# aukeschaap/ttcross

Measured on AMD Instinct MI355X. Metric: fiber evals/s (neval / wall time of dtt_dmrgg), Ising C_64 n=51 r=32 piv=2 (d=63), higher is better.
Workload: dtype f64; 1 GPU; Ising C_64 n=51 r=32 piv=2 (d=63); driver=test_crs_ising c 64 51 32 2, bond_groups=8, transport=none (single process), arith=exact, sweeps=16

## Files before the change

### include/ttx.h

```cpp
#ifndef TTX_H
#define TTX_H
#include <stdint.h>

#ifdef __cplusplus
extern "C" {
#endif

#define TTX_OK 0
#define TTX_EINVAL 1
#define TTX_ENODEV 2
#define TTX_EHIP 3
#define TTX_ESTATE 4

#define TTX_FUN_ISING 1
#define TTX_FUN_STDNORM 2
#define TTX_FUN_MVN 3
#define TTX_FUN_HOST 4
#define TTX_FUN_COSCOEFF 5
#define TTX_FUN_DEVICE 6
#define TTX_FUN_TRAINS 7
#define TTX_FUN_PULLBACK 8

#define TTX_ARITH_EXACT 0
#define TTX_ARITH_FAST 1
// ... 53 lines not shown
typedef double (*ttx_host_fun)(const int32_t *m, const int32_t *ind, const int32_t *n, const double *par);
int ttx_set_integrand_host(ttx_engine *h, ttx_host_fun fun, const double *par);
int64_t ttx_host_calls(const ttx_engine *h);

int ttx_set_integrand_device(ttx_engine *h, const void *image, int64_t nbytes, const char *name, const double *par, int32_t npar);
int ttx_set_integrand_device_file(ttx_engine *h, const char *path, const char *name, const double *par, int32_t npar);
int ttx_eval_device(ttx_engine *h, int64_t npts, const int32_t *ind , double *out );

#define TTX_TRAINS_MAX 8
#define TTX_TOP_PRODUCT 1
#define TTX_TOP_RATIO   2
#define TTX_TOP_SQRTABS 3
#define TTX_TOP_DEVICE  4
int ttx_set_integrand_trains(ttx_engine *h, int32_t m, ttx_engine *const *x, int32_t op);
int ttx_set_integrand_trains_device(ttx_engine *h, int32_t m, ttx_engine *const *x, const void *image, int64_t nbytes,
                                    const char *name, const double *par, int32_t npar);
int ttx_set_integrand_trains_device_file(ttx_engine *h, int32_t m, ttx_engine *const *x, const char *path,
                                         const char *name, const double *par, int32_t npar);
int ttx_trainfun_last(const ttx_engine *h, double *ms, int64_t *launches, int64_t *elements);

#define TTX_PULLBACK_MAX 8
typedef struct { ttx_engine *x; const double *const *nodes; double gamma; } ttx_layer;
int ttx_set_integrand_pullback     (ttx_engine *h, int32_t m, const ttx_layer *layer, const double *const *ref ,
                                    const void *image, int64_t nbytes, const char *name, const double *par, int32_t npar);
int ttx_set_integrand_pullback_file(ttx_engine *h, int32_t m, const ttx_layer *layer, const double *const *ref,
                                    const char *path, const char *name, const double *par, int32_t npar);
int ttx_pullback_points(ttx_engine *h, int64_t npts, const int32_t *ind , double *x , double *logq, double *val);
int ttx_pullback_last(const ttx_engine *h, double *ms, int64_t *launches, int64_t *elements, int64_t *nfailed);

int ttx_run(ttx_engine *h);

int ttx_num_sweeps(const ttx_engine *h);
int ttx_get_sweeps(const ttx_engine *h, ttx_sweep_rec *out, int cap);
int ttx_get_tapes(const ttx_engine *h, int32_t *out , int64_t cap);
int64_t ttx_neval(const ttx_engine *h);
double ttx_seconds(const ttx_engine *h);
int ttx_get_ranks(const ttx_engine *h, int32_t *r );
int64_t ttx_core_size(const ttx_engine *h, int k);
int ttx_get_core(const ttx_engine *h, int k, double *buf);

int ttx_quad(ttx_engine *h, const double *w, double *val);

int ttx_accchk(ttx_engine *h, int32_t nlot, double *einf, double *efro, double *ainf, double *afro, int32_t *pivot);

int ttx_ort(ttx_engine *h);
int ttx_svd(ttx_engine *h, double tol, int32_t rmax);
int ttx_norm(ttx_engine *h, double tol, double *val);
int ttx_lognrm(ttx_engine *h, double tol, double *val);
int ttx_dot(ttx_engine *hx, ttx_engine *hy, double *val);
int ttx_ijk(ttx_engine *h, const int32_t *ind, double *val);
#define TTX_EVAL_EXACT 0
#define TTX_EVAL_MFMA 1
#define TTX_EVAL_AUTO 2
int ttx_ijk_batch(ttx_engine *h, int64_t npts, const int32_t *ind , double *out , int32_t mode);
int ttx_ijk_batch_dev(ttx_engine *h, int64_t npts, const int32_t *ind_dev, double *out_dev, int32_t mode);
int ttx_value_batch(ttx_engine *h, int64_t npts, int32_t dd, const double *x , double *out, int32_t mode);
int ttx_eval_last_mode(const ttx_engine *h);
int ttx_zquad(ttx_engine *h, int32_t nf, const double *w, double *out);

int ttx_contract(ttx_engine *h, const int32_t *keep, const double *w, ttx_engine **out);
int ttx_marginals(ttx_engine *h, const double *w, double *out);
int ttx_contract_modesum(const ttx_engine *h, double *ms, double *bytes);

int ttx_lincomb(int32_t m, const double *coef , ttx_engine *const *x , ttx_engine **out);
int ttx_hadamard(ttx_engine *x, ttx_engine *y, ttx_engine **out);
int ttx_algebra_last(const ttx_engine *h, double *ms, double *bytes_read, double *bytes_written);

int ttx_lincomb_round(int32_t m, const double *coef, ttx_engine *const *x, int32_t rsketch, double tol, int32_t rmax,
                      uint64_t seed, int32_t mode, ttx_engine **out);
int ttx_roundsum_last(const ttx_engine *h, double *ms , double *flops, int32_t *lsk , int32_t *mode_ran);

int ttx_mode_apply    (ttx_engine *h, const int32_t *m , const double *A, int32_t mode, ttx_engine **out);
int ttx_mode_apply_dev(ttx_engine *h, const int32_t *m, const double *A_dev, int32_t mode, ttx_engine **out);
int ttx_mode_apply_last(const ttx_engine *h, double *ms, double *bytes_read, double *bytes_written, double *flops, int32_t *mode_ran);

#define TTX_BASIS_COS    1
#define TTX_BASIS_LINEAR 2
#define TTX_BASIS_HALVE_FIRST 1
typedef struct { int32_t kind, flags; double a, b; const double *nodes ; } ttx_basis;

int ttx_basis_batch    (ttx_engine *h, int64_t npts, const double *x , const ttx_basis *basis , double *out, int32_t mode);
int ttx_basis_batch_dev(ttx_engine *h, int64_t npts, const double *x_dev, const ttx_basis *basis, double *out_dev, int32_t mode);
int ttx_basis_tab      (ttx_engine *h, int64_t npts, const double *phi , double *out, int32_t mode);
int ttx_basis_tab_dev  (ttx_engine *h, int64_t npts, const double *phi_dev, double *out_dev, int32_t mode);
int ttx_basis_host     (const ttx_basis *b, int32_t n, int64_t npts, const double *x, int64_t ldx, double *phi );
int ttx_basis_last     (const ttx_engine *h, double *ms_table, double *ms_chain, double *flops, int32_t *mode_ran);

int ttx_basis_grad_batch    (ttx_engine *h, int64_t npts, const double *x , const ttx_basis *basis , double *val, double *grad , int32_t mode);
int ttx_basis_grad_batch_dev(ttx_engine *h, int64_t npts, const double *x_dev, const ttx_basis *basis, double *val_dev, double *grad_dev, int32_t mode);
int ttx_basis_grad_tab      (ttx_engine *h, int64_t npts, const double *phi, const double *dphi , double *val, double *grad, int32_t mode);
int ttx_basis_grad_tab_dev  (ttx_engine *h, int64_t npts, const double *phi_dev, const double *dphi_dev, double *val_dev, double *grad_dev, int32_t mode);
int ttx_basis_host_d        (const ttx_basis *b, int32_t n, int64_t npts, const double *x, int64_t ldx, double *dphi );
int ttx_basis_grad_last     (const ttx_engine *h, double *ms_table, double *ms_back, double *ms_fwd, double *flops, int32_t *mode_ran, int64_t *chunk_ran);

int ttx_sample(ttx_engine *h, int64_t npts, const double *u , const double *w, const int32_t *fixed, int32_t *ind, double *logq, double *val);
int ttx_sample_dev(ttx_engine *h, int64_t npts, const double *u, const double *w, const int32_t *fixed, int32_t *ind, double *logq, double *val);
int ttx_sample_last(const ttx_engine *h, double *ms_head, double *bytes_head, double *ms_draw, int64_t *nfailed);

int ttx_sample_sq    (ttx_engine *h, int64_t npts, const double *u , const double *w, const int32_t *fixed,
                      double gamma, int32_t mode, int32_t *ind, double *logq, double *val);
int ttx_sample_sq_dev(ttx_engine *h, int64_t npts, const double *u, const double *w, const int32_t *fixed,
                      double gamma, int32_t mode, int32_t *ind, double *logq, double *val);
int ttx_sample_sq_last(const ttx_engine *h, double *ms_head, double *ms_rows, double *ms_pick, double *flops, int64_t *nfailed, int32_t *mode_ran);

int ttx_sample_real    (ttx_engine *h, int64_t npts, const double *u , const double *const *nodes ,
                        const double *cond , double *x , int32_t *cell , double *logq, double *val);
int ttx_sample_real_dev(ttx_engine *h, int64_t npts, const double *u, const double *const *nodes, const double *cond, double *x, int32_t *cell, double *logq, double *val);
int ttx_sample_real_last(const ttx_engine *h, double *ms_head, double *bytes_head, double *ms_draw, int64_t *nfailed);

int ttx_sample_sq_real    (ttx_engine *h, int64_t npts, const double *u , const double *const *nodes ,
                           const double *cond , double gamma, int32_t mode, double *x , int32_t *cell ,
                           double *logq, double *val);
int ttx_sample_sq_real_dev(ttx_engine *h, int64_t npts, const double *u, const double *const *nodes, const double *cond, double gamma, int32_t mode, double *x,
                           int32_t *cell, double *logq, double *val);
int ttx_sample_sq_real_last(const ttx_engine *h, double *ms_head, double *ms_rows, double *ms_pick, double *flops, int64_t *nfailed, int32_t *mode_ran);

int ttx_rosenblatt_sq_real    (ttx_engine *h, int64_t npts, const double *x , const double *const *nodes ,
                               const double *cond , double gamma, int32_t mode, double *u , int32_t *cell ,
                               double *logq, double *val);
int ttx_rosenblatt_sq_real_dev(ttx_engine *h, int64_t npts, const double *x, const double *const *nodes, const double *cond, double gamma, int32_t mode, double *u,
                               int32_t *cell, double *logq, double *val);
int ttx_rosenblatt_sq_real_last(const ttx_engine *h, double *ms_head, double *ms_rows, double *ms_cdf, double *flops, int64_t *nfailed, int32_t *mode_ran);

#define TTX_TOPK_ABS 0
#define TTX_TOPK_MAX 1
#define TTX_TOPK_MIN 2
int ttx_topk(ttx_engine *h, int32_t K, int32_t which, const int32_t *fixed , int32_t mode,
             int32_t *nfound, int32_t *ind , double *val , double *bound);
int ttx_topk_last(const ttx_engine *h, double *ms_gram, double *ms_score, double *ms_select, double *flops, int32_t *mode_ran);

int ttx_replicate(ttx_engine *h, ttx_engine **out);

int ttx_from_tt(ttx_engine **out, int32_t d, const int32_t *n, const int32_t *r, const double *cores, int32_t device);
int ttx_write(const ttx_engine *h, const char *path);
int ttx_read(ttx_engine **out, const char *path, int32_t device);
int ttx_get_modes(const ttx_engine *h, int32_t *d, int32_t *n);
int ttx_write_hdf5(const ttx_engine *h, const char *path);
int ttx_read_hdf5(ttx_engine **out, const char *path, int32_t device);

#define TTX_K_LOTTERY 0
#define TTX_K_HALFSTEP 1
#define TTX_K_ACCEPT 2
#define TTX_K_EXCHANGE 3
#define TTX_K_QUAD 4
#define TTX_K_OTHER 5
#define TTX_K_NKINDS 6
int ttx_set_profile(ttx_engine *h, int on);
int ttx_sweep_path(const ttx_engine *h);
int ttx_plan_describe(const ttx_engine *h, char *buf, int64_t cap);
int ttx_cluster_eval(const ttx_engine *h);
int ttx_arith(const ttx_engine *h);
int ttx_cluster_fallbacks(const ttx_engine *h);
int ttx_cluster_entry(const ttx_engine *h, int64_t out[3]);
int ttx_det_fallbacks(const ttx_engine *h);
int ttx_fun_id(const ttx_engine *h);
int64_t ttx_resid_halfsteps(const ttx_engine *h);
int ttx_kernel_stats(const ttx_engine *h, int64_t launches[TTX_K_NKINDS], double ms[TTX_K_NKINDS], double bytes[TTX_K_NKINDS]);


int ttx_k_residual_argmax(int32_t device, int32_t m, int32_t r, const double *a, const double *F, const double *x,
                          double *b_out, int32_t *imax, double *bmax);
int ttx_k_residual_bench(int32_t device, int64_t m, int32_t r, int32_t iters, double *avg_ms, double *bytes);
int ttx_k_eval(int32_t device, int32_t fun_id, int32_t d, const int32_t *n, const double *par, int32_t npar,
               const double *aux, int32_t naux, int64_t npts, const int32_t *ind, double *out);
int ttx_k_eval_arith(int32_t device, int32_t fun_id, int32_t d, const int32_t *n, const double *par, int32_t npar,
                     const double *aux, int32_t naux, int64_t npts, const int32_t *ind, double *out, int32_t arith);
int ttx_k_lottery(int32_t device, int32_t npnt, int32_t m, int32_t n, int32_t nz, const int32_t *zcol,
                  const int32_t *zrow, uint64_t rngpos, int32_t *points );
int ttx_k_fast_block(int32_t device, int32_t fun_id, int32_t d, int32_t n, const double *par, int32_t npar, const double *aux, int32_t naux,
                     int32_t p, int32_t rL, const int32_t *Lidx, int32_t rR, const int32_t *Ridx, int32_t cap, int32_t chain,
                     int64_t npts, const int32_t *pts, double *near, double *dv, double *piv, double *lot, double *colf, double *rowf,
                     double *nfar, double *pnt);
int ttx_fast_tables(const ttx_engine *h, int32_t group, int32_t side, int32_t bond, int32_t cols, int32_t *info, int32_t *idx, double *near,
                    double *dv, double *piv);

int ttx_k_exp(int32_t device, int64_t n, const double *x, double *out);
int ttx_exp_host(int64_t n, const double *x, double *out);

int ttx_k_latency_probe(int32_t device, double out[5]);

int ttx_k_rccl_selftest(int32_t device, int64_t msg_bytes, int32_t nsum);

int ttx_k_xcc_map(int32_t device, int32_t nblocks, int32_t *out);

#ifdef __cplusplus
}
#endif
#endif
```

### ttcross_amd/csrc/ttx_cluster.h

```cpp
#pragma once
#include "ttx_fused.h"
#include "ttx_mvn.h"
#include "ttx_cluster_rules.h"

#define CB 256

struct ClD2 { double a, b; };
struct ClStrided {
    const char *p; size_t sb; unsigned at;
    __device__ __forceinline__ ClStrided(const double *base, size_t at_, size_t stride) : p((const char *)base), sb(8 * stride), at((unsigned)(8 * at_)) {}
    __device__ __forceinline__ double operator()() { const double v = *(const double *)(p + at); p += sb; return v; }
};

__device__ __forceinline__ double f_ising_c4p(int m, int A, const double *an, const double *aw, double s1n, double s1w,
                                              double s2n, double s2w, const double *bn, const double *bw,
                                              double pv, double pvk, double pw, double pwk)
{
    const int nb = m - A - 2;
    double v = pv, w = pw, vk = pvk, wk = pwk;
    auto vstep = [&](double xv) { vk = vk * xv; v = v + vk; };
    auto wstep = [&](double xv) { wk = wk * xv; w = w + wk; };
    vstep(s2n); vstep(s1n);
    chain8v<true>(an, A, vstep);
    wstep(s1n); wstep(s2n);
    chain8v<false>(bn, nb, wstep);
    double b = 1.0 / (v * w);
    double f = 2 * b;
    auto fstep = [&](double xv) { f = f * xv; };
    chain8v<false>(aw, A, fstep);
    fstep(s1w); fstep(s2w);
    chain8v<false>(bw, nb, fstep);
    return f;
}

template <class STEP>
__device__ __forceinline__ void chain8w(const double *p, int nc, STEP step)
{
#pragma unroll 1
    for (int ch = 0; ch < nc; ch++) {
        double x[8];
        ld8d(p + 8 * ch, x);
#pragma unroll
        for (int k = 0; k < 8; k++) step(x[k]);
    }
}
__device__ __forceinline__ double f_ising_c4w(int cA, int cB, const double *an, const double *aw, double s1n, double s1w,
                                              double s2n, double s2w, const double *bn, const double *bw,
                                              double pv, double pvk, double pw, double pwk)
{
    double v = pv, w = pw, vk = pvk, wk = pwk;
    auto vstep = [&](double xv) { vk = vk * xv; v = v + vk; };
    auto wstep = [&](double xv) { wk = wk * xv; w = w + wk; };
    vstep(s2n); vstep(s1n);
    chain8w(an, cA, vstep);
    wstep(s1n); wstep(s2n);
    chain8w(bn, cB, wstep);
    double b = 1.0 / (v * w);
    double f = 2 * b;
    auto fstep = [&](double xv) { f = f * xv; };
    chain8w(aw, cA, fstep);
    fstep(s1w); fstep(s2w);
    chain8w(bw, cB, fstep);
    return f;
}

__device__ __forceinline__ double wave_max_key(double x)
{
    const ClKey k = cl_key(x);
    const int hmax = wave_max_i(k.hi);
    const unsigned lmax = wave_max_u(cl_key_lo_at(k, hmax));
    return cl_unkey(ClKey{hmax, lmax});
}
__device__ __forceinline__ void wave_argmax2(double &a, double &v, int &idx)
{
    const double amx = wave_max_key(a);
    const int key = (a == amx && idx != INT_MAX) ? ((idx << 1) | (signbit(v) ? 1 : 0)) : INT_MAX;
    const int kmin = wave_min_i(key);
    a = amx;
    if (kmin == INT_MAX) { idx = INT_MAX; v = 0.0; }
    else { idx = kmin >> 1; v = (kmin & 1) ? -amx : amx; }
}

__device__ __forceinline__ double f_ising_cfast(double xj, double wj, double xk, double wk, double pv, double pvk, double pw, double pwk,
                                                double SL, double WL, double SR, double WR)
{
    const double v = pv + pvk * xk * (1.0 + xj * (1.0 + SL));
    const double w = pw + pwk * xj * (1.0 + xk * (1.0 + SR));
    return 2.0 / (v * w) * ((WL * wj) * (wk * WR));
}

typedef unsigned int u4 __attribute__((ext_vector_type(4)));
struct ClRec { u4 a, b; };
static_assert(sizeof(ClRec) == sizeof(ClPart), "record buffers are sized as ClPart: [2][G][TTX_CLREC] u4 arg-max records, then as many running-maximum records");
__device__ __forceinline__ void st16(void *p, u4 v) { asm volatile("global_store_dwordx4 %0, %1, off sc1" :: "v"(p), "v"(v) : "memory"); }
__device__ __forceinline__ u4 ld16(const void *p)
{
    u4 v;
    asm volatile("global_load_dwordx4 %0, %1, off sc1\n\ts_waitcnt vmcnt(0)" : "=v"(v) : "v"(p) : "memory");
    return v;
}

__device__ __forceinline__ int xcc_id() { return (int)__builtin_amdgcn_s_getreg(((4 - 1) << 11) | 20) & 15; }

__device__ __forceinline__ bool cluster_sync(unsigned *ctr, unsigned target, int *abortflag, int *s_ok)
{
    asm volatile("s_waitcnt vmcnt(0)" ::: "memory");
    __syncthreads();
    if (threadIdx.x == 0) {
        int ok = 1;
        unsigned spins = 0;
        __hip_atomic_fetch_add(ctr, 1u, __ATOMIC_RELEASE, __HIP_MEMORY_SCOPE_AGENT);
        while (__hip_atomic_load(ctr, __ATOMIC_RELAXED, __HIP_MEMORY_SCOPE_AGENT) < target) {
            __builtin_amdgcn_s_sleep(1);
            if (++spins > (1u << 22)) { ok = 0; __hip_atomic_store(abortflag, 1, __ATOMIC_RELAXED, __HIP_MEMORY_SCOPE_SYSTEM); break; }
            if ((spins & 1023u) == 0 && __hip_atomic_load(abortflag, __ATOMIC_RELAXED, __HIP_MEMORY_SCOPE_SYSTEM)) { ok = 0; break; }
        }
        __atomic_thread_fence(__ATOMIC_ACQUIRE);
        *s_ok = ok;
    }
    __syncthreads();
    return *s_ok != 0;
}

#ifdef TTX_STAMPS
#define CST_DECL const bool t_me = (threadIdx.x == 0 && g == 0 && cb == 0); long long t_prev = wall_clock64()
#define CST(k) do { if (t_me) { long long t_now = wall_clock64(); gs.stamp[0][k] += t_now - t_prev; t_prev = t_now; } } while (0)
#define CST_END() do { if (t_me) gs.nstamp[0]++; } while (0)
#define CSE_DECL const int t_eb = (threadIdx.x == 0 && g == 0 && cb <= 1) ? cb : -1; long long t_eprev = wall_clock64()
#define CSE_MARK() do { if (t_eb >= 0) t_eprev = wall_clock64(); } while (0)
#define CSE(k) do { if (t_eb >= 0) { long long t_now = wall_clock64(); P.gs[0].stamp[1][8 * t_eb + (k)] += t_now - t_eprev; t_eprev = t_now; } } while (0)
#define CSE_END() do { if (t_eb == 0) P.gs[0].nstamp[1]++; } while (0)
#define WST(k) do { if (P.dbg && g == 0 && epoch == 8 && pp == 4 && lane == 0 && h < 8) P.dbg[((size_t)(h * 64 + cb * 4 + wv)) * 8 + (k)] = (long long)__builtin_readcyclecounter(); } while (0)
#else
#define WST(k)
#define CST_DECL
#define CST(k)
#define CST_END()
#define CSE_DECL
#define CSE_MARK()
#define CSE(k)
#define CSE_END()
#endif

#define CL_ZKEEP 1
#define CL_ZCARRY 2
#define CL_WORD 4
#define CL_POWTAB 8
static_assert(CL_POWTAB_N == CB, "one table entry per thread of a workgroup");
__device__ const ClPowTab cl_powtab = cl_make_powtab();
struct ClArgs { DevProb P; int dir, nsteps, NB, ldsinv, epoch, zkeep; };
__device__ __forceinline__ int *cl_zimage(const DevProb &P, int g, int nsteps)
{ return (int *)(P.cl_part + (size_t)2 * P.G * TTX_CLREC) + (size_t)g * cl_zimage_ints(nsteps, P.RM); }

template <bool CFAST, bool CPAD>
__global__ __launch_bounds__(CB) void k_sweep_cluster(DevProb P, int dir, int nsteps, int NB, int ldsinv, int epoch, int zkeep)
{
    extern __shared__ __align__(16) double dyn[];
    __shared__ int zc[128], zr[128], zcs[128], zrs[128], keepc[128], keepr[128];
    __shared__ int nzc, nzr, nsc, nsr, s_ok;
    __shared__ int slt[2][TTX_CLMAX + 1], wtab[TTX_CLMAX];
    __shared__ ttx_cdfseg segc[TTX_TABSEG], segr[TTX_TABSEG];
    __shared__ double sha[8], shv[8], shm[8]; __shared__ int shi[8];
    __shared__ double pLw[64], pLk[64], pRv[64], pRk[64];
    static_assert(!(CFAST && CPAD), "the closed form reads the rows in dimension order");
    constexpr int NFT = CFAST ? 64 : 1;
    __shared__ double fSL[NFT], fWL[NFT], fSR[NFT], fWR[NFT];
    __shared__ struct { int ii, jj, kk, qq, hcount, rc_k, rc_q, rr_i, rr_j; double pivot, amax, bytes_half; long long neval, n_resid; } s_rook;
    const int bid = blockIdx.x;
    const int g = (bid & 7) + 8 * (bid / (8 * NB)), cb = (bid >> 3) % NB;
    CSE_DECL;
    if (g >= P.G || P.ctl[0]) return;
    const int bpar = (epoch - 1) & 1;
    if (P.tail_side && epoch >= 2) {
        const TailRec &t0 = P.tailrec[(size_t)bpar * P.G];
        if (stop_rule(epoch - 1, P.maxrank, P.accuracy, t0.pivotmax, max_pos(t0.amax, P.gs[0].amax_bnd[bpar]), P.strk[epoch & 1]).ready) return;
    }
    if (P.cl_test_abort && P.cl_test_abort == epoch && g == 0 && cb == 0) {
        if (threadIdx.x == 0) { __hip_atomic_store(P.cl_abort, 1, __ATOMIC_RELAXED, __HIP_MEMORY_SCOPE_SYSTEM); P.ctl[0] = 1; }
        return;
    }
    const int tid = threadIdx.x, m = P.d, RM = P.RM, NM = P.NM;
    const int lane = tid & 63, wv = tid >> 6;
    GroupState &gs = P.gs[g];
    const int first = gs.first, last = gs.last, nbonds = last - first + 1;
    int *r = P.r + (size_t)g * (m + 2);
    const int VS = ((m + 7) & ~7) + 8;
    const int RS = 2 * VS + 2;
    const int n1m = P.n[1];
    const int SL = RM * ((NM + NB - 1) / NB + 1);
    unsigned *ctr = P.cl_ctr + g;
    unsigned nbar = (unsigned)(epoch - 1) * (unsigned)min(nsteps, nbonds);
    ClPart *part = P.cl_part;
    double *par = dyn;
    double *XL = par + ((P.npar + 1) & ~1);
    double *XR = XL + (size_t)RM * RS;
    double *acol = XR + (size_t)RM * RS;
    double *arow = acol + SL;
    double *resc = arow + SL;
    double *resr = resc + SL;
    double *xsc = resr + SL;
    double *xsr = xsc + ((RM + 1) & ~1);
    int *lot = (int *)(xsr + ((RM + 1) & ~1));
    double *GL = (double *)(lot + 4 * ((2 * RM + 2 * NM + 4 + 1) & ~1));
    double *GU = GL + (size_t)RM * RM;
    int *ZK = (int *)(ldsinv ? GU + (size_t)RM * RM : GL);
    int *ZN = ZK + (size_t)nsteps * 2 * RM;
    for (int x = tid; x < P.npar; x += CB) par[x] = P.par[x];
    if (cb == 0) {
        if (tid == 0) { gs.pivotmax = -1.0; gs.pivotmin = -1.0; }
        int *rr = P.rr + (size_t)g * (m + 2);
        for (int s = tid; s <= m; s += CB) rr[s] = r[s];
    }
    __syncthreads();
    CSE(0);
    if ((zkeep & CL_ZCARRY) && cl_lists_valid(gs.zk_epoch, epoch)) {
        const int *img = cl_zimage(P, g, nsteps);
        for (int x = tid; x < nbonds * 2 * RM; x += CB) ZK[x] = img[x];
        for (int x = tid; x < 2 * nbonds; x += CB) ZN[x] = img[(size_t)nsteps * 2 * RM + x];
        if (cb == 0 && tid == 0) gs.n_zload++;
        __syncthreads();
    } else if (zkeep & CL_ZKEEP) {
        int *TMP = (int *)XL;
        const int E = nbonds * 2 * RM;
        for (int x = tid; x < E; x += CB) {
            const int b = x / (2 * RM), side = (x / RM) & 1, u = x % RM, pb = first + b;
            if (u < r[pb]) { const int *vp = vip_ptr(P, g, pb, first) + 4 * u; TMP[x] = (vp[2 * side + 1] << 16) | vp[2 * side]; }
        }
        __syncthreads();
        for (int x = tid; x < E; x += CB) {
            const int b = x / (2 * RM), u = x % RM, nb_ = r[first + b];
            if (u < nb_) {
                const int *src = TMP + (x - u); const int a = src[u]; int ra = 0;
                for (int t = 0; t < nb_; t++) ra += (src[t] < a) || (src[t] == a && t < u);
                ZK[(x - u) + ra] = a;
            }
        }
        __syncthreads();
        for (int x = tid; x < E; x += CB) {
            const int b = x / (2 * RM), u = x % RM, nb_ = r[first + b];
            if (u < nb_) {
                const int *src = ZK + (x - u); int pc = 0;
                for (int t = 1; t <= u; t++) pc += (src[t] != src[t - 1]);
                const bool keep = (u == 0) || (src[u] != src[u - 1]);
                TMP[x] = keep ? pc : -1;
                if (u == nb_ - 1) ZN[x / RM] = pc + 1;
            }
        }
        __syncthreads();
        int mykey = 0, mypos = -1;
        for (int x0 = 0; x0 < E; x0 += CB) {
            const int x = x0 + tid;
            mypos = -1;
            if (x < E) { const int b = x / (2 * RM), u = x % RM; if (u < r[first + b]) { mypos = TMP[x]; mykey = ZK[x]; } }
            __syncthreads();
            if (mypos >= 0) ZK[(x - x % RM) + mypos] = mykey;
            __syncthreads();
        }
    }
    double amax = gs.amax, pivotmax = -1.0, pivotmin = -1.0;
    if (P.tail_side && epoch >= 2) amax = max_pos(amax, gs.amax_bnd[bpar]);
    const double pivotmax_prev = gs.pivotmax_prev;
    long long neval = gs.neval;
    unsigned long long rngpos = gs.rngpos;
    double bytes_half = gs.bytes_half; long long n_resid = gs.n_resid;
    int hcount = 0;
    CSE(1);
    const bool ptab = (zkeep & CL_POWTAB) != 0;
    const unsigned long long bil0 = ptab ? cl_powtab.v[tid] : ttx_minstd_pow(2ull * tid);
    unsigned long long sA0;
    {
        const unsigned long long cw = gs.rngword, cwpos = gs.rngword_pos;
        if ((zkeep & CL_WORD) && cl_word_valid(cw, cwpos, rngpos)) { sA0 = cw; if (cb == 0 && tid == 0) gs.n_wload++; }
        else sA0 = ttx_minstd_pow(2 * rngpos + 1);
    }
    const int bl0 = ptab ? (int)cl_powtab.v[lane] : (int)ttx_minstd_pow(2ull * lane);
    constexpr unsigned long long c64 = cl_minstd_pow_c(128);
    CSE(2);
    CST_DECL;

    for (int pp = 1; pp <= nsteps; pp++) {
        if (pp > nbonds) break;
        const int p = (dir == 1) ? first + pp - 1 : last + 1 - pp;
        const int r0 = r[p - 1], r1 = r[p], r2 = r[p + 1], n1 = P.n[p], n2 = P.n[p + 1];
        const int nlot = r0 + n1 + n2 + r2;
        double *Cp = core_ptr(P, P.col, g, p, first), *Wq = core_ptr(P, P.row, g, p + 1, first);
        double *Ap = core_ptr(P, P.arg, g, p, first), *Aq = core_ptr(P, P.arg, g, p + 1, first);
        const short *Lt = L_ptr(P, g, p - 1, first), *Rt = R_ptr(P, g, p + 1, first);
        const int cA = (p - 1 + 7) >> 3, cB = (m - p - 1 + 7) >> 3;
        const int sside = (tid >> 6) & 1, sseg = tid & 63;
        double sg_a0 = 0.0, sg_al = 0.0, sg_de = 0.0; int sg_k0 = 0, sg_cn = 0, myns = 0;
        auto seg_issue = [&](int Kc_, int Kr_) {
            if (tid >= 128) {
                const int K = sside ? Kr_ : Kc_; const ttx_cdfseg *sp = P.cdf_tab + (size_t)K * TTX_TABSEG + sseg;
                myns = P.cdf_ns[K]; sg_a0 = sp->a0; sg_al = sp->alast; sg_de = sp->delta; sg_k0 = sp->k0; sg_cn = sp->cnt;
            }
        };
        {
            const int AL = min(VS, (p - 1 + 7) & ~7), AR = min(VS, (m - p - 1 + 7) & ~7);
            if (AL > 0) {
                int c = tid / AL, o = tid - c * AL;
// ... 232 lines not shown
            if (resid) wave_argmax2(ab, bb, ix);
            WST(5);
            if (!ok) {
                if (lane == 0) { __hip_atomic_store(P.cl_abort, 1, __ATOMIC_RELAXED, __HIP_MEMORY_SCOPE_SYSTEM); P.ctl[0] = 1; *(volatile int *)&s_ok = 0; }
                return;
            }
            CST(9);
            hcount++;
            neval += nf;
            bytes_half += resid ? 8.0 * ((double)nf * r1 + r1 + 2.0 * nf) : 8.0 * nf;
            n_resid += resid ? 1 : 0;
            done = dn;
            if (resid) {
                if (ix == INT_MAX) ix = 0;
                if (iscol) { const int i = ix % r0 + 1, j = ix / r0 + 1; done = havecol && haverow && (i == ii && j == jj); ii = i; jj = j; }
                else       { const int k = ix % n2 + 1, q = ix / n2 + 1; done = havecol && haverow && (k == kk && q == qq); kk = k; qq = q; }
                pivot = bb;
            }
        }
        if (P.piv != 0) {
            u4 *bufB = (u4 *)part + ((size_t)((hcount - 1) & 1) * P.G + g) * TTX_CLREC + (size_t)2 * P.G * TTX_CLREC;
            const unsigned gen = ((unsigned)epoch << 20) | (unsigned)hcount;
            double mx = 0.0; int ok = 1;
            if (slot_on) {
                unsigned spins = 0;
                for (;;) {
                    const u4 rb = ld16(&bufB[lane]);
                    if (rb.z == gen) { mx = __longlong_as_double((long long)(((unsigned long long)rb.y << 32) | rb.x)); break; }
                    if (++spins > 64u) __builtin_amdgcn_s_sleep(1);
                    if (spins > (1u << 22)) { ok = 0; break; }
                    if ((spins & 1023u) == 0 && __hip_atomic_load(P.cl_abort, __ATOMIC_RELAXED, __HIP_MEMORY_SCOPE_SYSTEM)) { ok = 0; break; }
                }
            }
            ok = __all(ok);
            if (!ok) {
                if (lane == 0) { __hip_atomic_store(P.cl_abort, 1, __ATOMIC_RELAXED, __HIP_MEMORY_SCOPE_SYSTEM); P.ctl[0] = 1; *(volatile int *)&s_ok = 0; }
                return;
            }
            amax = fmax(amax, wave_max_key(mx));
        }
        if (tid == 0) {
            s_rook.ii = ii; s_rook.jj = jj; s_rook.kk = kk; s_rook.qq = qq; s_rook.hcount = hcount; s_rook.rc_k = rc_k; s_rook.rc_q = rc_q;
            s_rook.rr_i = rr_i; s_rook.rr_j = rr_j; s_rook.pivot = pivot; s_rook.amax = amax; s_rook.bytes_half = bytes_half; s_rook.neval = neval; s_rook.n_resid = n_resid;
        }
        }
        __syncthreads();
        if (!*(volatile int *)&s_ok) return;
        if (!rook_active) {
            ii = s_rook.ii; jj = s_rook.jj; kk = s_rook.kk; qq = s_rook.qq; hcount = s_rook.hcount; rc_k = s_rook.rc_k; rc_q = s_rook.rc_q;
            rr_i = s_rook.rr_i; rr_j = s_rook.rr_j; pivot = s_rook.pivot; amax = s_rook.amax; bytes_half = s_rook.bytes_half; neval = s_rook.neval; n_resid = s_rook.n_resid;
        }
        CST(10);
        int *tape = P.tape + ((size_t)g * (m + 2) + p) * 4;
        const bool upd = accept_pivot(pivot, amax, pivotmax_prev, P.small_element, P.small_pivot);
        if (!upd) {
            if (cb == 0 && tid == 0) { tape[0] = tape[1] = tape[2] = tape[3] = -1; P.upd[(size_t)g * (m + 2) + p] = 0; }
        } else {
            const int i0 = ii - 1, j0 = jj - 1, k0 = kk - 1, q0 = qq - 1;
            double *gI = inv_ptr(P, g, p, first);
            const bool reuseA = (rc_k == kk && rc_q == qq), reuseB = (rr_i == ii && rr_j == jj);
            AppendTab tab{0, 0};
            if (cb == 0) tab = append_tables_fetch(P, g, p, first, ii, qq, tid);
            if (reuseA && reuseB) {
                if (cb == 0)
                    for (int s = tid; s < r1; s += CB) {
                        const double c = Wq[k0 + (size_t)NM * q0 + P.SW * s], w = Cp[i0 + (size_t)RM * j0 + P.SS * s];
                        gI[r1 * r1 + s] = w; gI[r1 * r1 + r1 + s] = c;
                    }
            } else {
                for (int s = tid; s < r1; s += CB) { xsc[s] = Wq[k0 + (size_t)NM * q0 + P.SW * s]; xsr[s] = Cp[i0 + (size_t)RM * j0 + P.SS * s]; }
                __syncthreads();
                if (cb == 0)
                    for (int s = tid; s < r1; s += CB) { gI[r1 * r1 + s] = xsr[s]; gI[r1 * r1 + r1 + s] = xsc[s]; }
            }
            for (int u = tid; u < r0 * nj; u += CB) {
                const int i = u % r0, j = jlo + u / r0; const size_t o = i + (size_t)RM * j;
                const double a = acol[u];
                Ap[o + P.SS * r1] = a;
                double y;
                if (reuseA) y = resc[u];
                else {
                    y = a;
                    ClStrided lc(Cp, o, P.SS); const double *xp = xsc;
                    cl_ordered_sum<16>(r1u, [&] { const double xv = *xp++; return ClD2{xv, lc()}; }, [&](int, ClD2 e) { y = y + (-e.a) * e.b; });
                }
                Cp[o + P.SS * r1] = (1.0 / pivot) * y;
            }
            for (int u = tid; u < nk * r2; u += CB) {
                const int k = klo + u % nk, q = u / nk;
                const double a = arow[u];
                Aq[r1 + (size_t)RM * k + P.SS * q] = a;
                const size_t o = k + (size_t)NM * q;
                if (reuseB) Wq[o + P.SW * r1] = resr[u];
                else {
                    double tt = 0.0;
                    ClStrided lw(Wq, o, P.SW); const double *xp = xsr;
                    cl_ordered_sum<16>(r1u, [&] { const double xv = *xp++; return ClD2{lw(), xv}; }, [&](int, ClD2 e) { tt = tt + e.a * e.b; });
                    Wq[o + P.SW * r1] = a + (-1.0) * tt;
                }
            }
            CST(11);
            if (p > first) {
                const double *gL = ldsinv ? GL : inv_ptr(P, g, p - 1, first);
                double *Wp = core_ptr(P, P.row, g, p, first);
                const int pk = (r0 <= 32) ? 2 : 1, lw = 64 / pk, l = lane & (lw - 1), sub = lane / lw;
                for (int base = wv * pk; base < nj; base += (CB / 64) * pk) {
                    const int jl = base + sub, j = jlo + jl;
                    const bool on = (jl < nj) && (l < r0);
                    const double a = on ? acol[l + r0 * jl] : 0.0;
                    const double xf = (pk == 2) ? dev_solve_L<2>(gL, r0, a, l, sub) : dev_solve_L<1>(gL, r0, a, l, 0);
                    if (on) Wp[j + (size_t)NM * r1 + P.SW * l] = xf;
                }
            }
            CST(12);
            if (p < last) {
                const double *gU = ldsinv ? GU : inv_ptr(P, g, p + 1, first);
                double *Cq = core_ptr(P, P.col, g, p + 1, first);
                const int pk = (r2 <= 32) ? 2 : 1, lw = 64 / pk, l = lane & (lw - 1), sub = lane / lw;
                const double rdg = dev_solve_rdg(gU, r2, l);
                for (int base = wv * pk; base < nk; base += (CB / 64) * pk) {
                    const int kl = base + sub, k = klo + kl;
                    const bool on = (kl < nk) && (l < r2);
                    const double y0 = on ? arow[kl + nk * l] : 0.0;
                    const double y = (pk == 2) ? dev_solve_U<2>(gU, r2, y0, rdg, l, sub) : dev_solve_U<1>(gU, r2, y0, rdg, l, 0);
                    if (on) Cq[r1 + (size_t)RM * k + P.SS * l] = y;
                }
            }
            CST(13);
            if (cb == 0) {
                append_tables_store(P, g, p, first, r1, ii, jj, kk, qq, tid, CB, tab);
                if (tid == 0) append_scalars(P, g, p, first, r1, ii, jj, kk, qq, pivot);
            }
            if ((zkeep & CL_ZKEEP) && wv < 2) {
                const int b = p - first;
                int *kl = ZK + (size_t)b * 2 * RM + (size_t)wv * RM;
                const int nl = ZN[2 * b + wv];
                const int key = wv == 0 ? ((jj << 16) | ii) : ((qq << 16) | kk);
                const int v = (lane < nl) ? kl[lane] : INT_MAX;
                const bool dup = __ballot(v == key) != 0ull;
                const int pos = __popcll(__ballot(v < key));
                if (!dup) {
                    if (lane < nl && v > key) kl[lane + 1] = v;
                    if (lane == 0) { kl[pos] = key; ZN[2 * b + wv] = nl + 1; }
                }
            }
            pivot_range(pivotmax, pivotmin, fabs(pivot));
        }
        CST(14);
        if (!cluster_sync(ctr, (++nbar) * (unsigned)NB, P.cl_abort, &s_ok)) { if (tid == 0) P.ctl[0] = 1; return; }
        CST(15);
        CST_END();
    }
    CSE_MARK();
    if (cb == 0) {
        const ClArgs *K = (const ClArgs *)__builtin_amdgcn_kernarg_segment_ptr();
        asm volatile("" : "+s"(K));
        if (K->zkeep & CL_ZCARRY) {
            const int ns = K->nsteps, rm = K->P.RM;
            int *img = cl_zimage(K->P, g, ns);
            for (int x = tid; x < nbonds * 2 * rm; x += CB) img[x] = ZK[x];
            for (int x = tid; x < 2 * nbonds; x += CB) img[(size_t)ns * 2 * rm + x] = ZN[x];
        }
        if (tid == 0) {
            gs.amax = amax; gs.pivotmax = pivotmax; gs.pivotmin = pivotmin; gs.neval = neval; gs.rngpos = rngpos;
            gs.bytes_half = bytes_half; gs.n_resid = n_resid;
            if (K->zkeep & CL_WORD) { gs.rngword = sA0; gs.rngword_pos = rngpos; }
            if (K->zkeep & CL_ZCARRY) gs.zk_epoch = K->epoch;
            if (P.tail_side) gs.amax_bnd[epoch & 1] = 0.0;
        }
        __syncthreads();
        exch_pack_group(P, g);
        CSE(3);
        CSE_END();
    }
}
```

### ttcross_amd/csrc/ttx_cluster_rules.h

```cpp
#pragma once
#include "ttx_cdf.h"

TTX_HD int cl_slice(int c, int n, int NB) { return (int)((unsigned)c * (unsigned)n / (unsigned)NB); }

TTX_HD int cl_wact(int nj, int nk, int r0, int r2, int nw)
{
    const int a = r0 * nj, b = nk * r2, e = a > b ? a : b, w = (e + 63) >> 6;
    return w < 1 ? 1 : (w > nw ? nw : w);
}

struct ClKey { int hi; unsigned lo; };
TTX_HD ClKey cl_key(double x) { const uint64_t b = ttx_dbits(x); return ClKey{(int)(uint32_t)(b >> 32), (unsigned)b}; }
TTX_HD double cl_unkey(ClKey k) { return ttx_bitsd(((uint64_t)(uint32_t)k.hi << 32) | k.lo); }
TTX_HD unsigned cl_key_lo_at(ClKey k, int hmax) { return k.hi == hmax ? k.lo : 0u; }

#if defined(__clang__)
#define CL_UNROLL _Pragma("unroll")
#define CL_NO_UNROLL _Pragma("unroll 1")
#else
#define CL_UNROLL
#define CL_NO_UNROLL
#endif
template <int N, class LD, class TM>
TTX_HD void cl_sum_piece(int s0, LD &ld, TM &tm)
{
    decltype(ld()) v[N];
    CL_UNROLL
    for (int k = 0; k < N; k++) v[k] = ld();
    CL_UNROLL
    for (int k = 0; k < N; k++) tm(s0 + k, v[k]);
}
template <int B, class LD, class TM>
TTX_HD void cl_ordered_sum(int n, LD ld, TM tm)
{
    static_assert(B == 16 || B == 8, "batches of 16 or 8 terms");
    int s = 0;
    CL_NO_UNROLL
    for (; s + B <= n; s += B) cl_sum_piece<B>(s, ld, tm);
    const int rem = n - s;
    if constexpr (B > 8) if (rem & 8) { cl_sum_piece<8>(s, ld, tm); s += 8; }
    if (rem & 4) { cl_sum_piece<4>(s, ld, tm); s += 4; }
    if (rem & 2) { cl_sum_piece<2>(s, ld, tm); s += 2; }
    if (rem & 1) cl_sum_piece<1>(s, ld, tm);
}

#define CL_POWTAB_N 256
constexpr uint64_t cl_mulmod31_c(uint64_t a, uint64_t b)
{
    uint64_t x = a * b;
    x = (x & 2147483647ULL) + (x >> 31);
    x = (x & 2147483647ULL) + (x >> 31);
    return (x >= 2147483647ULL) ? x - 2147483647ULL : x;
}
constexpr uint64_t cl_minstd_pow_c(uint64_t e)
{
    uint64_t base = 48271ULL, w = 1;
    while (e) { if (e & 1) w = cl_mulmod31_c(w, base); base = cl_mulmod31_c(base, base); e >>= 1; }
    return w;
}
struct ClPowTab { uint32_t v[CL_POWTAB_N]; };
constexpr ClPowTab cl_make_powtab()
{
    ClPowTab t{};
    for (int k = 0; k < CL_POWTAB_N; k++) t.v[k] = (uint32_t)cl_minstd_pow_c(2ULL * (uint64_t)k);
    return t;
}

template <class LANE>
TTX_HD uint64_t cl_stepmul(int nlot, LANE lane, uint64_t c64)
{
    if (nlot >= 512) return ttx_minstd_pow(2ull * (uint64_t)nlot);
    uint64_t s = lane(nlot & 63);
    for (int a = 0; a < (nlot >> 6); a++) s = ttx_mulmod31(s, c64);
    return s;
}

TTX_HD bool cl_word_valid(uint64_t word, uint64_t wpos, uint64_t rngpos) { return word != 0 && wpos == rngpos; }
TTX_HD bool cl_lists_valid(int tag, int epoch) { return tag != 0 && tag == epoch - 1; }
TTX_HD size_t cl_zimage_ints(int nsteps, int RM) { return ((size_t)nsteps * 2 * (size_t)RM + 2 * (size_t)nsteps + 3) & ~(size_t)3; }
```

### ttcross_amd/csrc/ttx_create_plan.h

```cpp
#pragma once
#include <algorithm>
#include <cmath>
#include <cstdarg>
#include <cstddef>
#include <cstdio>
#include <cstdlib>
#include <cstring>
#include <mutex>
#include <string>
#include <vector>

#include "../../include/ttx.h"
#include "ttx_dev.h"
#include "ttx_qr_plan.h"

#if defined(__HIPCC__)
#define TTX_PLAN_HD __host__ __device__ inline
#else
#define TTX_PLAN_HD inline
#endif

#define DE5_W 4
#define DE5_SEG 16
TTX_PLAN_HD size_t de5_lds_doubles(int m) { const int VS = ((m + 7) & ~7) + 8 + DE5_SEG; return (size_t)5 * VS + 128 + (size_t)DE5_W * 64; }
TTX_PLAN_HD bool de5_fits(int m) { return m >= 3; }
TTX_PLAN_HD int de_rows_stride(int m) { const int s = m + 56; return ((s + 31) & ~31) + 16; }
TTX_PLAN_HD size_t de_rows_lds_doubles(int m) { return (size_t)12 * de_rows_stride(m); }
TTX_PLAN_HD int det_vs(int m) { return ((m + 7) & ~7) + 8; }
TTX_PLAN_HD size_t det_lds_doubles(int m, int nbk) { return (size_t)4 * det_vs(m) + 256 + (det_vs(m) + 48) + (size_t)3 * nbk * 16 * 64; }

constexpr int TTX_PLAN_FB = 1024;
constexpr int TTX_PLAN_FNR = 24;
constexpr int TTX_PLAN_MVN_MAXQ = 8;

struct EnvText { bool set = false; std::string v; };
struct CreateEnv {
    EnvText arith;
    EnvText sweep;
    EnvText cl_pad;
    bool fullpiv_mfma = false;
    bool fast_persist_off = false;
    bool de_lane = false;
    bool de_tables_off = false, de_fastdiv_off = false, de_cut_off = false, de_v2_off = false, de_team_off = false;
    bool de_lot_point_set = false; int de_lot_point = 0;
    int de_team_units = 256, de_team6_units = 1024;
    int de_test_fault = 0;
    bool de_v5 = false;
    int cluster_nb = 8;
    bool cluster_coop = false;
    int cluster_test_abort = 0;
    bool dbg_waves = false;
    bool lottery_one_block = false;
    bool lottery_wave_off = false;
    bool lottery_rows2 = false;
    bool mvn_v2_off = false;
    bool tail_off = false;
    bool tail_side_off = false;
    bool head_direct_off = false;
    bool init_wave_off = false;
    bool fin_early_off = false;
    bool fin_skip_exch_off = false;
    bool init_wide_off = false;
    bool quad_lds_off = false;
    bool cl_powtab_off = false;
    bool cl_word_off = false;
    bool cl_lists_off = false;
};
template <class Get>
CreateEnv create_env_from(Get get)
{
    auto text = [&](const char *name) { EnvText t; if (const char *e = get(name)) { t.set = true; t.v = e; } return t; };
    auto num = [&](const char *name, int dflt) { const char *e = get(name); return e ? atoi(e) : dflt; };
    auto off = [&](const char *name) { const char *e = get(name); return e && atoi(e) == 0; };
    CreateEnv v;
    v.arith = text("TTX_ARITH"); v.sweep = text("TTX_SWEEP"); v.cl_pad = text("TTX_CL_PAD");
    v.fullpiv_mfma = text("TTX_FULLPIV").v == "mfma";
    v.fast_persist_off = off("TTX_FAST_PERSIST");
    v.de_lane = num("TTX_DE_LANE", 0) == 1;
    v.de_tables_off = off("TTX_DE_TABLES"); v.de_fastdiv_off = off("TTX_DE_FASTDIV"); v.de_cut_off = off("TTX_DE_CUT");
    v.de_v2_off = off("TTX_DE_V2"); v.de_team_off = off("TTX_DE_TEAM");
    v.de_lot_point_set = get("TTX_DE_LOT_POINT") != nullptr; v.de_lot_point = num("TTX_DE_LOT_POINT", 0);
    v.de_team_units = num("TTX_DE_TEAM_UNITS", v.de_team_units); v.de_team6_units = num("TTX_DE_TEAM6_UNITS", v.de_team6_units);
    v.de_test_fault = num("TTX_DE_TEST_FAULT", 0);
    v.de_v5 = num("TTX_DE_V5", 0) == 1;
    v.cluster_nb = num("TTX_CLUSTER_NB", v.cluster_nb);
    v.cluster_coop = num("TTX_CLUSTER_COOP", 0) == 1;
    v.cluster_test_abort = num("TTX_CLUSTER_TEST_ABORT", 0);
    v.dbg_waves = get("TTX_DBG_WAVES") != nullptr;
    v.lottery_one_block = num("TTX_LOTTERY_NB", 0) == 1;
    v.lottery_wave_off = off("TTX_LOTTERY_WAVE");
    v.lottery_rows2 = num("TTX_LOTTERY_ROWS", 0) == 2;
    v.mvn_v2_off = off("TTX_MVN_V2");
    v.tail_off = off("TTX_TAIL"); v.tail_side_off = off("TTX_TAIL_SIDE");
    v.head_direct_off = off("TTX_HEAD_DIRECT"); v.init_wave_off = off("TTX_INIT_WAVE");
    v.fin_early_off = off("TTX_FIN_EARLY"); v.fin_skip_exch_off = off("TTX_FIN_SKIP_EXCH");
    v.init_wide_off = off("TTX_INIT_WIDE"); v.quad_lds_off = off("TTX_QUAD_LDS");
    v.cl_powtab_off = off("TTX_CL_POWTAB"); v.cl_word_off = off("TTX_CL_WORD"); v.cl_lists_off = off("TTX_CL_LISTS");
    return v;
}
struct DevCaps { int ncu = 0; bool coop = false; };

enum SweepWant { SWEEP_AUTO, SWEEP_CHAIN, SWEEP_FUSED, SWEEP_CLUSTER };
enum SlotKind { SLOTS_NONE, SLOTS_HOST, SLOTS_DEVICE };

struct CdfTables { std::vector<ttx_cdfseg> tab; std::vector<int> ns; };

struct CreatePlan {
    int err = TTX_OK; std::string errtext;
    int d = 0, RM = 0, NM = 0, W = 1, wrank = 0, nproc = 1, g0 = 0, G = 0, nbmax = 0, NC = 0, mode = 0, H = 0;
    std::vector<int32_t> own;
    int ising_id = 0; bool isDE = false;
    double mvn_norm = 1.0;
    size_t SS = 0, SW = 0, CS = 0, XD = 0, IOFF = 0, MSZ = 0, QB = 0, SB = 0, VS = 0;
    int nfb = 0, nlotmax = 0;
    int nn = 0, snum = 0;
    SlotKind slots = SLOTS_NONE; size_t HS = 0;
    int cdf_kmax = -1;
    bool pfull = false, qscr = false;
    bool want_fast = false;
    bool unit_nodes = false;
    int arith = 0, FD = 0, fpersist = 0;
    bool fast_tables = false;
    int de_npair = 0;
    int de_unit = 0, de_cut = 0;
    int de_slots = 0;
    int de_v2 = 0;
    int de_team = 0, de_team_units = 256, de_team6_units = 1024;
    int de_v5 = 0;
    int de_test_fault = 0;
    int de_lot_point = 0;
    int lot_wave = 0, lot_rows = 0;
    size_t lds_de = 0, lds_det = 0, lds_det6 = 0, lds_de5 = 0, lds_der = 0;
    int mvn_v2 = 0; size_t lds_mvn = 0;
    int lot_nb = 1, bnd_wave = 0;
    bool lot_cand = false;
    int fp_mfma = 0, fp_tiles = 0;
    size_t lds_par = 0, lds_half = 0, lds_lot = 0;
    int half_vals = 0, lot_vals = 0, fast_cap = 0;
    size_t lds_fused = 0, lds_cluster = 0;
    bool fused_ok = false;
    int cluster_cand = 0;
    int cluster_var = 0;
    int cluster_ldsinv = 0, cluster_zkeep = 0, cluster_coop = 0;
    bool cl_powtab = true, cl_word = true, cl_lists = false;
    int cl_test_abort = 0; bool dbg_waves = false;
    bool sweep_tail = true;
    bool sweep_tail_side = true;
    bool head_direct = true;
    size_t lds_qtree = 0;
    bool init_wide = true;
    bool init_wave = true;
    bool fin_early = true;
    bool fin_skip_exch = true;
    SweepWant sweep_want = SWEEP_AUTO; int ncu = 0;
    int fused = 0;
    int cluster = 0;
};

inline size_t quad_tree_lds(int nproc, size_t RM, bool on)
{
    const size_t need = sizeof(double) * 2 * (size_t)nproc * RM * RM;
    return on && nproc > 1 && need <= TTX_LDS_WORK ? need : 0;
}
struct InitSamplesPlan { int threads = 256, rows = 0; size_t lds = 0; };
inline InitSamplesPlan init_samples_plan(size_t lds_par, size_t VS, int d, long nsamples, bool own_rows, bool wide)
{
    InitSamplesPlan p;
    const size_t lds1 = lds_par + 16 + sizeof(short) * 256 * VS;
    p.rows = lds1 <= TTX_LDS_WORK ? 1 : 0;
    p.lds = p.rows ? lds1 : lds_par;
    if (!p.rows || !wide || !own_rows) return p;
    const int threads = (int)std::min<long>(512, std::max<long>(256, (nsamples + 63) / 64 * 64));
    const size_t lds2 = lds_par + 16 + sizeof(short) * (size_t)threads * VS + 16 + sizeof(int) * (size_t)(d + 1);
    if (lds2 <= TTX_LDS_WORK) { p.threads = threads; p.rows = 2; p.lds = lds2; }
    return p;
}

inline void share(int first, int last, int nproc, std::vector<int32_t> &own)
{
    own.assign(nproc + 1, 0);
    own[0] = first;
    for (int p = 1; p < nproc; p++) own[p] = first + (int)((double)(last - first + 1) * (double)p / nproc);
    own[nproc] = last + 1;
}
inline double powi(double a, int b)
{
    double r = 1.0;
    for (;;) { if (b & 1) r *= a; b /= 2; if (b == 0) break; a *= a; }
    return r;
}
inline bool cdf_tables(int kmax, CdfTables &out)
{
    out.tab.assign((size_t)(kmax + 1) * TTX_TABSEG, ttx_cdfseg());
    out.ns.assign(kmax + 1, 0);
    std::vector<ttx_cdfseg> tmp(TTX_MAXSEG);
    for (int K = 1; K <= kmax; K++) {
        const int n_ = ttx_cdf_build(K, tmp.data());
        if (n_ > TTX_TABSEG) { out = CdfTables(); return false; }
        out.ns[K] = n_;
        memcpy(&out.tab[(size_t)K * TTX_TABSEG], tmp.data(), sizeof(ttx_cdfseg) * n_);
    }
    return true;
}
inline bool cdf_table_fits(int kmax)
{
    static std::mutex mu;
    static int looked = 0, first_over = -1;
    if (kmax > 16384) return false;
    std::lock_guard<std::mutex> lk(mu);
    std::vector<ttx_cdfseg> tmp(TTX_MAXSEG);
    while (looked < kmax && first_over < 0) { looked++; if (ttx_cdf_build(looked, tmp.data()) > TTX_TABSEG) first_over = looked; }
    return first_over < 0 || kmax < first_over;
}

#if defined(__GNUC__)
__attribute__((format(printf, 3, 4)))
#endif
inline CreatePlan &plan_refuse(CreatePlan &p, int code, const char *fmt, ...)
{
    char buf[512];
    va_list ap; va_start(ap, fmt); vsnprintf(buf, sizeof buf, fmt, ap); va_end(ap);
    p.err = code; p.errtext = buf;
    return p;
}

inline CreatePlan create_plan(const ttx_config &cfg, bool nofun, const CreateEnv &env, const DevCaps &caps)
{
    CreatePlan p;
    const int d = cfg.d, fun = cfg.fun_id, nproc = std::max(cfg.nproc, 1);
    p.d = d; p.RM = cfg.maxrank; p.nproc = nproc; p.ncu = caps.ncu;
    p.W = cfg.world_size < 1 ? 1 : cfg.world_size; p.wrank = cfg.world_rank;
    int NM = 1;
    for (int k = 0; k < d; k++) { if (cfg.n[k] < 1 || cfg.n[k] > 32000) return plan_refuse(p, TTX_EINVAL, "bad mode size"); NM = std::max(NM, cfg.n[k]); }
    p.NM = NM;
    if ((long long)p.RM * NM > (long long)TTX_MAXPART * TTX_BLK) return plan_refuse(p, TTX_EINVAL, "maxrank*n too large");
    if (cfg.mybonds) p.own.assign(cfg.mybonds, cfg.mybonds + nproc + 1);
    else share(1, d - 1, nproc, p.own);
    for (int g = 0; g < nproc; g++) if (p.own[g + 1] <= p.own[g]) return plan_refuse(p, TTX_EINVAL, "mybonds: empty group %d", g);
    if (p.own[0] != 1 || p.own[nproc] != d) return plan_refuse(p, TTX_EINVAL, "mybonds: must run from 1 to d = %d (got %d .. %d)", d, p.own[0], p.own[nproc]);
    p.g0 = (int)((long long)nproc * p.wrank / p.W);
    p.G = (int)((long long)nproc * (p.wrank + 1) / p.W) - p.g0;
    for (int g = 0; g < nproc; g++) p.nbmax = std::max(p.nbmax, p.own[g + 1] - p.own[g]);
    p.NC = p.nbmax + 1;
    p.mode = (cfg.pivoting == 0) ? 1 : (cfg.pivoting < 0) ? 2 : 0;
    p.H = (cfg.pivoting <= 0) ? 2 : 2 * cfg.pivoting;
    p.ising_id = (fun == TTX_FUN_ISING) ? (int)cfg.par[2 * cfg.n[0]] : 0;
    p.isDE = fun == TTX_FUN_ISING && p.ising_id != 1;
    if (fun == TTX_FUN_MVN) {
        if (cfg.naux < d + d * d + 1) return plan_refuse(p, TTX_EINVAL, "mvn: aux too short");
        p.mvn_norm = std::sqrt(powi(2.0 * 3.141592653589793, d) * cfg.aux[d + (size_t)d * d]);
        if (!(p.mvn_norm > 0.0) || !std::isfinite(p.mvn_norm))
            return plan_refuse(p, TTX_EINVAL, "ttx_create: mvn normalisation sqrt((2 pi)^d det) = %g is not a positive finite number (det = %g under- or overflows at d = %d)",
                               p.mvn_norm, cfg.aux[d + (size_t)d * d], d);
    }
    const size_t RM = p.RM;
    const size_t VS = ((d + 7) & ~7) + 8;
    const int nlotmax = 2 * p.RM + 2 * NM;
    p.VS = VS; p.nlotmax = nlotmax;
    p.SS = RM * NM; p.SW = (size_t)NM * RM; p.CS = RM * NM * RM;
    p.nfb = (int)((RM * NM + TTX_BLK - 1) / TTX_BLK);
    p.XD = RM * NM + RM * RM;
    p.IOFF = (sizeof(int) * (XH + d + 2) + 15) & ~(size_t)15;
    p.MSZ = (p.IOFF + sizeof(double) * p.XD + 15) & ~(size_t)15;
    p.QB = (size_t)nproc * RM * RM + 2 * nproc;
    p.lds_qtree = quad_tree_lds(nproc, RM, !env.quad_lds_off);
    p.SB = SUM_HDR + nproc + 5 * (size_t)(d + 1);
    p.qscr = 2 * sizeof(double) * (RM * RM + 2) > TTX_LDS_WORK;
    p.nn = cfg.n[0];
    for (int k = 1; k < d; k++) p.nn = std::min(p.nn, cfg.n[k]);
    p.snum = std::max(8, nproc);

    bool want = cfg.arith == TTX_ARITH_FAST;
    if (cfg.arith != TTX_ARITH_EXACT && cfg.arith != TTX_ARITH_FAST) return plan_refuse(p, TTX_EINVAL, "ttx_create: arith must be TTX_ARITH_EXACT or TTX_ARITH_FAST (got %d)", cfg.arith);
    if (env.arith.set) {
        if (env.arith.v == "fast") want = true;
        else if (env.arith.v != "exact") return plan_refuse(p, TTX_EINVAL, "TTX_ARITH must be exact or fast (got %s)", env.arith.v.c_str());
    }
    p.want_fast = want && !nofun;
    bool unit = fun == TTX_FUN_ISING;
    for (int j = 0; unit && j < std::min(NM, (int)cfg.npar); j++) unit = cfg.par[j] >= 0.0 && cfg.par[j] <= 1.0;
    p.unit_nodes = unit;
    p.arith = (p.want_fast && ((p.isDE && unit) || fun == TTX_FUN_MVN)) ? 1 : 0;
    if (p.arith) {
        p.fast_tables = true;
        p.FD = d + 1;
        p.fpersist = (fun == TTX_FUN_MVN && env.fast_persist_off) ? 0 : 1;
    }
    if (p.isDE && !p.arith && env.de_lane) p.de_unit = unit;
    if (p.isDE && !p.arith && !env.de_lane && !env.de_tables_off) {
        p.de_npair = d * (d + 1) / 2;
        p.de_unit = unit && !env.de_fastdiv_off;
        p.de_cut = (p.de_unit && !env.de_cut_off) ? 1 : 0;
        p.de_lot_point = (env.de_lot_point_set ? env.de_lot_point : (int)(d <= 160)) != 0;
        p.de_slots = (int)RM * ((NM + 63) / 64);
        p.lds_de = sizeof(double) * (5 * VS + 256) + (p.de_cut ? sizeof(int) * VS : 0);
        p.de_v2 = cfg.pivoting >= 0 && p.de_slots <= TTX_MAXPART && p.lds_de <= TTX_LDS_WORK && !env.de_v2_off;
        p.lds_det = sizeof(double) * det_lds_doubles(d, 3);
        p.lds_det6 = sizeof(double) * det_lds_doubles(d, 1);
        p.de_team = p.de_v2 && !p.de_cut && p.lds_det <= TTX_LDS_WORK && !env.de_team_off;
        p.de_team_units = env.de_team_units;
        p.de_team6_units = env.de_team6_units;
        p.de_test_fault = env.de_test_fault;
        p.lds_de5 = sizeof(double) * de5_lds_doubles(d);
        p.de_v5 = p.de_v2 && !p.de_cut && de5_fits(d) && p.lds_de5 <= TTX_LDS_WORK && env.de_v5;
    }
    p.pfull = cfg.pivoting < 0;
    if (cfg.pivoting < 0 && env.fullpiv_mfma && RM <= 64 && (long long)(RM * NM) * (long long)(RM * NM) < (1LL << 31)) {
        const size_t side = RM * NM;
        p.fp_mfma = 1; p.fp_tiles = (int)(((side + 63) / 64) * ((side + 63) / 64));
    }
    if (cdf_table_fits(p.RM * NM)) p.cdf_kmax = p.RM * NM;

    p.lds_par = sizeof(double) * (cfg.npar + 2);
    {
        const size_t base = sizeof(double) * (cfg.npar + RM + 4);
        const size_t idx_bytes = sizeof(short) * ((RM + 1) * VS + 16), val_bytes = sizeof(double) * ((RM + 1) * 2 * VS + 4);
        p.half_vals = (fun == TTX_FUN_ISING && p.ising_id == 1 && base + val_bytes <= TTX_LDS_VALUES) ? 1 : 0;
        p.lds_half = base + (p.half_vals ? val_bytes : idx_bytes);
        const size_t dif_bytes = sizeof(double) * ((RM + 1) * VS + 4);
        if (fun == TTX_FUN_MVN && base + dif_bytes <= TTX_LDS_HALF_DIFF) { p.half_vals = 1; p.lds_half = base + dif_bytes; }
        if (p.arith) p.lds_half = std::max(p.lds_half, base + sizeof(double) * ((size_t)std::max(p.FD, TTX_PLAN_FNR) + 4 + RM + 2));
    }
    const size_t lot_hdr = sizeof(double) * (cfg.npar + 4) + sizeof(int) * 4 * (nlotmax + 4);
    {
        p.lds_lot = lot_hdr + sizeof(short) * (2 * RM * VS + 16);
        const size_t lot_dif = lot_hdr + sizeof(double) * (2 * RM * VS + 4);
        if (fun == TTX_FUN_MVN && lot_dif <= TTX_LDS_LOTTERY) { p.lot_vals = 1; p.lds_lot = lot_dif; }
        if (p.arith && fun == TTX_FUN_ISING) {
            const size_t hdr = lot_hdr + 32;
            const size_t rowb = 2 * sizeof(double) * RM;
            p.fast_cap = (int)std::min<size_t>(std::min<size_t>(40, (size_t)d + 1), hdr < TTX_LDS_VALUES ? (TTX_LDS_VALUES - hdr) / rowb : 0);
            p.lds_lot = std::max(p.lds_lot, hdr + rowb * p.fast_cap);
        }
    }
    {
        const bool fastc = fun == TTX_FUN_ISING && p.ising_id == 1 && cfg.pivoting >= 0 && p.cdf_kmax >= 0;
        p.lds_fused = sizeof(double) * (cfg.npar + 4 + 4 * RM * VS + 2 * RM * NM + RM + 4) + sizeof(int) * 4 * (nlotmax + 4);
        p.fused_ok = fastc && p.RM <= 64 && nlotmax <= TTX_PLAN_FB && p.lds_fused <= TTX_LDS_WORK;
        int NB = std::max(1, std::min(env.cluster_nb, TTX_CLMAX));
        while (NB > 1 && p.G * NB > caps.ncu / 2) NB--;
        const size_t SL = RM * ((NM + NB - 1) / NB + 1);
        p.lds_cluster = sizeof(double) * (cfg.npar + 4 + 2 * RM * (2 * VS + 2) + 4 * SL + 2 * RM + 8) + sizeof(int) * 4 * (nlotmax + 4);
        if (p.lds_cluster + sizeof(double) * 2 * RM * RM <= TTX_LDS_WORK) { p.cluster_ldsinv = 1; p.lds_cluster += sizeof(double) * 2 * RM * RM; }
        const size_t zk = sizeof(int) * ((size_t)p.nbmax * 2 * RM + 2 * p.nbmax + 4);
        if (p.lds_cluster + zk <= TTX_LDS_WORK) { p.cluster_zkeep = 1; p.lds_cluster += zk; }
        p.cl_powtab = !env.cl_powtab_off; p.cl_word = !env.cl_word_off; p.cl_lists = p.cluster_zkeep && !env.cl_lists_off;
        const bool cfastc = p.want_fast && fun == TTX_FUN_ISING && p.ising_id == 1;
        if (env.cl_pad.set && env.cl_pad.v != "0" && env.cl_pad.v != "1") return plan_refuse(p, TTX_EINVAL, "TTX_CL_PAD must be 0 or 1 (got %s)", env.cl_pad.v.c_str());
        p.cluster_var = cfastc ? 2 : (unit && !(env.cl_pad.set && env.cl_pad.v == "0")) ? 1 : 0;
        if (fastc && p.RM <= 64 && NB >= 2 && p.G * NB <= caps.ncu && p.lds_cluster <= TTX_LDS_WORK) {
            p.cluster_cand = NB;
            p.cluster_coop = caps.coop && env.cluster_coop;
        }
        p.cl_test_abort = env.cluster_test_abort; p.dbg_waves = env.dbg_waves;
        p.sweep_tail = !env.tail_off; p.sweep_tail_side = !env.tail_side_off;
        p.head_direct = !env.head_direct_off; p.init_wave = !env.init_wave_off; p.init_wide = !env.init_wide_off;
        p.fin_early = !env.fin_early_off; p.fin_skip_exch = !env.fin_skip_exch_off;
        const std::string want_sweep = env.sweep.set ? env.sweep.v : "auto";
        if (want_sweep == "cluster") p.sweep_want = SWEEP_CLUSTER;
        else if (want_sweep == "fused") p.sweep_want = SWEEP_FUSED;
        else if (want_sweep == "auto") p.sweep_want = SWEEP_AUTO;
        else if (want_sweep == "chain") p.sweep_want = SWEEP_CHAIN;
        else return plan_refuse(p, TTX_EINVAL, "TTX_SWEEP must be auto, chain, fused or cluster (got %s)", want_sweep.c_str());
    }
    if (!nofun && (p.lds_half > TTX_LDS_DEVICE || p.lds_lot > TTX_LDS_LOTTERY)) return plan_refuse(p, TTX_EINVAL, "problem too large for LDS staging (d*maxrank)");
    {
        const bool heavy = p.isDE || fun == TTX_FUN_MVN;
        if (heavy && !env.lottery_one_block) p.lot_nb = std::min((nlotmax + 63) / 64, 64);
        if (p.lot_nb > 1 && (nlotmax + p.lot_nb - 1) / p.lot_nb > 64) p.lot_nb = 1;
        if (fun == TTX_FUN_MVN && d <= 64 * TTX_PLAN_MVN_MAXQ && cfg.pivoting >= 0 && (int)RM * ((NM + 63) / 64) <= TTX_MAXPART && !env.mvn_v2_off) {
            p.lot_cand = true;
            p.mvn_v2 = 1; p.de_slots = (int)RM * ((NM + 63) / 64);
            p.bnd_wave = 1;
            p.lds_mvn = sizeof(double) * (3 * (size_t)d + 8);
        }
        if (p.isDE && p.arith) p.bnd_wave = 1;
        if (p.isDE && p.de_npair) {
            p.lot_cand = true;
            p.lds_der = sizeof(double) * de_rows_lds_doubles(d);
            p.lot_wave = p.de_v2 && !p.de_cut && p.lds_der <= TTX_LDS_WORK && !env.lottery_wave_off;
            p.bnd_wave = p.lot_wave || (p.de_cut && p.de_v2 && p.lds_der <= TTX_LDS_WORK);
            p.lot_rows = p.lot_wave ? (env.lottery_rows2 ? 2 : 1) : 0;
        }
    }
    if (fun == TTX_FUN_HOST || fun == TTX_FUN_COSCOEFF || fun == TTX_FUN_DEVICE || fun == TTX_FUN_TRAINS || fun == TTX_FUN_PULLBACK) {
        p.HS = std::max<size_t>({RM * NM, (size_t)p.nn * p.snum, (size_t)p.NC * NM, (size_t)nlotmax, (size_t)2 * NM, (size_t)256});
        p.slots = fun == TTX_FUN_HOST ? SLOTS_HOST : SLOTS_DEVICE;
    }
    return p;
}

inline void create_admit(CreatePlan &p, int occ)
{
    bool cluster_ok = p.cluster_cand != 0;
    if (cluster_ok) {
        const long long cap = (long long)occ * p.ncu;
        const long long grid = 8LL * p.cluster_cand * ((p.G + 7) / 8);
        if (grid * 2 > cap) cluster_ok = false;
    }
    if (p.sweep_want == SWEEP_CLUSTER) { if (cluster_ok) p.cluster = p.cluster_cand; }
    else if (p.sweep_want == SWEEP_FUSED) { if (p.fused_ok) p.fused = 1; }
    else if (p.sweep_want == SWEEP_AUTO) { if (cluster_ok) p.cluster = p.cluster_cand; else if (p.fused_ok && p.G == 1) p.fused = 1; }
    if (p.cluster && p.cluster_var == 2) p.arith = 1;
}
```

### ttcross_amd/csrc/ttx_engine.hip

```cpp
#include <hip/hip_runtime.h>

#include <chrono>
#include <cmath>
#include <cstdarg>
#include <cstdio>
#include <cstdlib>
#include <cstring>
#include <map>
#include <memory>
#include <string>
#include <thread>
#include <type_traits>
#include <vector>

#include <atomic>
#include <dlfcn.h>
#include <rccl/rccl.h>

#include "../../include/ttx.h"
#include "../../include/ttx_device_fun.h"
#include "ttx_err.h"
#include "ttx_lds.h"
#include "ttx_qr_plan.h"
#include "ttx_create_plan.h"
#include "ttx_loop_plan.h"
#include "ttx_shm.h"
#include "ttx_host_pool.h"
#include "ttx_files.h"
#include "ttx_init.h"
#include "ttx_kernels.h"
#include "ttx_wavestep.h"
#include "ttx_de.h"
#include "ttx_mvn.h"
#include "ttx_quadfin.h"
#include "ttx_exchange.h"
#include "ttx_sweep_end.h"
#include "ttx_ttops.h"
#include "ttx_fused.h"
#include "ttx_cluster.h"
#include "ttx_coscoeff.h"
#include "ttx_eval.h"
#include "ttx_contract.h"
#include "ttx_modeapply.h"
#include "ttx_basis.h"
#include "ttx_basis_grad.h"
#include "ttx_algebra.h"
#include "ttx_roundsum.h"
#include "ttx_sample.h"
#include "ttx_sample_real.h"
#include "ttx_topk.h"
#include "ttx_sample_sq.h"
#include "ttx_sample_sq_real.h"
#include "ttx_trainfun.h"
#include "ttx_pullback.h"

typedef void (*cluster_kernel_t)(DevProb, int, int, int, int, int, int);
static cluster_kernel_t cluster_kernel(int var)
{
    return var == 2 ? k_sweep_cluster<true, false> : var == 1 ? k_sweep_cluster<false, true> : k_sweep_cluster<false, false>;
}


static int env_int(const char *name, int dflt) { const char *e = getenv(name); return e ? atoi(e) : dflt; }
static bool env_off(const char *name) { const char *e = getenv(name); return e && atoi(e) == 0; }

static int ensure_lds(int device, const void *fn, size_t need)
{
    return ttx_lds_raise(device, fn, need, [](const void *fn, size_t need) -> int {
        HIPCHECK(hipFuncSetAttribute(fn, hipFuncAttributeMaxDynamicSharedMemorySize, (int)need));
        return TTX_OK;
    });
}

extern "C" const char *ttx_last_error(void) { return g_err.c_str(); }
extern "C" int ttx_version(void) { return 3; }


struct RcclApi {
    void *lib = nullptr;
    ncclResult_t (*GetUniqueId)(ncclUniqueId *) = nullptr;
    ncclResult_t (*CommInitRank)(ncclComm_t *, int, ncclUniqueId, int) = nullptr;
    ncclResult_t (*CommDestroy)(ncclComm_t) = nullptr;
    ncclResult_t (*Send)(const void *, size_t, ncclDataType_t, int, ncclComm_t, hipStream_t) = nullptr;
    ncclResult_t (*Recv)(void *, size_t, ncclDataType_t, int, ncclComm_t, hipStream_t) = nullptr;
    ncclResult_t (*AllReduce)(const void *, void *, size_t, ncclDataType_t, ncclRedOp_t, ncclComm_t, hipStream_t) = nullptr;
    ncclResult_t (*GroupStart)() = nullptr;
    ncclResult_t (*GroupEnd)() = nullptr;
    const char *(*GetErrorString)(ncclResult_t) = nullptr;
};
static RcclApi g_rccl;
static int rccl_load()
{
    if (g_rccl.lib) return TTX_OK;
    void *L = dlopen("librccl.so", RTLD_NOW | RTLD_GLOBAL);
    if (!L) L = dlopen("/opt/rocm/lib/librccl.so", RTLD_NOW | RTLD_GLOBAL);
    if (!L) return fail(TTX_EHIP, "cannot load librccl.so: %s", dlerror());
#define SYM_(f, name) *(void **)(&g_rccl.f) = dlsym(L, name); if (!g_rccl.f) return fail(TTX_EHIP, "librccl.so lacks %s", name);
    SYM_(GetUniqueId, "ncclGetUniqueId") SYM_(CommInitRank, "ncclCommInitRank") SYM_(CommDestroy, "ncclCommDestroy")
    SYM_(Send, "ncclSend") SYM_(Recv, "ncclRecv") SYM_(AllReduce, "ncclAllReduce") SYM_(GroupStart, "ncclGroupStart")
    SYM_(GroupEnd, "ncclGroupEnd") SYM_(GetErrorString, "ncclGetErrorString")
#undef SYM_
    g_rccl.lib = L;
    return TTX_OK;
}
#define NCCLCHECK(x) do { ncclResult_t e_ = (x); if (e_ != ncclSuccess) return fail(TTX_EHIP, "%s failed: %s", #x, g_rccl.GetErrorString(e_)); } while (0)

enum {
    SC_TRAIN,
    SC_META,
    SC_IND, SC_OUT, SC_X,
    SC_FLAG, SC_LQ,
    SC_XA, SC_XB, SC_SORT,
    SC_W, SC_M, SC_P, SC_SCR, SC_VEC,
    SC_H, SC_ROW, SC_CNT,
    SC_SRX,
    SC_TFUN, SC_TVAL,
    SC_PB, SC_PBREF, SC_PBVAL,
    SC_MAT,
    SC_KP, SC_KW, SC_KS, SC_KX,
    SC_KREC, SC_KSEL, SC_KOUT,
    SC_RSO, SC_RSW, SC_RSYA, SC_RSYB,
    SC_RSM, SC_RSTAB,
    SC_QH, SC_QF, SC_QS, SC_QX,
    SC_BTAB,
    SC_GST,
    SC_NBUF
};
struct EvBuf { void *p = nullptr; size_t bytes = 0; };
struct OpTimer {
    hipEvent_t ev[2] = {nullptr, nullptr};
    int start(hipStream_t s) { for (auto &e : ev) if (!e) HIPCHECK(hipEventCreate(&e)); HIPCHECK(hipEventRecord(ev[0], s)); return TTX_OK; }
    int stop(hipStream_t s) { HIPCHECK(hipEventRecord(ev[1], s)); return TTX_OK; }
    int ms(double *out) { float t = 0.f; HIPCHECK(hipEventElapsedTime(&t, ev[0], ev[1])); *out = t; return TTX_OK; }
};
enum { TM_MODESUM, TM_ALG, TM_HEAD, TM_DRAW, TM_APPLY,
       TM_GRAM, TM_SCORE, TM_SELECT,
       TM_RS_SKETCH, TM_N };
struct OpMarks {
    enum { DISCARD = -1 };
    std::vector<hipEvent_t> &pool;
    std::vector<int> phase;
    explicit OpMarks(std::vector<hipEvent_t> &p) : pool(p) {}
    int mark(hipStream_t s, int ph)
    {
        if (phase.size() == pool.size()) { hipEvent_t e; HIPCHECK(hipEventCreate(&e)); pool.push_back(e); }
        HIPCHECK(hipEventRecord(pool[phase.size()], s));
        phase.push_back(ph);
        return TTX_OK;
    }
    int sum(double *ms)
    {
        for (size_t x = 1; x < phase.size(); x++) {
            if (phase[x] == DISCARD) continue;
            float t = 0.f;
            HIPCHECK(hipEventElapsedTime(&t, pool[x - 1], pool[x]));
            ms[phase[x]] += t;
        }
        phase.clear();
        return TTX_OK;
    }
};

enum { SMP_GRID, SMP_REAL, SMP_SQ, SMP_SQ_REAL, SMP_ROS_SQ_REAL, SMP_N };
struct SampleLast { double ms_head = 0.0, bytes = 0.0, ms_draw = 0.0, ms_rows = 0.0, ms_pick = 0.0, flops = 0.0; int64_t failed = 0; int mode = -1; };
struct CtLast { double ms = 0.0, bytes = 0.0; };
struct AlgLast { double ms = 0.0, rd = 0.0, wr = 0.0; };
struct MaLast { double ms = 0.0, rd = 0.0, wr = 0.0, flops = 0.0; int mode = -1; };
struct TkLast { double ms_gram = 0.0, ms_score = 0.0, ms_select = 0.0, flops = 0.0; int mode = -1; };
struct RsLast {
    double ms[4] = {0.0, 0.0, 0.0, 0.0}, flops = 0.0;
    std::vector<int32_t> l;
    int mode = -1;
};
struct BsLast { double ms[2] = {0.0, 0.0}, flops = 0.0; int mode = -1; };
struct BgLast { double ms[3] = {0.0, 0.0, 0.0}, flops = 0.0; int mode = -1; int64_t chunk = 0; };

struct DevFun;
struct TrainFun;
struct PullFun;
struct ttx_engine {
    ttx_config cfg;
    std::vector<int32_t> n1;
    std::vector<double> par, aux, quadw;
    std::vector<int32_t> own;
    int d = 0, RM = 0, NM = 0, G = 0, NC = 0, nbmax = 0, H = 0, mode = 0;
    int g0 = 0;
    int W = 1, wrank = 0;
    DevProb P{};
    hipStream_t stream = nullptr;
    std::vector<void *> allocs;
    size_t SB = 0, QB = 0;
    double *h_sum = nullptr;
    char *h_msg = nullptr;
    double *h_tmp = nullptr;
    char *recvL = nullptr, *recvR = nullptr;
    ncclComm_t comm = nullptr;
    ttx_transport cb{};
    bool have_cb = false;
    int cb_error = 0;
    struct RedJob { ttx_engine *h; double *buf; size_t count; int op; };
    static const int NRED = 16;
    RedJob red[NRED];
    double *red_mem = nullptr; size_t red_cap = 0; int red_next = 0;
    RedJob *red_slot(size_t count, int op)
    {
        if (!red_mem || count > red_cap) return nullptr;
        RedJob *j = &red[red_next];
        j->h = this; j->buf = red_mem + (size_t)red_next * red_cap; j->count = count; j->op = op;
        red_next = (red_next + 1) % NRED;
        return j;
    }
    ShmTransport *shm = nullptr;
    std::vector<ttx_sweep_rec> recs;
    std::vector<int32_t> tapes;
    std::vector<int32_t> rfinal;
    std::vector<std::vector<uint8_t>> updhist;
    int64_t neval = 0;
    double seconds = 0.0;
    bool ran = false;
    bool profile = false;
    struct Ev { int kind, n; hipEvent_t a, b; };
    std::vector<Ev> evs;
    std::vector<hipEvent_t> evpool;
    int64_t k_launches[TTX_K_NKINDS] = {0};
    double k_ms[TTX_K_NKINDS] = {0}, k_bytes[TTX_K_NKINDS] = {0};
    double *Wa = nullptr, *Wb = nullptr, *Wc = nullptr, *Wd = nullptr, *Sm = nullptr, *bak = nullptr;
    int *Si = nullptr;
    CreatePlan sel;
    struct Retired { bool cluster = false, de_team = false, de_v5 = false; } retired;
    int cluster_nb() const { return retired.cluster ? 0 : sel.cluster; }
    bool de_team() const { return sel.de_team && !retired.de_team; }
    bool de_v5() const { return sel.de_v5 && !retired.de_v5; }
    int arith() const { return P.arith; }
    int cluster_fallbacks = 0;
    int det_fallbacks = 0, de5_fallbacks = 0;
    bool cluster_aborted = false;
    double *h_svd = nullptr; double svd_seq = 0.0;
    hipStream_t qstream = nullptr;
    hipEvent_t ev_sum[2] = {nullptr, nullptr}, ev_val[2] = {nullptr, nullptr}, ev_tail[2] = {nullptr, nullptr}, ev_qb[2] = {nullptr, nullptr}, ev_fin[2] = {nullptr, nullptr};
    double *h_sum_base = nullptr;
    double *h_val = nullptr;
    int *h_abort = nullptr;
    ttx_host_fun hfun = nullptr;
    const double *hfun_par = nullptr;
    std::shared_ptr<DevFun> dfun;
    std::shared_ptr<TrainFun> tfun;
    TfOps tf_ops{};
    std::vector<char> tf_host;
    std::vector<std::pair<hipEvent_t, hipEvent_t>> tf_evs;
    bool tf_figures = false;
    int64_t tf_launches = 0, tf_elements = 0;
    double tf_ms = 0.0;
    std::shared_ptr<PullFun> pfun;
    const PullFun *pb_ref_of = nullptr;
    PbOps pb_ops{};
    PbPlan pb_pl;
    std::vector<char> pb_host;
    int64_t pb_failed = 0;
    int64_t host_calls = 0;
    int64_t n_resid = 0;
    EvBuf scratch[SC_NBUF];
    std::vector<char> train_host, meta_host;
    OpTimer timer[TM_N];
    int ncu = 0;
    int ev_last_mode = -1;
    SampleLast smp[SMP_N];
    CtLast ct;
    AlgLast alg;
    MaLast ma;
    TkLast tk;
    RsLast rs;
    BsLast bs;
    BgLast bg;
    std::vector<hipEvent_t> op_ev;
};

static HostPool &host_pool()
{
    static HostPool p(host_pool_threads(getenv("TTX_HOST_THREADS"), getenv("OMP_NUM_THREADS"), std::thread::hardware_concurrency()));
    return p;
}

static int host_eval(ttx_engine *h)
{
    HIPCHECK(hipStreamSynchronize(h->stream));
    HIPCHECK(hipGetLastError());
    DevProb &P = h->P;
    const size_t nslot = (size_t)h->G * h->sel.HS;
    std::vector<uint32_t> todo;
    for (size_t s = 0; s < nslot; s++) if (P.hreq[s]) { todo.push_back((uint32_t)s); P.hreq[s] = 0; }
    const int32_t d = h->d;
    const int32_t *nn = h->n1.data() + 1;
    host_pool().run(todo.size(), [&](size_t i) {
        int32_t ind[2048];
        const short *row = P.hidx + (size_t)todo[i] * d;
        for (int k = 0; k < d; k++) ind[k] = row[k];
        P.hval[todo[i]] = h->hfun(&d, ind, nn, h->hfun_par);
    });
    h->host_calls += (int64_t)todo.size();
    return TTX_OK;
}

struct DevFun {
    int device = 0;
    hipModule_t mod = nullptr;
    hipFunction_t slots = nullptr, list = nullptr;
    ttx_devfun_info info{};
    double *par = nullptr;
    std::string name;
    std::vector<unsigned char> image;
    ~DevFun()
    {
        (void)hipSetDevice(device);
        if (par) (void)hipFree(par);
        else (void)hipDeviceSynchronize();
        if (mod) (void)hipModuleUnload(mod);
    }
};
#define DEVFUN_LAUNCHCHECK(x) do { hipError_t e_ = (x); if (e_ != hipSuccess) return fail(TTX_EHIP, "%s failed: %s (%s:%d)", #x, hipGetErrorString(e_), __FILE__, __LINE__); } while (0)
static int devfun_slots(ttx_engine *h)
{
    DevFun &f = *h->dfun;
    DevProb &P = h->P;
    int d = P.d;
    long long nslot = (long long)h->G * h->sel.HS;
    const int *n = P.n + 1;
    const double *par = f.par;
    const short *hidx = P.hidx; unsigned char *hreq = P.hreq; double *hval = P.hval;
    const int waves = f.info.block / 64;
    const long long want = f.info.kind == TTX_DEVFUN_KIND_WAVE ? (nslot + waves - 1) / waves : (nslot + f.info.block - 1) / f.info.block;
    const unsigned grid = (unsigned)std::max<long long>(1, std::min<long long>(want, 4096));
    void *args[] = {&d, &n, &par, &nslot, &hidx, &hreq, &hval};
    DEVFUN_LAUNCHCHECK(hipModuleLaunchKernel(f.slots, grid, 1, 1, (unsigned)f.info.block, 1, 1, (unsigned)(f.info.lds_per_wave * waves), h->stream, args, nullptr));
    return TTX_OK;
}

struct TrainFun {
    std::vector<ttx_engine *> x;
    int op = 0;
    std::shared_ptr<DevFun> comb;
};
static int tf_grid(ttx_engine *h, long long items);
static int tf_prepare(ttx_engine *h, const char *who, bool figures);
static int tf_finish(ttx_engine *h);
static int tf_eval_list(ttx_engine *h, int64_t npts, const int32_t *ind, double *out);
struct PullFun {
    struct Layer { ttx_engine *x; std::vector<std::vector<double>> nodes; double gamma; };
    std::vector<Layer> layer;
    std::vector<double> ref;
    std::vector<size_t> roff;
    std::shared_ptr<DevFun> comb;
};
static int pb_prepare(ttx_engine *h, const char *who, bool figures, bool need_comb);
static int pb_slots(ttx_engine *h);
static int pb_finish(ttx_engine *h);
static int pb_eval_list(ttx_engine *h, int64_t npts, const int32_t *ind, double *out);
struct TfScope {
    ttx_engine *h; hipEvent_t a = nullptr, b = nullptr;
    bool on;
    explicit TfScope(ttx_engine *h_) : h(h_), on(h_->profile && h_->tf_figures) { if (on) { (void)hipEventCreate(&a); (void)hipEventCreate(&b); (void)hipEventRecord(a, h->stream); } }
    ~TfScope() { if (on) { (void)hipEventRecord(b, h->stream); h->tf_evs.push_back({a, b}); } }
};
static int tf_slots(ttx_engine *h)
{
    const TrainFun &f = *h->tfun;
    DevProb &P = h->P;
    long long nslot = (long long)h->G * h->sel.HS;
    const TfOps &O = h->tf_ops;
    const size_t lds = sizeof(double) * TTX_TF_WAVES * tf_lds_doubles(O.ldx, O.d);
    const dim3 grid(tf_grid(h, nslot)), block(64 * TTX_TF_WAVES);
    const short *hidx = P.hidx; unsigned char *hreq = P.hreq; double *hval = P.hval;
    double *tval = (double *)h->scratch[SC_TVAL].p;
    unsigned long long *cnt = (unsigned long long *)h->scratch[SC_CNT].p;
    if (h->tf_figures) h->tf_launches++;
    TfScope timed(h);
    switch (f.op) {
        case TTX_TOP_PRODUCT: hipLaunchKernelGGL(k_tf_slots<TF_PRODUCT>, grid, block, lds, h->stream, O, nslot, hidx, hreq, hval, tval, cnt); break;
        case TTX_TOP_RATIO: hipLaunchKernelGGL(k_tf_slots<TF_RATIO>, grid, block, lds, h->stream, O, nslot, hidx, hreq, hval, tval, cnt); break;
        case TTX_TOP_SQRTABS: hipLaunchKernelGGL(k_tf_slots<TF_SQRTABS>, grid, block, lds, h->stream, O, nslot, hidx, hreq, hval, tval, cnt); break;
        default: {
            hipLaunchKernelGGL(k_tf_slots<TF_DEVICE>, grid, block, lds, h->stream, O, nslot, hidx, hreq, hval, tval, cnt);
            DevFun &c = *f.comb;
            int m = O.m, d = O.d;
            const int *n = P.n + 1;
            const double *par = c.par, *tv = tval;
            const unsigned cg = (unsigned)std::max<long long>(1, std::min<long long>((nslot + c.info.block - 1) / c.info.block, 4096));
            void *args[] = {&m, &d, &n, &par, &nslot, &hidx, &hreq, &tv, &hval};
            DEVFUN_LAUNCHCHECK(hipModuleLaunchKernel(c.slots, cg, 1, 1, (unsigned)c.info.block, 1, 1, 0, h->stream, args, nullptr));
        }
// ... 781 lines not shown
    const KLaunch de = KUNIT_(k_halfstep_de, slots, dim3(64), s.lds_de, true);
    const KLaunch det3 = KUNIT2_(k_halfstep_det, 3, dim3(1, G), dim3(64 * 14), s.lds_det, true);
    const KLaunch det1 = KUNIT2_(k_halfstep_det, 1, dim3(1, G), dim3(64 * 6), s.lds_det6, true);
    const KLaunch de5 = KUNIT_(k_halfstep_de5, slots, dim3(64 * DE5_W), s.lds_de5, true);
    const KLaunch rows = KUNIT2_(k_lottery_eval_de_rows, false, cand4, dim3(64), s.lds_der, true);
    const KLaunch rows_tab = KUNIT2_(k_lottery_eval_de_rows, true, cand4, dim3(64), s.lds_der, true);
    if (fastk) p.lot_eval = KLaunch();
    else if (FUN == FUN_MVN && s.mvn_v2) p.lot_eval = kl(k_lottery_eval_mvn, "k_lottery_eval_mvn", cand, dim3(64), s.lds_mvn);
    else if (FUN == FUN_ISING && P.de_cut && s.de_v2 && s.lot_cand)
        p.lot_eval = s.de_lot_point ? kl(k_lottery_eval_decp, "k_lottery_eval_decp", cand, dim3(64), sizeof(double) * (2 * (size_t)(d + 64) + 2048), true)
                                    : kl(k_lottery_eval_dec, "k_lottery_eval_dec", cand, dim3(64), s.lds_de, true);
    else if (FUN == FUN_ISING && s.lot_wave) p.lot_eval = s.lot_rows == 2 ? rows_tab : rows;
    if (p.lot_eval) { p.lottery.grid = dim3(1, G); p.lottery.block = dim3(512); }
    if (fastk) { p.half[p.ntier++].k = p.base; p.half_vals = 0; }
    else if (FUN == FUN_MVN && s.mvn_v2) p.half[p.ntier++].k = kl(k_halfstep_mvn, "k_halfstep_mvn", slots, dim3(64), s.lds_mvn);
    else if (FUN == FUN_ISING && s.de_v2) {
        if (h->de_team() && !h->de_v5()) { p.half[p.ntier++] = {det3, s.de_team_units}; p.half[p.ntier++] = {det1, s.de_team6_units}; }
        p.half[p.ntier++].k = h->de_v5() ? de5 : P.de_cut ? kl(k_halfstep_dec, "k_halfstep_dec", slots, dim3(64), s.lds_de, true) : de;
    } else { p.half[p.ntier++].k = p.base; p.half_vals = s.half_vals; }
    p.fullpiv = FUN == FUN_HOST ? ChainPlan::FP_COLUMNS : P.fp_mfma ? ChainPlan::FP_MFMA : ChainPlan::FP_PLAIN;
    p.accept = kl(k_accept, "k_accept", dim3(2 * p.nfb + 2 * NM + 1, G), dim3(TTX_BLK), sizeof(double) * std::max<size_t>(RM + 2, (size_t)std::min<int>(RM, 64) * std::min<int>(RM, 64)));
    {
        const bool own_rows = FUN != FUN_HOST && !(FUN == FUN_ISING && P.arith && P.ising_id != 1);
        const InitSamplesPlan ip = init_samples_plan(s.lds_par, VS, h->d, (long)s.nn * s.snum, own_rows, s.init_wide);
        p.srows = ip.rows;
        p.init_samples = kl(k_init_samples<FUN>, KFUN_(k_init_samples), dim3(G), dim3(ip.threads), ip.lds, ip.rows != 0);
        p.init_fibers = kl(k_init_fibers<FUN>, KFUN_(k_init_fibers), dim3(h->NC, G), dim3(256), s.lds_par);
    }
    if (s.de_npair) p.tables = P.de_cut ? kl(k_de_ctables, "k_de_ctables", dim3(2 * RM, G), dim3(256), sizeof(double) * (size_t)(d + 2))
                                    : kl(k_de_tables, "k_de_tables", dim3((2 * (d + 1) * RM + 255) / 256, G), dim3(256), 0);
    else if (fastk && !P.fpersist) p.tables = kl(k_fast_tables<FUN>, KFUN_(k_fast_tables), dim3(2 * RM, G), dim3(64), sizeof(double) * 2 * (d + 8));
    if (nproc > 1) {
        const size_t lds_b = s.lds_par + 16 + sizeof(short) * 2 * VS + sizeof(double) * (64 * 64 + 4) +
                             (P.bnd_wave ? sizeof(double) * (std::max<size_t>(2 * (size_t)de_rows_stride(d), 3 * (size_t)d + 2) + 8 + (P.de_cut ? 64 * 32 : 0)) : 0);
        p.exch_boundary = kl(k_exch_boundary<FUN>, KFUN_(k_exch_boundary), dim3(2 * NM, G), dim3(TTX_BLK), lds_b, true);
        if constexpr (FUN != FUN_HOST) p.exch_tail = kl(k_exch_tail<FUN>, KFUN_(k_exch_tail), dim3(2 * NM + 1, G), dim3(TTX_BLK), std::max(lds_b, lds_fpersist(P)), true);
    }
    {
        int ft = 256;
        while (ft > 64 && sizeof(double) * ((size_t)RM * RM + (size_t)ft * RM) > TTX_LDS_FIN) ft >>= 1;
        const size_t lds_f = sizeof(double) * ((size_t)RM * RM + (size_t)ft * RM);
        p.fl = lds_f <= TTX_LDS_WORK ? 1 : 0;
        const dim3 gr(h->NC, G, std::max(1, std::min(64, (NM * RM + ft - 1) / ft)));
        p.fin_luar = kl(k_fin_luar, "k_fin_luar", gr, dim3(ft), p.fl ? lds_f : 0, p.fl != 0);
        p.fin_lual = kl(k_fin_lual, "k_fin_lual", gr, dim3(ft), p.fl ? lds_f : 0, p.fl != 0);
    }
    return p;
}
#undef KFUN_
#undef KUNIT_
#undef KUNIT2_

#ifdef TTX_STAMPS
static int dump_stamps(ttx_engine *h)
{
    const DevProb &P = h->P;
    if (P.dbg) {
        std::vector<long long> hb(8 * 64 * 8);
        HIPCHECK(hipMemcpy(hb.data(), P.dbg, sizeof(long long) * hb.size(), hipMemcpyDeviceToHost));
        long long t0 = 0;
        for (long long v : hb) if (v && (!t0 || v < t0)) t0 = v;
        for (int hh = 0; hh < 8; hh++) {
            bool any = false;
            for (int w = 0; w < 64; w++) if (hb[((size_t)hh * 64 + w) * 8]) any = true;
            if (!any) continue;
            fprintf(stderr, "half-step %d (cycles since the first stamp; per wave: start eval-done reduced published polled reduced2)\n", hh);
            for (int w = 0; w < 64; w++) {
                const long long *e = &hb[((size_t)hh * 64 + w) * 8];
                if (!e[0]) continue;
                fprintf(stderr, "  blk %d wave %d: %7lld %7lld %7lld %7lld %7lld %7lld\n", w / 4, w % 4, e[0] - t0, e[1] - t0, e[2] - t0, e[3] - t0, e[4] - t0, e[5] - t0);
            }
        }
    }
    GroupState g0s;
    HIPCHECK(hipMemcpy(&g0s, P.gs, sizeof(GroupState), hipMemcpyDeviceToHost));
    for (int k = 0; k < 2; k++) {
        fprintf(stderr, "stamps kernel %d (n=%lld):", k, g0s.nstamp[k]);
        for (int x = 0; x < 16; x++) fprintf(stderr, " %.2fus", g0s.nstamp[k] ? 0.01 * (double)g0s.stamp[k][x] / (double)g0s.nstamp[k] : 0.0);
        fprintf(stderr, "\n");
    }
    return TTX_OK;
}
#endif

template <int FUN>
struct SweepRun {
    using clk = std::chrono::steady_clock;
    ttx_engine *const h; DevProb &P; const hipStream_t st;
    const int d, G, nproc, cluster, fused;
    const clk::time_point t0 = clk::now();
    LoopPlan L; ChainPlan plan;
    DevProb Pq;
    double val = 1.0, val_prev = 1.0;
    int strike = 0, sweeps = 0; bool ready = false, fin_enqueued = false;
    double *sum_final = nullptr;
    explicit SweepRun(ttx_engine *h_) : h(h_), P(h_->P), st(h_->stream), d(h_->d), G(h_->G), nproc(h_->cfg.nproc), cluster(h_->cluster_nb()), fused(h_->sel.fused) {}
    double since() const { return std::chrono::duration<double>(clk::now() - t0).count(); }
    template <class... A>
    int EV(const KLaunch &k, A... a)
    {
        if (FUN != FUN_HOST) { launch(st, k, P, a...); return TTX_OK; }
        DevProb Q = P;
        Q.hostpass = 1; launch(st, k, Q, a...);
        if (int rc = slot_eval(h)) return rc;
        Q.hostpass = 2; launch(st, k, Q, a...);
        return TTX_OK;
    }
    int prepare()
    {
        LoopIn in;
        in.whole = cluster || fused; in.cluster = cluster != 0; in.profile = h->profile; in.pipeline_off = env_off("TTX_PIPELINE");
        in.W = h->W; in.nproc = nproc; in.has_quad = P.has_quad; in.host_pass = FUN == FUN_HOST;
        in.sweep_tail = h->sel.sweep_tail; in.sweep_tail_side = h->sel.sweep_tail_side; in.maxrank = h->cfg.maxrank;
        in.head_direct = h->sel.head_direct; in.fin_early = h->sel.fin_early; in.fin_skip_exch = h->sel.fin_skip_exch;
        L = loop_plan(in);
        P.tail_side = L.side ? 1 : 0;
        h->recs.clear(); h->tapes.clear();
        plan = chain_plan<FUN>(h);
        for (const KLaunch *k : plan.all()) if (k->raise) if (int rc = ensure_lds(h, k->fn, k->lds)) return rc;
        if (fused) if (int rc = ensure_lds(h, reinterpret_cast<const void *>(k_sweep_fused), h->sel.lds_fused)) return rc;
        if (cluster) { if (int rc = ensure_lds_cluster(h)) return rc; *h->h_abort = 0; }
        Pq = P;
        if (L.pipe) Pq.r = P.rq;
        hipLaunchKernelGGL(k_reset, dim3(64), dim3(256), 0, st, P, h->SB, h->QB);
        {
            KScope ks(h, TTX_K_OTHER, 4);
            if (int rc = EV(plan.init_samples, h->sel.snum, h->sel.nn, FUN == FUN_HOST ? 0 : plan.srows, 0)) return rc;
            if (int rc = EV(plan.init_fibers)) return rc;
            hipLaunchKernelGGL(k_init_factors, dim3(h->NC, G), dim3(256), lds_fpersist(P), st, P);
            hipLaunchKernelGGL(k_init_final, dim3(G), dim3(256), 0, st, P, h->sel.init_wave ? 1 : 0, L.head_direct ? h->h_sum_base : (double *)nullptr);
        }
        if (L.head) {
            h->h_sum = h->h_sum_base;
            if (!L.head_direct) {
                hipLaunchKernelGGL(k_collect, dim3(1), dim3(256), 0, st, P);
                HIPCHECK(hipMemcpyAsync(h->h_sum, P.sumrecv, sizeof(double) * h->SB, hipMemcpyDeviceToHost, st));
            }
            HIPCHECK(hipEventRecord(h->ev_sum[0], st));
            if (int rc = launch_sweep_kernel(1)) return rc;
            HIPCHECK(hipEventSynchronize(h->ev_sum[0]));
        } else if (int rc = readback(h)) return rc;
        HIPCHECK(hipGetLastError());
        for (int g = 0; g < nproc; g++) val = (g == 0) ? h->h_sum[SUM_HDR + g] : val * h->h_sum[SUM_HDR + g];
        if (!P.has_quad) val = 0.0;
        val_prev = val;
        record(0, 0);
        ready = (1 >= h->cfg.maxrank);
        return TTX_OK;
    }
    int launch_sweep_kernel(int it_)
    {
        const CreatePlan &s = h->sel;
        int dir = 2 - it_ % 2, epoch = it_, nsteps = h->nbmax, NB = s.cluster, ldsinv = s.cluster_ldsinv;
        int zkeep = (s.cluster_zkeep ? CL_ZKEEP : 0) | (s.cl_lists ? CL_ZCARRY : 0) | (s.cl_word ? CL_WORD : 0) | (s.cl_powtab ? CL_POWTAB : 0);
        const dim3 grid(8 * NB * ((G + 7) / 8)), block(CB);
        KScope ks(h, TTX_K_HALFSTEP, 1);
        if (!cluster) hipLaunchKernelGGL(k_sweep_fused, dim3(G), dim3(FB), s.lds_fused, st, P, dir, nsteps);
        else if (s.cluster_coop) {
            void *args[] = {&P, &dir, &nsteps, &NB, &ldsinv, &epoch, &zkeep};
            HIPCHECK(hipLaunchCooperativeKernel(reinterpret_cast<const void *>(cluster_kernel(s.cluster_var)), grid, block, args, (unsigned)s.lds_cluster, st));
        } else hipLaunchKernelGGL(cluster_kernel(s.cluster_var), grid, block, s.lds_cluster, st, P, dir, nsteps, NB, ldsinv, epoch, zkeep);
        return TTX_OK;
    }
    int enqueue_chain_sweep(int it_)
    {
        const int dir = 2 - it_ % 2;
        const int rb = std::min((int)h->RM, it_ + 1);
        const int units = (h->sel.de_test_fault && it_ == h->sel.de_test_fault) ? 1 : rb * ((h->NM + 63) / 64);
        KLaunch half = plan.half[plan.ntier - 1].k;
        for (int t = plan.ntier - 2; t >= 0; t--) if (units * G <= plan.half[t].upto) { half = plan.half[t].k; half.grid.x = units; }
        for (int pp = 1; pp <= h->nbmax; pp++) {
            if (plan.tables) { KScope ks(h, TTX_K_OTHER); launch(st, plan.tables, P, dir, pp); }
            if (h->cfg.pivoting < 0) { if (int rc = enqueue_full_pivoting(dir, pp, rb)) return rc; }
            else {
                if (plan.lot_eval) {
                    KScope ks(h, TTX_K_LOTTERY, 3);
                    launch(st, plan.lottery, P, dir, pp, plan.lot_vals, 1);
                    launch(st, plan.lot_eval, P);
                    launch(st, plan.lottery, P, dir, pp, plan.lot_vals, 2);
                } else { KScope ks(h, TTX_K_LOTTERY); if (int rc = EV(plan.lottery, dir, pp, plan.lot_vals, 0)) return rc; }
                KScope ks(h, TTX_K_HALFSTEP, h->H);
                for (int hh = 0; hh < h->H; hh++) {
                    if (plan.half_vals < 0) launch(st, half, P, hh, dir, h->mode);
                    else if (int rc = EV(half, hh, dir, h->mode, plan.half_vals)) return rc;
                }
            }
            { KScope ks(h, TTX_K_ACCEPT); launch(st, plan.accept, P, h->H, plan.nfb); }
        }
        return TTX_OK;
    }
    int enqueue_full_pivoting(int dir, int pp, int rb)
    {
        KScope ks(h, TTX_K_HALFSTEP, 5);
        KLaunch cols = plan.base;
        cols.grid.z = h->NM * h->RM;
        hipLaunchKernelGGL(k_bond_begin, dim3(G), dim3(64), 0, st, P, dir, pp);
        if (plan.fullpiv == ChainPlan::FP_MFMA) {
            const int side = h->RM * h->NM, gx = (side + 63) / 64;
            launch(st, cols, P, 0, dir, 4, plan.base_vals);
            hipLaunchKernelGGL(k_full_gemm_argmax, dim3(gx, gx, G), dim3(256), 0, st, P);
            hipLaunchKernelGGL(k_full_resolve2, dim3(G), dim3(256), 0, st, P, gx, gx);
        } else if (plan.fullpiv == ChainPlan::FP_COLUMNS) {
            for (int z = 0; z < h->NM * rb; z++) {
                DevProb Q = P;
                Q.zbase = z;
                Q.hostpass = 1; launch(st, plan.base, Q, 0, dir, 3, 0);
                if (int rc = slot_eval(h)) return rc;
                Q.hostpass = 2; launch(st, plan.base, Q, 0, dir, 3, 0);
            }
            hipLaunchKernelGGL(k_full_resolve, dim3(G), dim3(256), 0, st, P);
        } else {
            launch(st, cols, P, 0, dir, 3, plan.base_vals);
            hipLaunchKernelGGL(k_full_resolve, dim3(G), dim3(256), 0, st, P);
        }
        if (int rc = EV(plan.base, 0, dir, 2, plan.base_vals)) return rc;
        return EV(plan.base, 1, dir, 2, plan.base_vals);
    }
    int enqueue_sweep_end(int it_)
    {
        const int slot = it_ & 1;
        if (L.side) return end_side(it_);
        if (L.forkq) HIPCHECK(hipStreamWaitEvent(st, h->ev_val[slot ^ 1], 0));
        if (int rc = L.tail ? end_tail(it_) : end_classic(it_)) return rc;
        if (L.pipe) HIPCHECK(hipEventRecord(h->ev_sum[slot], st));
        if (!P.has_quad) return TTX_OK;
        if (L.forkq) HIPCHECK(hipStreamWaitEvent(h->qstream, h->ev_sum[slot], 0));
        return enqueue_quadrature(it_, L.forkq ? h->qstream : st);
    }
    int end_side(int it_)
    {
        const int slot = it_ & 1;
        HIPCHECK(hipStreamWaitEvent(st, h->ev_val[slot ^ 1], 0));
        KScope ks(h, TTX_K_EXCHANGE, 1);
        launch(st, plan.exch_tail, P, it_);
        HIPCHECK(hipEventRecord(h->ev_tail[slot], st));
        return TTX_OK;
    }
    int end_tail(int it_)
    {
        { KScope ks(h, TTX_K_EXCHANGE, 1); launch(st, plan.exch_tail, P, it_); }
        hipLaunchKernelGGL(k_sweep_end, dim3(1), dim3(256), 0, st, P, it_, h->h_sum_base + (size_t)(it_ & 1) * h->SB, 1);
        return TTX_OK;
    }
    int end_classic(int it_)
    {
        {
            KScope ks(h, TTX_K_EXCHANGE, (h->W > 1 ? 4 : 2) + (nproc > 1 ? 1 : 0));
            if (!cluster) hipLaunchKernelGGL(k_exch_pack, dim3(G), dim3(256), 0, st, P, 0);
            if (h->W > 1) {
                hipLaunchKernelGGL(k_exch_localmax, dim3(1), dim3(64), 0, st, P);
                if (int rc = xfer_neighbours(h)) return rc;
                if (int rc = allreduce_dev(h, P.redsend, P.redrecv, 4, 1)) return rc;
            }
            hipLaunchKernelGGL(k_exch_max_apply, dim3(G), dim3(256), lds_fpersist(P), st, P, h->W > 1 ? 1 : 0, nproc > 1 ? 1 : 0);
            if (nproc > 1) { if (int rc = EV(plan.exch_boundary)) return rc; }
        }
        double *const pinned = h->h_sum_base + (size_t)(it_ & 1) * h->SB;
        if (L.pipe) hipLaunchKernelGGL(k_sweep_end, dim3(1), dim3(256), 0, st, P, it_, h->W > 1 ? P.sumsend : pinned, 0);
        if (L.pipe && h->W > 1) {
            if (int rc = allreduce_dev(h, P.sumsend, P.sumrecv, h->SB, 0)) return rc;
            HIPCHECK(hipMemcpyAsync(pinned, P.sumrecv, sizeof(double) * h->SB, hipMemcpyDeviceToHost, st));
        }
        return TTX_OK;
    }
    int enqueue_quadrature(int it_, hipStream_t sq)
    {
        const int slot = it_ & 1;
        KScope ks(h, TTX_K_QUAD, nproc > 1 ? 3 : 2);
        if (int rc = launch_quad(h, sq, L.pipe ? Pq : P, 0, P.quadw, L.fin_early ? h->ev_qb[slot] : nullptr)) return rc;
        if (L.pipe) {
            HIPCHECK(hipMemcpyAsync(h->h_val + slot, &P.gs[0].val, sizeof(double), hipMemcpyDeviceToHost, sq));
            HIPCHECK(hipEventRecord(h->ev_val[slot], sq));
        }
        return h->cb_error ? fail(TTX_EHIP, "host transport: a sendrecv / allreduce callback failed") : TTX_OK;
    }
    int enqueue_side(int it_)
    {
        const int slot = it_ & 1;
        hipStream_t sq = h->qstream;
        HIPCHECK(hipStreamWaitEvent(sq, h->ev_tail[slot], 0));
        hipLaunchKernelGGL(k_sweep_summary, dim3(1), dim3(256), 0, sq, P, it_, h->h_sum_base + (size_t)slot * h->SB);
        HIPCHECK(hipEventRecord(h->ev_sum[slot], sq));
        return enqueue_quadrature(it_, sq);
    }
    int enqueue_final(int after_val)
    {
        if (fin_enqueued) return TTX_OK;
        fin_enqueued = true;
        const bool early = L.fin_early && after_val >= 0;
        if (early) HIPCHECK(hipEventRecord(h->ev_fin[0], st));
        if (after_val >= 0) HIPCHECK(hipStreamWaitEvent(st, early ? h->ev_qb[after_val] : h->ev_val[after_val], 0));
        if (!early) HIPCHECK(hipMemsetAsync(P.ctl, 0, sizeof(int) * 3, st));
        {
            KScope ks(h, TTX_K_OTHER, 2);
            if (L.final_exchange(sweeps)) {
                hipLaunchKernelGGL(k_exch_pack, dim3(G), dim3(256), 0, st, P, 1);
                if (int rc = xfer_neighbours(h)) return rc;
                hipLaunchKernelGGL(k_exch_apply, dim3(G), dim3(256), lds_fpersist(P), st, P);
            }
            launch(st, plan.fin_luar, P, plan.fl);
            launch(st, plan.fin_lual, P, plan.fl);
        }
        if (!early) return TTX_OK;
        const hipStream_t sq = h->qstream;
        HIPCHECK(hipStreamWaitEvent(sq, h->ev_fin[0], 0));
        HIPCHECK(hipMemsetAsync(P.ctl, 0, sizeof(int) * 3, sq));
        sum_final = h->h_sum_base + (size_t)(after_val ^ 1) * h->SB;
        if (int rc = readback_enqueue(h, sum_final, sq)) return rc;
        HIPCHECK(hipEventRecord(h->ev_fin[1], sq));
        return TTX_OK;
    }
    void record(int it_, int dir)
    {
        ttx_sweep_rec r{};
        r.it = it_; r.dir = dir; r.erank = erank_host(h, rank0_view(h, it_).data()); r.neval = (int64_t)h->h_sum[SUM_NEVAL]; r.val = val;
        r.amax = h->h_sum[SUM_AMAX]; r.pivotmax = it_ ? h->h_sum[SUM_PMAX] : -1; r.pivotmin = it_ ? h->h_sum[SUM_PMIN] : -1; r.seconds = since();
        h->recs.push_back(r);
        if (h->cfg.verbose) print_line(h, r, val_prev);
    }
    int process_sweep(int it_)
    {
        const int slot = it_ & 1;
        sweeps = it_;
        if (L.pipe) {
            HIPCHECK(hipEventSynchronize(h->ev_sum[slot]));
            h->h_sum = h->h_sum_base + (size_t)slot * h->SB;
        } else if (int rc = readback(h)) return rc;
        const StopRule sr = stop_rule(it_, h->cfg.maxrank, h->cfg.accuracy, h->h_sum[SUM_PMAX], h->h_sum[SUM_AMAX], strike);
        if (L.pipe && sr.ready) if (int rc = enqueue_final(P.has_quad ? slot : -1)) return rc;
        if (P.has_quad) {
            if (L.pipe) { HIPCHECK(hipEventSynchronize(h->ev_val[slot])); val = h->h_val[slot]; }
            else val = h->h_sum[SUM_VAL];
        }
        HIPCHECK(hipGetLastError());
        if (cluster && *(volatile int *)h->h_abort) { h->cluster_aborted = true; return fail(TTX_EHIP, "cluster sweep kernel: barrier timed out (workgroups of a bond group were not co-resident)"); }
        record(it_, 2 - it_ % 2);
        const size_t o = h->tapes.size();
        h->tapes.resize(o + (size_t)(d + 1) * 4, -1);
        for (int p = 1; p < d; p++) for (int x = 0; x < 4; x++) h->tapes[o + (size_t)p * 4 + x] = (int32_t)sum_bond(h, p)[1 + x];
        val_prev = val;
        strike = sr.strikes;
        ready = ready || sr.ready;
        return TTX_OK;
    }
    int run()
    {
        if (int rc = prepare()) return rc;
        if (!L.pipe) {
            for (int it = 1; !ready; it++) {
                if (int rc = (cluster || fused) ? launch_sweep_kernel(it) : enqueue_chain_sweep(it)) return rc;
                if (int rc = enqueue_sweep_end(it)) return rc;
                if (int rc = process_sweep(it)) return rc;
            }
        } else if (!ready) {
            if (L.forkq) { HIPCHECK(hipEventRecord(h->ev_val[0], h->qstream)); HIPCHECK(hipEventRecord(h->ev_val[1], h->qstream)); }
            if (!L.head) if (int rc = launch_sweep_kernel(1)) return rc;
            for (int it = 1; !ready; it++) {
                if (int rc = enqueue_sweep_end(it)) return rc;
                if (it + 1 < h->cfg.maxrank) if (int rc = launch_sweep_kernel(it + 1)) return rc;
                if (L.side) if (int rc = enqueue_side(it)) return rc;
                if (int rc = process_sweep(it)) return rc;
            }
        }
        if (int rc = enqueue_final(-1)) return rc;
        if (sum_final) h->h_sum = sum_final;
        if (int rc = sum_final ? readback_wait(h) : readback(h)) return rc;
        if (sum_final) HIPCHECK(hipEventSynchronize(h->ev_fin[1]));
        HIPCHECK(hipGetLastError());
#ifdef TTX_STAMPS
        if (int rc = dump_stamps(h)) return rc;
#endif
        h->neval = (int64_t)h->h_sum[SUM_NEVAL];
        h->k_bytes[TTX_K_HALFSTEP] += h->h_sum[SUM_BYTES];
        h->n_resid = (int64_t)h->h_sum[SUM_NRESID];
        h->rfinal = global_ranks(h);
        h->seconds = since();
        h->ran = true;
        return TTX_OK;
    }
};
template <int FUN>
static int run_impl(ttx_engine *h) { return SweepRun<FUN>(h).run(); }

template <class F>
static int with_fun(const ttx_engine *h, const char *who, F f)
{
    switch (h->cfg.fun_id) {
        case TTX_FUN_ISING: return f(std::integral_constant<int, FUN_ISING>());
        case TTX_FUN_STDNORM: return f(std::integral_constant<int, FUN_STDNORM>());
        case TTX_FUN_HOST:
            if (who && !h->hfun) return fail(TTX_ESTATE, "%s: call ttx_set_integrand_host first", who);
            return f(std::integral_constant<int, FUN_HOST>());
        case TTX_FUN_COSCOEFF: return f(std::integral_constant<int, FUN_HOST>());
        case TTX_FUN_DEVICE:
            if (who && !h->dfun) return fail(TTX_ESTATE, "%s: call ttx_set_integrand_device first", who);
            return f(std::integral_constant<int, FUN_HOST>());
        case TTX_FUN_TRAINS:
            if (who && !h->tfun) return fail(TTX_ESTATE, "%s: call ttx_set_integrand_trains first", who);
            return f(std::integral_constant<int, FUN_HOST>());
        case TTX_FUN_PULLBACK:
            if (who && !(h->pfun && h->pfun->comb)) return fail(TTX_ESTATE, "%s: call ttx_set_integrand_pullback with a combiner first", who);
            return f(std::integral_constant<int, FUN_HOST>());
        default: return f(std::integral_constant<int, FUN_MVN>());
    }
}

static void reset_kernel_stats(ttx_engine *h)
{
// ... 1065 lines not shown
    const size_t lds = sizeof(double) * TTX_TF_WAVES * tf_lds_doubles(O.ldx, O.d);
    const dim3 block(64 * TTX_TF_WAVES);
    for (int64_t o = 0; o < npts; o += (int64_t)chunk) {
        long long c = std::min<int64_t>((int64_t)chunk, npts - o);
        const dim3 grid(tf_grid(h, c));
        HIPCHECK(hipMemcpyAsync(sind, ind + (size_t)o * d, sizeof(int) * (size_t)c * d, hipMemcpyHostToDevice, h->stream));
        h->tf_launches++;
        {
            TfScope timed(h);
            switch (f.op) {
                case TTX_TOP_PRODUCT: hipLaunchKernelGGL(k_tf_list<TF_PRODUCT>, grid, block, lds, h->stream, O, c, (const int *)sind, sout, tval, cnt); break;
                case TTX_TOP_RATIO: hipLaunchKernelGGL(k_tf_list<TF_RATIO>, grid, block, lds, h->stream, O, c, (const int *)sind, sout, tval, cnt); break;
                case TTX_TOP_SQRTABS: hipLaunchKernelGGL(k_tf_list<TF_SQRTABS>, grid, block, lds, h->stream, O, c, (const int *)sind, sout, tval, cnt); break;
                default: {
                    hipLaunchKernelGGL(k_tf_list<TF_DEVICE>, grid, block, lds, h->stream, O, c, (const int *)sind, sout, tval, cnt);
                    DevFun &cb = *f.comb;
                    int m = O.m, dd = d;
                    const int *n = h->P.n + 1, *ip = sind;
                    const double *par = cb.par, *tv = tval;
                    const unsigned cg = (unsigned)std::max<long long>(1, std::min<long long>((c + cb.info.block - 1) / cb.info.block, 4096));
                    void *args[] = {&m, &dd, &n, &par, &c, &ip, &tv, &sout};
                    DEVFUN_LAUNCHCHECK(hipModuleLaunchKernel(cb.list, cg, 1, 1, (unsigned)cb.info.block, 1, 1, 0, h->stream, args, nullptr));
                }
            }
        }
        HIPCHECK(hipMemcpyAsync(out + o, sout, sizeof(double) * (size_t)c, hipMemcpyDeviceToHost, h->stream));
        HIPCHECK(hipStreamSynchronize(h->stream));
    }
    HIPCHECK(hipGetLastError());
    return tf_finish(h);
}

static int ev_train(ttx_engine *h, EvTrain *T)
{
    const int d = h->d;
    std::vector<const double *> cp(d);
    std::vector<int> r(h->rfinal.begin(), h->rfinal.begin() + d + 1), n(h->n1.begin() + 1, h->n1.begin() + 1 + d);
    for (int k = 1; k <= d; k++) cp[k - 1] = core_dev(h, k);
    const int rmax = std::max(1, *std::max_element(r.begin(), r.end()));
    if (rmax > 128) return fail(TTX_EINVAL, "ttx_ijk_batch: ranks up to 128 only (got %d)", rmax);
    OpMeta meta(h->train_host);
    const size_t o_core = meta.put(cp), o_r = meta.put(r), o_n = meta.put(n);
    char *m;
    if (int rc = meta.upload(h, SC_TRAIN, &m)) return rc;
    T->d = d; T->RM = h->RM; T->ldx = (rmax + 3) & ~3; T->SS = h->P.SS;
    T->core = (const double *const *)(m + o_core); T->r = (const int *)(m + o_r); T->n = (const int *)(m + o_n);
    return TTX_OK;
}
static EvPlan ev_plan(ttx_engine *h, EvStage st, int64_t npts, int32_t dd, int32_t mode)
{
    return ev_plan(h->d, h->n1.data() + 1, h->rfinal.data(), h->NM, dev_ncu(h), st, npts, dd, mode, env_chunk("TTX_IJK_CHUNK", op_chunk_default(h->RM)));
}
static int ev_run(ttx_engine *h, const EvPlan &pl, const EvTrain &T, int c, const int *ind, const int *flag, double *out)
{
    const int d = h->d;
    if (pl.eff == TTX_EVAL_EXACT) {
        hipLaunchKernelGGL(k_ev_exact, dim3(pl.g_wave(c)), dim3(256), pl.exact_lds, h->stream, T, (long long)c, ind, flag, out);
        return TTX_OK;
    }
    const size_t NM = h->NM;
    double *X = buf<double>(h, SC_XA), *Z = buf<double>(h, SC_XB);
    int *valid = buf<int>(h, SC_SORT), *perm = valid + c, *cnt = perm + c, *off = cnt + NM, *tile = off + NM + 1, *cur = tile + NM + 1;
    hipLaunchKernelGGL(k_ev_init, dim3(pl.g_wave(c)), dim3(256), 0, h->stream, T, c, ind, flag, valid, X, out);
    const int nb = pl.g_sort(c);
    for (int i = d - 2; i >= 0; i--) {
        const EvStep &s = pl.step[i];
        HIPCHECK(hipMemsetAsync(cnt, 0, sizeof(int) * s.nmode, h->stream));
        hipLaunchKernelGGL(k_ev_hist, dim3(nb), dim3(256), s.hist_lds, h->stream, d, i, s.nmode, c, ind, (const int *)valid, cnt);
        hipLaunchKernelGGL(k_ev_scan, dim3(1), dim3(1024), 0, h->stream, s.nmode, (const int *)cnt, off, tile, cur);
        hipLaunchKernelGGL(k_ev_scatter, dim3(nb), dim3(256), s.hist_lds, h->stream, d, i, s.nmode, c, ind, (const int *)valid, cur, perm);
        if (int rc = with_tier(s.tier, [&](auto mr) {
                constexpr int MR = decltype(mr)::value;
                if (int rc = op_lds_raise(h, reinterpret_cast<const void *>(k_ev_gemm<MR>), s.lds)) return rc;
                hipLaunchKernelGGL(k_ev_gemm<MR>, dim3(pl.g_gemm(i, c)), dim3(256), s.lds.bytes, h->stream, T, i, s.nmode, (const int *)off, (const int *)tile, (const int *)perm,
                                   (const double *)X, Z);
                return (int)TTX_OK;
            })) return rc;
        std::swap(X, Z);
    }
    hipLaunchKernelGGL(k_ev_final, dim3(pl.g_final(c)), dim3(256), 0, h->stream, c, T.ldx, (const int *)valid, (const double *)X, out);
    return TTX_OK;
}
extern "C" int ttx_eval_last_mode(const ttx_engine *h) { return h ? h->ev_last_mode : -1; }

static int ev_batch(ttx_engine *h, const char *who, EvStage st, int64_t npts, int32_t dd, const void *in, double *out, int32_t mode)
{
    int rc = tt_prepare(h, st == EV_HOST_COORD ? "dtt_value" : "dtt_ijk");
    if (rc) return rc;
    if (npts < 0 || (npts > 0 && (!in || !out))) return fail(TTX_EINVAL, "%s: null argument or negative npts", who);
    if (st == EV_HOST_COORD && dd < 1) return fail(TTX_EINVAL, "%s: %d coordinates per point", who, dd);
    if (!op_mode_known(mode)) return fail(TTX_EINVAL, "%s: unknown mode %d", who, mode);
    const EvPlan pl = ev_plan(h, st, npts, dd, mode);
    if (npts == 0) { if (st != EV_HOST_COORD) h->ev_last_mode = pl.eff; return TTX_OK; }
    const int32_t *ind = (const int32_t *)in;
    const double *x = (const double *)in;
    if (st == EV_HOST_COORD)
        for (size_t e = 0; e < (size_t)npts * dd; e++) if (!(x[e] < 2147483648.0)) return fail(TTX_EINVAL, "%s: coordinate %g of point %lld is not below 2^31", who, x[e], (long long)(e / dd));
    EvTrain T;
    if ((rc = ev_train(h, &T)) ||
        (rc = buf_reserve(h, {{SC_IND, pl.b_ind}, {SC_OUT, pl.b_out}, {SC_FLAG, pl.b_flag}, {SC_X, pl.b_x}, {SC_XA, pl.b_xa}, {SC_XB, pl.b_xb}, {SC_SORT, pl.b_sort}}))) return rc;
    const size_t d = h->d;
    int *sind = buf<int>(h, SC_IND), *sflag = st == EV_HOST_COORD ? buf<int>(h, SC_FLAG) : nullptr;
    double *sout = buf<double>(h, SC_OUT), *sx = buf<double>(h, SC_X);
    for (int64_t o = 0; o < npts; o += (int64_t)pl.chunk) {
        const int c = (int)std::min<int64_t>((int64_t)pl.chunk, npts - o);
        if (st == EV_ON_DEVICE) {
            if ((rc = ev_run(h, pl, T, c, ind + (size_t)o * d, nullptr, out + o))) return rc;
            continue;
        }
        if (st == EV_HOST_INDEX) HIPCHECK(hipMemcpyAsync(sind, ind + (size_t)o * d, sizeof(int) * (size_t)c * d, hipMemcpyHostToDevice, h->stream));
        else {
            HIPCHECK(hipMemcpyAsync(sx, x + (size_t)o * dd, sizeof(double) * (size_t)c * dd, hipMemcpyHostToDevice, h->stream));
            hipLaunchKernelGGL(k_ev_digits, g1((size_t)c), dim3(256), 0, h->stream, (int)d, T.n, (int)dd, (long long)c, (const double *)sx, sind, sflag);
        }
        if ((rc = ev_run(h, pl, T, c, sind, sflag, sout))) return rc;
        HIPCHECK(hipMemcpyAsync(out + o, sout, sizeof(double) * c, hipMemcpyDeviceToHost, h->stream));
        HIPCHECK(hipStreamSynchronize(h->stream));
    }
    if (st == EV_ON_DEVICE) HIPCHECK(hipStreamSynchronize(h->stream));
    HIPCHECK(hipGetLastError());
    h->ev_last_mode = pl.eff;
    return TTX_OK;
}
extern "C" int ttx_ijk_batch_dev(ttx_engine *h, int64_t npts, const int32_t *ind_dev, double *out_dev, int32_t mode)
{
    return ev_batch(h, "ttx_ijk_batch_dev", EV_ON_DEVICE, npts, 0, ind_dev, out_dev, mode);
}
extern "C" int ttx_ijk_batch(ttx_engine *h, int64_t npts, const int32_t *ind, double *out, int32_t mode)
{
    return ev_batch(h, "ttx_ijk_batch", EV_HOST_INDEX, npts, 0, ind, out, mode);
}
extern "C" int ttx_value_batch(ttx_engine *h, int64_t npts, int32_t dd, const double *x, double *out, int32_t mode)
{
    return ev_batch(h, "ttx_value_batch", EV_HOST_COORD, npts, dd, x, out, mode);
}

extern "C" int ttx_arith(const ttx_engine *h) { return h ? h->arith() : -1; }
extern "C" int ttx_sweep_path(const ttx_engine *h) { return !h ? -1 : h->cluster_nb() ? 2 : h->sel.fused ? 1 : 0; }
extern "C" int64_t ttx_resid_halfsteps(const ttx_engine *h) { return h ? h->n_resid : 0; }
extern "C" int ttx_cluster_eval(const ttx_engine *h) { return !h ? -1 : h->cluster_nb() ? 1 + h->sel.cluster_var : 0; }
extern "C" int ttx_cluster_fallbacks(const ttx_engine *h) { return h ? h->cluster_fallbacks : 0; }
extern "C" int ttx_cluster_entry(const ttx_engine *h, int64_t out[3])
{
    if (!h || !out) return fail(TTX_EINVAL, "ttx_cluster_entry: null argument");
    out[0] = out[1] = out[2] = 0;
    if (!h->cluster_nb()) return TTX_OK;
    const CreatePlan &s = h->sel;
    out[0] = (s.cl_powtab ? 1 : 0) | (s.cl_word ? 2 : 0) | (s.cl_lists ? 4 : 0);
    GroupState g0s;
    HIPCHECK(hipSetDevice(h->cfg.device));
    HIPCHECK(hipStreamSynchronize(h->stream));
    HIPCHECK(hipMemcpy(&g0s, h->P.gs, offsetof(GroupState, S), hipMemcpyDeviceToHost));
    out[1] = g0s.n_zload; out[2] = g0s.n_wload;
    return TTX_OK;
}
extern "C" int ttx_det_fallbacks(const ttx_engine *h) { return h ? h->det_fallbacks + h->de5_fallbacks : 0; }
extern "C" int ttx_fun_id(const ttx_engine *h) { return h ? h->cfg.fun_id : -1; }
extern "C" int ttx_set_profile(ttx_engine *h, int on) { if (!h) return fail(TTX_EINVAL, "null"); h->profile = on != 0; return TTX_OK; }
static void ct_plan(ttx_engine *h, const std::vector<char> &contracted, CtPlan &pl)
{
    ct_plan(h->d, h->n1.data() + 1, h->rfinal.data(), contracted, pl);
    for (int k = 0; k < h->d; k++) pl.cores[k].src = core_dev(h, k + 1);
}
static int ct_modesum(ttx_engine *h, const CtPlan &pl, const double *w, const CtCore *dcores, const CtTile *dtiles, OpTimer *tm)
{
    int rc;
    if ((rc = buf_reserve(h, SC_W, sizeof(double) * pl.wsize)) || (rc = buf_reserve(h, SC_M, sizeof(double) * std::max<size_t>(pl.msize, 1)))) return rc;
    std::vector<double> ones;
    if (!w) { ones.assign(pl.wsize, 1.0); w = ones.data(); }
    HIPCHECK(hipMemcpyAsync(buf<double>(h, SC_W), w, sizeof(double) * pl.wsize, hipMemcpyHostToDevice, h->stream));
    HIPCHECK(hipStreamSynchronize(h->stream));
    if (pl.tiles.empty()) return TTX_OK;
    if (tm && (rc = tm->start(h->stream))) return rc;
    hipLaunchKernelGGL(k_ct_modesum, dim3((unsigned)pl.tiles.size()), dim3(256), 0, h->stream, dcores, dtiles, h->RM, h->P.SS,
                       (const double *)buf<double>(h, SC_W), buf<double>(h, SC_M));
    return tm ? tm->stop(h->stream) : TTX_OK;
}
static int ct_finish(ttx_engine *h, const CtPlan &pl)
{
    HIPCHECK(hipStreamSynchronize(h->stream));
    HIPCHECK(hipGetLastError());
    h->ct = CtLast{0.0, pl.bytes};
    return pl.tiles.empty() ? TTX_OK : h->timer[TM_MODESUM].ms(&h->ct.ms);
}
static int ct_fill(ttx_engine *h, ttx_engine *e, const std::vector<int> &kept, const double *w)
{
    const int d = h->d, m = (int)kept.size();
    std::vector<char> contracted(d, 1);
    for (int k : kept) contracted[k] = 0;
    CtPlan pl;
    ct_plan(h, contracted, pl);
    const std::vector<int> &r = pl.r;
    std::vector<CtRun> runs;
    std::vector<int> run_left(m, -1);
    int run_trail = -1;
    size_t psize = 0, ssize = 0;
    for (int j = 0; j <= m; j++) {
        const int a = j ? kept[j - 1] + 1 : 0, b = (j < m ? kept[j] : d) - 1;
        if (b < a) continue;
        CtRun R{};
        R.k0 = a; R.cnt = b - a + 1; R.kind = j == 0 ? 0 : j == m ? 1 : 2; R.wmax = 1;
        for (int k = a; k <= b; k++) R.wmax = std::max(R.wmax, r[k + 1]);
        R.poff = psize; R.soff = ssize;
        psize += R.kind == 2 ? (size_t)r[a] * r[b + 1] : R.kind == 0 ? (size_t)r[b + 1] : (size_t)r[a];
        if (R.kind == 2 && 2 * (size_t)r[a] * R.wmax > TTX_CT_LDS) ssize += 2 * (size_t)r[a] * R.wmax;
        if (j < m) run_left[j] = (int)runs.size(); else run_trail = (int)runs.size();
        runs.push_back(R);
    }
    int rc;
    if ((rc = buf_reserve(h, SC_P, sizeof(double) * std::max<size_t>(psize, 1))) ||
        (rc = buf_reserve(h, SC_SCR, sizeof(double) * std::max<size_t>(ssize, 1)))) return rc;
    const double *Pb = buf<double>(h, SC_P);
    std::vector<CtKeep> keeps(m);
    long long items = 0;
    for (int j = 0; j < m; j++) {
        const int k = kept[j];
        CtKeep &K = keeps[j];
        K.src = pl.cores[k].src; K.dst = core_dev(e, j + 1);
        K.r0 = r[k]; K.n = h->n1[k + 1]; K.r1 = r[k + 1];
        K.P = run_left[j] >= 0 ? Pb + runs[run_left[j]].poff : nullptr;
        K.q0 = run_left[j] >= 0 ? r[runs[run_left[j]].k0] : K.r0;
        K.t = (j == m - 1 && run_trail >= 0) ? Pb + runs[run_trail].poff : nullptr;
        K.ncol = (K.n + 15) / 16; K.first = items; K.pad = 0;
        items += (long long)K.ncol * (K.t ? 1 : K.r1);
    }
    if (items > 0x7fffffffll) return fail(TTX_EINVAL, "ttx_contract: too many column tiles (%lld)", items);
    OpMeta meta(h->meta_host);
    const size_t o_cores = meta.put(pl.cores), o_tiles = meta.put(pl.tiles), o_runs = meta.put(runs), o_r = meta.put(r), o_moff = meta.put(pl.moff), o_keeps = meta.put(keeps);
    char *dm;
    if ((rc = meta.upload(h, SC_META, &dm)) ||
        (rc = ct_modesum(h, pl, w, (const CtCore *)(dm + o_cores), (const CtTile *)(dm + o_tiles), &h->timer[TM_MODESUM]))) return rc;
    if (!runs.empty())
        hipLaunchKernelGGL(k_ct_runs, dim3((unsigned)runs.size()), dim3(1024), 0, h->stream, (const CtRun *)(dm + o_runs), (const int *)(dm + o_r), (const size_t *)(dm + o_moff),
                           (const double *)buf<double>(h, SC_M), buf<double>(h, SC_P), buf<double>(h, SC_SCR));
    hipLaunchKernelGGL(k_ct_absorb, dim3((unsigned)items), dim3(64), 0, h->stream, (const CtKeep *)(dm + o_keeps), m, h->RM, h->P.SS, e->RM, e->P.SS);
    return ct_finish(h, pl);
}
extern "C" int ttx_contract(ttx_engine *h, const int32_t *keep, const double *w, ttx_engine **out)
{
    if (out) *out = nullptr;
    if (!keep || !out) return fail(TTX_EINVAL, "ttx_contract: null argument");
    int rc = check_train_one_process(h, "ttx_contract");
    if (rc) return rc;
    const int d = h->d;
    std::vector<int> kept;
    for (int k = 0; k < d; k++) {
        if (keep[k] != 0 && keep[k] != 1) return fail(TTX_EINVAL, "ttx_contract: keep(%d) = %d (0 or 1 expected)", k + 1, keep[k]);
        if (keep[k]) kept.push_back(k);
    }
    const int m = (int)kept.size();
    if (m < 2) return fail(TTX_EINVAL, "ttx_contract: %d kept mode%s, but the engine holds trains of at least two cores: ttx_marginals gives the one-mode marginals, ttx_quad the full sum", m, m == 1 ? "" : "s");
    std::vector<int32_t> nn(m), rr(m + 1, 1);
    for (int j = 0; j < m; j++) { nn[j] = h->n1[kept[j] + 1]; if (j < m - 1) rr[j + 1] = h->rfinal[kept[j] + 1]; }
    rr[0] = kept[0] == 0 ? h->rfinal[0] : 1; rr[m] = kept[m - 1] == d - 1 ? h->rfinal[d] : 1;
    return new_train(out, "ttx_contract", m, nn.data(), rr.data(), h->cfg.device, [&](ttx_engine *e) { return ct_fill(h, e, kept, w); });
}
extern "C" int ttx_marginals(ttx_engine *h, const double *w, double *out)
{
    if (!out) return fail(TTX_EINVAL, "ttx_marginals: null argument");
    int rc = check_train_one_process(h, "ttx_marginals");
    if (rc) return rc;
    const int d = h->d;
    CtPlan pl;
    ct_plan(h, std::vector<char>(d, 1), pl);
    const int ldv = h->RM;
    OpMeta meta(h->meta_host);
    const size_t o_cores = meta.put(pl.cores), o_tiles = meta.put(pl.tiles), o_r = meta.put(pl.r), o_moff = meta.put(pl.moff);
    char *dm;
    if ((rc = meta.upload(h, SC_META, &dm)) || (rc = buf_reserve(h, SC_VEC, sizeof(double) * (2 * (size_t)d + 4) * ldv)) ||
        (rc = buf_reserve(h, SC_OUT, sizeof(double) * pl.wsize)) ||
        (rc = ct_modesum(h, pl, w, (const CtCore *)(dm + o_cores), (const CtTile *)(dm + o_tiles), &h->timer[TM_MODESUM]))) return rc;
    double *L = buf<double>(h, SC_VEC), *S = L + (size_t)d * ldv, *dout = buf<double>(h, SC_OUT);
    hipLaunchKernelGGL(k_ct_chains, dim3(2), dim3(1024), 0, h->stream, d, (const int *)(dm + o_r), (const size_t *)(dm + o_moff), (const double *)buf<double>(h, SC_M), L, S, ldv);
    hipLaunchKernelGGL(k_ct_marg, dim3((unsigned)((pl.wsize + 3) / 4)), dim3(256), 0, h->stream, d, (const CtCore *)(dm + o_cores), (long long)pl.wsize, h->RM, h->P.SS,
                       (const double *)L, (const double *)S, ldv, dout);
    HIPCHECK(hipMemcpyAsync(out, dout, sizeof(double) * pl.wsize, hipMemcpyDeviceToHost, h->stream));
    return ct_finish(h, pl);
}
extern "C" int ttx_contract_modesum(const ttx_engine *h, double *ms, double *bytes)
{
    if (!h || !ms || !bytes) return fail(TTX_EINVAL, "ttx_contract_modesum: null argument");
    *ms = h->ct.ms; *bytes = h->ct.bytes;
    return TTX_OK;
}

namespace {
struct SmLoop { size_t chunk = 0; int gridmax = 0; long long *dcnt = nullptr; };
struct SmPrep {
    SmLoop loop;
    EvTrain T;
    std::vector<size_t> hoff;
    std::vector<SmTile> tiles;
    size_t hsize = 0;
    int nrow = 0;
    double bytes = 0.0;
    char *dm = nullptr;
    size_t o_hoff = 0;
    double *H = nullptr, *grow = nullptr;
    size_t growlen = 0, lds = 0;
    int ldsrow = 0;
};
struct SmStage { void *user; size_t bytes; int slot; void *dev; };
}
static int sm_check_fixed(const ttx_engine *h, const char *who, const int32_t *fixed)
{
    if (fixed) for (int k = 0; k < h->d; k++) if (fixed[k] < 0 || fixed[k] > h->n1[k + 1]) return fail(TTX_EINVAL, "%s: fixed(%d) = %d (0 .. %d expected)", who, k + 1, fixed[k], h->n1[k + 1]);
// ... 1585 lines not shown
```

### ttcross_amd/csrc/ttx_exchange.h

```cpp
#pragma once
#include "ttx_kernels.h"
#include "ttx_de.h"
#include "ttx_mvn.h"

__device__ __forceinline__ void exch_pack_group(const DevProb &P, int g)
{
    const int tid = threadIdx.x, m = P.d;
    GroupState &gs = P.gs[g];
    const int first = gs.first, last = gs.last;
    const int *r = P.r + (size_t)g * (m + 2), *rr = P.rr + (size_t)g * (m + 2), *upd = P.upd + (size_t)g * (m + 2);
    if (tid == 0) {
        double *red = P.red + (size_t)g * 4;
        red[0] = gs.amax; red[1] = gs.pivotmax; red[2] = (gs.pivotmin > 0.0) ? -gs.pivotmin : -999e9;
    }
    {
        const int q = last, u = upd[q];
        char *base = P.msgR + (size_t)g * P.MSZ;
        int *hh = (int *)base; int *ix = hh + XH; double *dd = (double *)(base + P.IOFF);
        if (tid == 0) { hh[0] = u; hh[1] = r[q]; }
        const int rq = r[q];
        const double *gI = inv_ptr(P, g, q, first);
        for (int x = tid; x < rq * rq; x += blockDim.x) dd[(size_t)P.RM * P.NM + x] = gI[x];
        if (u) {
            const short *Lt = L_ptr(P, g, q, first);
            for (int x = tid; x < q; x += blockDim.x) ix[x] = Lt[(size_t)x * P.RM + (rq - 1)];
            const double *A = core_ptr(P, P.arg, g, q + 1, first);
            const int n2 = P.n[q + 1], rrq1 = rr[q + 1];
            for (int x = tid; x < n2 * rrq1; x += blockDim.x) dd[x] = A[(rq - 1) + (size_t)P.RM * (x % n2) + P.SS * (x / n2)];
        }
    }
    {
        const int q = first, u = upd[q];
        char *base = P.msgL + (size_t)g * P.MSZ;
        int *hh = (int *)base; int *ix = hh + XH; double *dd = (double *)(base + P.IOFF);
        if (tid == 0) { hh[0] = u; hh[1] = r[q]; }
        if (u) {
            const int rq = r[q];
            const short *Rt = R_ptr(P, g, q, first);
            for (int x = tid; x < m - q; x += blockDim.x) ix[x] = Rt[(size_t)x * P.RM + (rq - 1)];
            const double *A = core_ptr(P, P.arg, g, q, first);
            const int n1 = P.n[q], rr0 = rr[q - 1];
            for (int x = tid; x < rr0 * n1; x += blockDim.x) dd[x] = A[(x % rr0) + (size_t)P.RM * (x / rr0) + P.SS * (rq - 1)];
        }
    }
}

__global__ void k_exch_localmax(DevProb P)
{
    if (P.ctl[0]) return;
    if (threadIdx.x != 0 || blockIdx.x != 0) return;
    double a = -1e300, b = -1e300, c = -1e300;
    for (int g = 0; g < P.G; g++) { a = fmax(a, P.red[4 * g]); b = fmax(b, P.red[4 * g + 1]); c = fmax(c, P.red[4 * g + 2]); }
    P.redsend[0] = a; P.redsend[1] = b; P.redsend[2] = c; P.redsend[3] = 0.0;
}
__device__ __forceinline__ void exch_apply_group(const DevProb &P, int g)
{
    const int tid = threadIdx.x, m = P.d;
    GroupState &gs = P.gs[g];
    const int first = gs.first, last = gs.last;
    int *r = P.r + (size_t)g * (m + 2), *upd = P.upd + (size_t)g * (m + 2);
    if (P.inL[g]) {
        const int bl = first - 1;
        const int *hh = (const int *)P.inL[g], *ix = hh + XH; const double *dd = (const double *)(P.inL[g] + P.IOFF);
        const int u = hh[0], rnew = hh[1];
        if (u) { short *Lt = L_ptr(P, g, bl, first); for (int x = tid; x < bl; x += blockDim.x) Lt[(size_t)x * P.RM + (rnew - 1)] = (short)ix[x]; }
        double *gI = inv_ptr(P, g, bl, first);
        for (int x = tid; x < rnew * rnew; x += blockDim.x) gI[x] = dd[(size_t)P.RM * P.NM + x];
        if (tid == 0) { upd[bl] = u; r[bl] = rnew; }
        if (u && P.arith && P.fpersist && tid < 64) {
            extern __shared__ __align__(16) double dyn_x[];
            double *xs = dyn_x, *ws = xs + m + 8;
            if (P.fun_id == FUN_MVN) {
                for (int k = tid; k < bl; k += 64) xs[k] = P.par[ix[k] - 1] - P.aux[k];
                __builtin_amdgcn_wave_barrier();
                mvn_entry_scratch(P, xs, bl, 0, fast_dv(P, 0, g, bl, first) + (rnew - 1), fast_near(P, 0, g, bl, first) + (rnew - 1), fast_piv(P, 0, g, bl, first) + (rnew - 1), tid);
            } else {
            for (int k = tid; k < bl; k += 64) { xs[k] = P.par[ix[k] - 1]; ws[k] = P.par[P.n[1] + ix[k] - 1]; }
            __builtin_amdgcn_wave_barrier();
            fast_entry_scratch(xs, ws, bl, 0, fast_near(P, 0, g, bl, first) + (rnew - 1), fast_piv(P, 0, g, bl, first) + (rnew - 1), P.RM, tid);
            }
        }
    }
    if (P.inR[g]) {
        const int br = last + 1;
        const int *hh = (const int *)P.inR[g], *ix = hh + XH;
        const int u = hh[0], rnew = hh[1];
        if (u) { short *Rt = R_ptr(P, g, br, first); for (int x = tid; x < m - br; x += blockDim.x) Rt[(size_t)x * P.RM + (rnew - 1)] = (short)ix[x]; }
        if (tid == 0) { upd[br] = u; r[br] = rnew; }
        if (u && P.arith && P.fpersist && tid >= 64 && tid < 128) {
            extern __shared__ __align__(16) double dyn_x[];
            double *xs = dyn_x + 2 * (m + 8), *ws = xs + m + 8;
            const int lane_ = tid - 64;
            if (P.fun_id == FUN_MVN) {
                for (int k = lane_; k < m - br; k += 64) xs[k] = P.par[ix[k] - 1] - P.aux[br + k];
                __builtin_amdgcn_wave_barrier();
                mvn_entry_scratch(P, xs, m - br, br, fast_dv(P, 1, g, br, first) + (rnew - 1), fast_near(P, 1, g, br, first) + (rnew - 1), fast_piv(P, 1, g, br, first) + (rnew - 1), lane_);
            } else {
            for (int k = lane_; k < m - br; k += 64) { xs[k] = P.par[ix[k] - 1]; ws[k] = P.par[P.n[1] + ix[k] - 1]; }
            __builtin_amdgcn_wave_barrier();
            fast_entry_scratch(xs, ws, m - br, 1, fast_near(P, 1, g, br, first) + (rnew - 1), fast_piv(P, 1, g, br, first) + (rnew - 1), P.RM, lane_);
            }
        }
    }
}

__global__ __launch_bounds__(256) void k_exch_pack(DevProb P, int force) { if (P.ctl[0] && !force) return; exch_pack_group(P, blockIdx.x); }
__global__ __launch_bounds__(256) void k_exch_apply(DevProb P) { exch_apply_group(P, blockIdx.x); }

__device__ __forceinline__ void exch_max_group(const DevProb &P, int g, int from_recv)
{
    double a = -1e300, b = -1e300, c = -1e300;
    if (from_recv) { a = P.redrecv[0]; b = P.redrecv[1]; c = P.redrecv[2]; }
    else for (int x = 0; x < P.G; x++) { a = fmax(a, P.red[4 * x]); b = fmax(b, P.red[4 * x + 1]); c = fmax(c, P.red[4 * x + 2]); }
    GroupState &gs = P.gs[g];
    gs.amax = a; gs.pivotmax = b; gs.pivotmin = (-c == 999e9) ? -1.0 : -c;
    gs.pivotmax_prev = b;
}
__global__ __launch_bounds__(256) void k_exch_max_apply(DevProb P, int from_recv, int do_apply)
{
    if (P.ctl[0]) return;
    const int g = blockIdx.x;
    if (threadIdx.x == 0) exch_max_group(P, g, from_recv);
    if (do_apply) exch_apply_group(P, g);
}

template <int FUN, bool MSG>
__device__ __forceinline__ void exch_boundary_block(const DevProb &P, int bx, int g, int par_)
{
    extern __shared__ __align__(16) double dyn[];
    __shared__ double s_bc;
    const int tid = threadIdx.x, m = P.d;
    GroupState &gs = P.gs[g];
    double *amax_to = MSG ? &gs.amax_bnd[par_] : &gs.amax;
    const int first = gs.first, last = gs.last;
    const int *r = P.r + (size_t)g * (m + 2), *rr = P.rr + (size_t)g * (m + 2), *upd = P.upd + (size_t)g * (m + 2);
    double *par = dyn;
    const int VSr = ((m + 7) & ~7) + 8;
    short *rowA = (short *)(((size_t)(dyn + P.npar) + 15) & ~(size_t)15), *rowB = rowA + VSr;
    double *lu = (double *)(rowB + VSr);
    double *wscr = lu + 64 * 64 + 4;
    __shared__ double s_corner;
    const bool dewave = (FUN == FUN_ISING) && P.ising_id != 1 && P.bnd_wave;
    const bool mvwave = (FUN == FUN_MVN) && P.bnd_wave;
    if (bx < P.NM) {
        const int k = bx, p = last, br = last + 1;
        if (!P.inR[g]) return;
        const int *hh = (const int *)P.inR[g], *ix = hh + XH;
        if (!(MSG ? hh[0] : upd[br]) || k >= P.n[br]) return;
        const int rp = r[p], rrp = rr[p], snew = (MSG ? hh[1] : r[br]) - 1, n2 = P.n[br];
        const double *msg = (const double *)(P.inR[g] + P.IOFF);
        double *A = core_ptr(P, P.arg, g, br, first), *W = core_ptr(P, P.row, g, br, first);
        double a = 0.0;
        if (tid < rrp) a = msg[tid + (size_t)rrp * k];
        if (upd[p]) {
            for (int x = tid; x < P.npar; x += TTX_BLK) par[x] = P.par[x];
            const int *vp = vip_ptr(P, g, p, first) + 4 * (rp - 1);
            const short *Lt = L_ptr(P, g, p - 1, first), *Rt = R_ptr(P, g, br, first);
            auto dimv = [&](int s) -> short { return (s < p) ? Lt[(size_t)(s - 1) * P.RM + (vp[0] - 1)] : (s == p) ? (short)vp[1] : (s == p + 1) ? (short)(k + 1) : MSG ? (short)ix[s - p - 2] : Rt[(size_t)(s - p - 2) * P.RM + snew]; };
            for (int x = tid; x < VSr; x += TTX_BLK) { rowA[x] = (x < p - 1) ? dimv(x + 1) : (short)1; rowB[x] = (x < m - p) ? dimv(p + 1 + x) : (short)1; }
            __syncthreads();
            if (dewave || mvwave) {
                if (tid < 64) {
                    const double c_ = dewave ? de_corner_wave(P, par, rowA, p, (int)vp[1], rowB, wscr, tid) : mvn_corner_wave(P, par, rowA, p, (int)vp[1], rowB, wscr, tid);
                    if (tid == 0) s_corner = c_;
                }
                __syncthreads();
            }
            if (tid == rrp) {
                Src3 sx{rowA, p - 1, (int)vp[1], rowB};
                a = (dewave || mvwave) ? s_corner : eval_src3<FUN, true>(P, par, sx, (long)g * P.HS + k);
                if (!HOST_PASS1(FUN, P)) {
                    atomic_max_pos(amax_to, fabs(a));
                    if (!MSG && k == 0) atomicAdd((unsigned long long *)&gs.neval, (unsigned long long)n2);
                }
            }
        }
        if (HOST_PASS1(FUN, P)) return;
        if (tid < rp) A[tid + (size_t)P.RM * k + P.SS * snew] = a;
        const double *gI = inv_ptr(P, g, p, first);
        double tmp = 0.0, xf = 0.0;
        if (rp <= 64) {
            __syncthreads();
            for (int x = tid; x < rp * rp; x += TTX_BLK) lu[x] = gI[x];
            __syncthreads();
            if (tid < 64) xf = dev_solve_L<1>(lu, rp, a, tid, 0);
        } else
        for (int s = 0; s < rp; s++) {
            if (tid == s) { xf = (s == 0) ? a : a + (-1.0) * tmp; s_bc = xf; }
            __syncthreads();
            if (tid > s && tid < rp) tmp = tmp + s_bc * gI[tid * tid + s];
            __syncthreads();
        }
        if (tid < rp) W[k + (size_t)P.NM * snew + P.SW * tid] = xf;
    } else {
        const int j = bx - P.NM, p = first, bl = first - 1;
        if (!P.inL[g]) return;
        const int *hh = (const int *)P.inL[g], *ix = hh + XH;
        if (!(MSG ? hh[0] : upd[bl]) || j >= P.n[p]) return;
        const int rp = r[p], rrp = rr[p], inew = (MSG ? hh[1] : r[bl]) - 1, n1 = P.n[p];
        const double *msg = (const double *)(P.inL[g] + P.IOFF);
        double *A = core_ptr(P, P.arg, g, p, first), *C = core_ptr(P, P.col, g, p, first);
        double y = 0.0;
        if (tid < rrp) y = msg[j + (size_t)n1 * tid];
        if (upd[p]) {
            for (int x = tid; x < P.npar; x += TTX_BLK) par[x] = P.par[x];
            const int *vp = vip_ptr(P, g, p, first) + 4 * (rp - 1);
            const short *Lt = L_ptr(P, g, bl, first), *Rt = R_ptr(P, g, p + 1, first);
            auto dimv = [&](int s) -> short { return (s < p) ? (MSG ? (short)ix[s - 1] : Lt[(size_t)(s - 1) * P.RM + inew]) : (s == p) ? (short)(j + 1) : (s == p + 1) ? (short)vp[2] : Rt[(size_t)(s - p - 2) * P.RM + (vp[3] - 1)]; };
            for (int x = tid; x < VSr; x += TTX_BLK) { rowA[x] = (x < p - 1) ? dimv(x + 1) : (short)1; rowB[x] = (x < m - p) ? dimv(p + 1 + x) : (short)1; }
            __syncthreads();
            if (dewave || mvwave) {
                if (tid < 64) {
                    const double c_ = dewave ? de_corner_wave(P, par, rowA, p, j + 1, rowB, wscr, tid) : mvn_corner_wave(P, par, rowA, p, j + 1, rowB, wscr, tid);
                    if (tid == 0) s_corner = c_;
                }
                __syncthreads();
            }
            if (tid == rrp) {
                Src3 sx{rowA, p - 1, j + 1, rowB};
                y = (dewave || mvwave) ? s_corner : eval_src3<FUN, true>(P, par, sx, (long)g * P.HS + P.NM + j);
                if (!HOST_PASS1(FUN, P)) {
                    atomic_max_pos(amax_to, fabs(y));
                    if (!MSG && j == 0) atomicAdd((unsigned long long *)&gs.neval, (unsigned long long)n1);
                }
            }
        }
        if (HOST_PASS1(FUN, P)) return;
        if (tid < rp) A[inew + (size_t)P.RM * j + P.SS * tid] = y;
        const double *gI = inv_ptr(P, g, p, first);
        if (rp <= 64) {
            __syncthreads();
            for (int x = tid; x < rp * rp; x += TTX_BLK) lu[x] = gI[x];
            __syncthreads();
            if (tid < 64) y = dev_solve_U<1>(lu, rp, y, dev_solve_rdg(lu, rp, tid), tid, 0);
        } else
        for (int s = 0; s < rp; s++) {
            if (tid == s) { y = (1.0 / gI[(s + 1) * (s + 1) - 1]) * y; s_bc = y; }
            __syncthreads();
            if (tid > s && tid < rp) y = y + (-gI[tid * tid + tid + s]) * s_bc;
            __syncthreads();
        }
        if (tid < rp) C[inew + (size_t)P.RM * j + P.SS * tid] = y;
    }
}
template <int FUN>
__global__ __launch_bounds__(TTX_BLK) void k_exch_boundary(DevProb P)
{
    if (P.ctl[0]) return;
    exch_boundary_block<FUN, false>(P, (int)blockIdx.x, (int)blockIdx.y, 0);
}
template <int FUN>
__global__ __launch_bounds__(TTX_BLK) void k_exch_tail(DevProb P, int it)
{
    if (P.ctl[0]) return;
    const int g = blockIdx.y;
    if ((int)blockIdx.x < 2 * P.NM) { exch_boundary_block<FUN, true>(P, (int)blockIdx.x, g, it & 1); return; }
    if (threadIdx.x == 0) {
        exch_max_group(P, g, 0);
        GroupState &gs = P.gs[g];
        const int *upd = P.upd + (size_t)g * (P.d + 2);
        const int u_r = P.inR[g] ? ((const int *)P.inR[g])[0] : 0, u_l = P.inL[g] ? ((const int *)P.inL[g])[0] : 0;
        gs.neval += boundary_neval(P.inR[g] != nullptr, u_r, upd[gs.last], P.n[gs.last + 1], P.inL[g] != nullptr, u_l, upd[gs.first], P.n[gs.first]);
    }
    exch_apply_group(P, g);
    if (!P.tail_side) return;
    __syncthreads();
    const int m = P.d, tid = threadIdx.x, par = it & 1;
    const GroupState &gs = P.gs[g];
    const int *r = P.r + (size_t)g * (m + 2), *tp = P.tape + (size_t)g * (m + 2) * 4;
    int *rq = P.rq + (size_t)g * (m + 2), *tq = P.tail_tape + ((size_t)par * P.G + g) * (m + 2) * 4;
    for (int x = tid; x < m + 2; x += blockDim.x) rq[x] = r[x];
    for (int x = 4 * gs.first + tid; x < 4 * (gs.last + 1); x += blockDim.x) tq[x] = tp[x];
    if (tid == 0) {
        TailRec t;
        t.amax = gs.amax; t.pivotmax = gs.pivotmax; t.pivotmin = gs.pivotmin; t.bytes_half = gs.bytes_half; t.initval = gs.initval;
        t.neval = gs.neval; t.n_resid = gs.n_resid;
        P.tailrec[(size_t)par * P.G + g] = t;
    }
}
```

### ttcross_amd/engine.py

```python
import ctypes
import os
import shutil
import subprocess
from ctypes import POINTER, c_char_p, c_double, c_int32, c_int64, c_uint8, c_uint64, c_void_p

import numpy as np

TTX_FUN_ISING, TTX_FUN_STDNORM, TTX_FUN_MVN, TTX_FUN_HOST = 1, 2, 3, 4
TTX_FUN_COSCOEFF = 5
TTX_FUN_DEVICE = 6
TTX_FUN_TRAINS = 7
TTX_FUN_PULLBACK = 8
TTX_PULLBACK_MAX = 8
TTX_TRAINS_MAX = 8
TTX_TOP_PRODUCT, TTX_TOP_RATIO, TTX_TOP_SQRTABS, TTX_TOP_DEVICE = 1, 2, 3, 4
TRAIN_OPS = {"product": TTX_TOP_PRODUCT, "ratio": TTX_TOP_RATIO, "sqrtabs": TTX_TOP_SQRTABS}
TTX_EVAL_EXACT, TTX_EVAL_MFMA, TTX_EVAL_AUTO = 0, 1, 2
EVAL_MODES = {"exact": TTX_EVAL_EXACT, "mfma": TTX_EVAL_MFMA, "auto": TTX_EVAL_AUTO}
TOPK_WHICH = {"abs": 0, "max": 1, "min": 2}
TTX_BASIS_COS, TTX_BASIS_LINEAR, TTX_BASIS_HALVE_FIRST = 1, 2, 1
BASIS_KINDS = {"cos": TTX_BASIS_COS, "linear": TTX_BASIS_LINEAR}
K_NAMES = ("lottery", "halfstep", "accept", "exchange", "quad", "other")

_HERE = os.path.dirname(os.path.abspath(__file__))
# ... 509 lines not shown
            _check(L.ttx_set_integrand_device_file(self._h, os.fsencode(image_or_path), name.encode(), _dp(p) if p.size else None, p.size))
        return self

    @classmethod
    def of_trains(cls, trains, op, maxrank, accuracy=None, pivoting=3, quad=None, nproc=1, combiner=None, par=None, device=None):
        trains = list(trains)
        if not trains:
            raise ValueError("of_trains: at least one train")
        tt = cls(trains[0]._n, TTX_FUN_TRAINS, [], maxrank, pivoting=pivoting, accuracy=accuracy, quad=quad, nproc=nproc,
                 device=trains[0].device if device is None else device)
        try:
            return tt.set_integrand_trains(trains, combiner if combiner is not None else op, par)
        except Exception:
            tt.close()
            raise

    def set_integrand_trains(self, trains, op, par=None):
        L = load_library()
        trains = list(trains)
        hs = (c_void_p * max(len(trains), 1))(*[t._h if t is not None else None for t in trains])
        if isinstance(op, (tuple, list)):
            image_or_path, name = op
            p = np.zeros(0) if par is None else np.ascontiguousarray(par, dtype=np.float64)
            pp = _dp(p) if p.size else None
            if isinstance(image_or_path, (bytes, bytearray, memoryview)):
                img = bytes(image_or_path)
                _check(L.ttx_set_integrand_trains_device(self._h, len(trains), hs, img, len(img), name.encode(), pp, p.size))
            else:
                _check(L.ttx_set_integrand_trains_device_file(self._h, len(trains), hs, os.fsencode(image_or_path), name.encode(), pp, p.size))
        else:
            _check(L.ttx_set_integrand_trains(self._h, len(trains), hs, int(TRAIN_OPS.get(op, op))))
        self._operands = trains
        return self

    def trainfun_last(self):
        ms, nl, ne = c_double(), c_int64(), c_int64()
        _check(load_library().ttx_trainfun_last(self._h, ctypes.byref(ms), ctypes.byref(nl), ctypes.byref(ne)))
        return dict(ms=ms.value, launches=nl.value, elements=ne.value)

    @classmethod
    def pullback(cls, layers, ref, fun, maxrank, accuracy=None, pivoting=3, quad=None, nproc=1, par=None, device=None):
        layers = list(layers)
        if not layers:
            raise ValueError("pullback: at least one layer")
        d = layers[0][0].d
        refs = [ref] * d if not isinstance(ref, (list, tuple)) or (len(ref) and np.ndim(ref[0]) == 0) else list(ref)
        refs = [np.ascontiguousarray(r, dtype=np.float64).ravel() for r in refs]
        tt = cls([r.size for r in refs], TTX_FUN_PULLBACK, [], maxrank, pivoting=pivoting, accuracy=accuracy, quad=quad, nproc=nproc,
                 device=layers[0][0].device if device is None else device)
        try:
            return tt.set_integrand_pullback(layers, refs, fun, par)
        except Exception:
            tt.close()
            raise

    def set_integrand_pullback(self, layers, ref, fun=None, par=None):
        L = load_library()
        layers = [tuple(y) for y in layers]
        arr = (_Layer * max(len(layers), 1))()
        keep = []
        for t, (x, nodes, gamma) in enumerate(layers):
            arr[t].x = x._h if x is not None else None
            arr[t].gamma = float(gamma)
            if x is not None and nodes is not None:
                _, rowp = x._node_rows(nodes, f"set_integrand_pullback: layer {t + 1}")
                arr[t].nodes = ctypes.cast(rowp, POINTER(POINTER(c_double)))
                keep.append(rowp)
        refs = [ref] * self.d if not isinstance(ref, (list, tuple)) or (len(ref) and np.ndim(ref[0]) == 0) else list(ref)
        _, refp = self._node_rows(refs, "set_integrand_pullback: ref")
        p = np.zeros(0) if par is None else np.ascontiguousarray(par, dtype=np.float64)
        pp = _dp(p) if p.size else None
        if fun is None:
            _check(L.ttx_set_integrand_pullback(self._h, len(layers), arr, refp, None, 0, None, pp, p.size))
        else:
            image_or_path, name = fun
            if isinstance(image_or_path, (bytes, bytearray, memoryview)):
                img = bytes(image_or_path)
                _check(L.ttx_set_integrand_pullback(self._h, len(layers), arr, refp, img, len(img), name.encode(), pp, p.size))
            else:
                _check(L.ttx_set_integrand_pullback_file(self._h, len(layers), arr, refp, os.fsencode(image_or_path), name.encode(), pp, p.size))
        self._operands = [y[0] for y in layers]
        return self

    def pullback_points(self, ind):
        ind = np.ascontiguousarray(ind, dtype=np.int32).reshape(-1, self.d)
        x, lq, v = np.zeros((ind.shape[0], self.d)), np.zeros(ind.shape[0]), np.zeros(ind.shape[0])
        _check(load_library().ttx_pullback_points(self._h, ind.shape[0], _ip(ind), _dp(x), _dp(lq), _dp(v)))
        return x, lq, v

    def pullback_last(self):
        ms, nl, ne, nf = c_double(), c_int64(), c_int64(), c_int64()
        _check(load_library().ttx_pullback_last(self._h, ctypes.byref(ms), ctypes.byref(nl), ctypes.byref(ne), ctypes.byref(nf)))
        return dict(ms=ms.value, launches=nl.value, elements=ne.value, failed=nf.value)

    def eval_device(self, ind):
        ind = np.ascontiguousarray(ind, dtype=np.int32).reshape(-1, self.d)
        out = np.zeros(ind.shape[0])
        _check(load_library().ttx_eval_device(self._h, ind.shape[0], _ip(ind), _dp(out)))
        return out

    @property
    def host_calls(self):
        return int(load_library().ttx_host_calls(self._h))

    @property
    def fun_id(self):
        L = load_library()
        L.ttx_fun_id.argtypes = [c_void_p]
        return L.ttx_fun_id(self._h)

    @property
    def arith(self):
        L = load_library()
        L.ttx_arith.argtypes = [c_void_p]
        return ("exact", "fast")[L.ttx_arith(self._h)]

    def sweep_path(self):
        L = load_library()
        L.ttx_sweep_path.argtypes = [c_void_p]
        return ("chain", "fused", "cluster")[L.ttx_sweep_path(self._h)]

    def plan(self):
        L = load_library()
        L.ttx_plan_describe.argtypes = [c_void_p, c_char_p, c_int64]
        buf = ctypes.create_string_buffer(1024)
        _check(L.ttx_plan_describe(self._h, buf, len(buf)))
        return dict(line.split(": ", 1) for line in buf.value.decode().splitlines())

    def cluster_eval(self):
        L = load_library()
        L.ttx_cluster_eval.argtypes = [c_void_p]
        return ("none", "predicated", "chunks", "closed")[L.ttx_cluster_eval(self._h)]

    @property
    def resid_halfsteps(self):
        L = load_library()
        L.ttx_resid_halfsteps.argtypes = [c_void_p]
        L.ttx_resid_halfsteps.restype = c_int64
        return int(L.ttx_resid_halfsteps(self._h))

    @property
    def cluster_fallbacks(self):
        L = load_library()
        L.ttx_cluster_fallbacks.argtypes = [c_void_p]
        return int(L.ttx_cluster_fallbacks(self._h))

    def cluster_entry(self):
        L = load_library()
        L.ttx_cluster_entry.argtypes = [c_void_p, ctypes.POINTER(c_int64)]
        out = (c_int64 * 3)()
        _check(L.ttx_cluster_entry(self._h, out))
        return {"powtab": bool(out[0] & 1), "word": bool(out[0] & 2), "lists": bool(out[0] & 4), "lists_taken": int(out[1]), "word_taken": int(out[2])}

    @property
    def det_fallbacks(self):
        L = load_library()
        L.ttx_det_fallbacks.argtypes = [c_void_p]
        return int(L.ttx_det_fallbacks(self._h))

    def set_profile(self, on=True):
        _check(load_library().ttx_set_profile(self._h, 1 if on else 0))

    def run(self):
        _check(load_library().ttx_run(self._h))
        return self

    @property
    def neval(self):
        return int(load_library().ttx_neval(self._h))

    @property
    def seconds(self):
        return float(load_library().ttx_seconds(self._h))

    def sweeps(self):
        L = load_library()
        k = L.ttx_num_sweeps(self._h)
        buf = (SweepRec * k)()
        _check(L.ttx_get_sweeps(self._h, buf, k))
        return [dict(it=b.it, dir=b.dir, erank=b.erank, neval=b.neval, val=b.val, amax=b.amax,
                     pivotmax=b.pivotmax, pivotmin=b.pivotmin, seconds=b.seconds) for b in buf]

    def tapes(self):
        L = load_library()
        k = L.ttx_num_sweeps(self._h) - 1
        out = np.zeros((max(k, 0), self.d + 1, 4), dtype=np.int32)
        if k > 0:
            _check(L.ttx_get_tapes(self._h, _ip(out), out.size))
        return out

    def fast_tables(self, group, side=None, bond=None, cols=None):
        L = load_library()
        L.ttx_fast_tables.argtypes = [c_void_p, c_int32, c_int32, c_int32, c_int32, POINTER(c_int32), POINTER(c_int32)] + [POINTER(c_double)] * 3
        info = np.zeros(3, dtype=np.int32)
        if side is None:
            _check(L.ttx_fast_tables(self._h, group, 0, 0, 0, _ip(info), None, None, None, None))
            return int(info[1]), int(info[2])
        cols = 4096 if cols is None else int(cols)
        d = self.d
        idx = np.zeros(d * cols, dtype=np.int32)
        near, dv, piv = np.zeros((d + 1) * cols), np.zeros((d + 1) * cols), np.zeros(8 * cols)
        _check(L.ttx_fast_tables(self._h, group, side, bond, cols, _ip(info), _ip(idx), _dp(near), _dp(dv), _dp(piv)))
        r = int(info[0])
        ln = bond if side == 0 else d - bond
        return dict(r=r, idx=idx[:d * r].reshape(d, r)[:ln], near=near[:(d + 1) * r].reshape(d + 1, r), dv=dv[:(d + 1) * r].reshape(d + 1, r),
                    piv=piv[:8 * r].reshape(8, r))

    def ranks(self):
        r = np.zeros(self.d + 1, dtype=np.int32)
        _check(load_library().ttx_get_ranks(self._h, _ip(r)))
        return r

    def core(self, k):
        L = load_library()
        r = self.ranks()
        sz = L.ttx_core_size(self._h, k)
        buf = np.zeros(sz, dtype=np.float64)
        _check(L.ttx_get_core(self._h, k, _dp(buf)))
        return buf.reshape((r[k - 1], self._n[k - 1], r[k]), order="F")

    def _weights(self, w, who):
        if w is None:
            return None
        if len(w) != self.d or any(np.size(q) != int(nk) for q, nk in zip(w, self._n)):
            raise ValueError(f"{who}: {self.d} weight vectors of lengths {list(map(int, self._n))} expected")
        return np.ascontiguousarray(np.concatenate([np.asarray(q, dtype=np.float64).ravel() for q in w]))

    def quad(self, w=None):
        v = c_double()
        wa = self._weights(w, "quad")
        _check(load_library().ttx_quad(self._h, _dp(wa), ctypes.byref(v)))
        return v.value

    def contract(self, keep, w=None):
        k = np.asarray(keep)
        if k.ndim != 1 or k.size != self.d:
            raise ValueError(f"contract: {self.d} keep flags expected")
        k = np.ascontiguousarray(k.astype(np.int32))
        wa = self._weights(w, "contract")
        h = c_void_p()
        _check(load_library().ttx_contract(self._h, _ip(k), _dp(wa), ctypes.byref(h)))
        return TTCross._adopt(h, self.device)

    def marginals(self, w=None):
        out = np.zeros(int(self._n.sum()))
        _check(load_library().ttx_marginals(self._h, _dp(self._weights(w, "marginals")), _dp(out)))
        return [a.copy() for a in np.split(out, np.cumsum(self._n)[:-1])]

    def contract_modesum(self):
        ms, by = c_double(), c_double()
        _check(load_library().ttx_contract_modesum(self._h, ctypes.byref(ms), ctypes.byref(by)))
        return ms.value, by.value

    @staticmethod
    def lincomb(coefs, trains):
        trains = list(trains)
        c = np.ascontiguousarray(np.asarray(coefs, dtype=np.float64).ravel())
        if not trains or c.size != len(trains):
            raise ValueError(f"lincomb: one coefficient per train expected (got {c.size} and {len(trains)})")
        hs = (c_void_p * len(trains))(*[t._h for t in trains])
        h = c_void_p()
        _check(load_library().ttx_lincomb(len(trains), _dp(c), hs, ctypes.byref(h)))
        return TTCross._adopt(h, trains[0].device)

    def axpby(self, alpha, beta, y):
        return TTCross.lincomb([alpha, beta], [self, y])

    def hadamard(self, y):
        h = c_void_p()
        _check(load_library().ttx_hadamard(self._h, y._h, ctypes.byref(h)))
        return TTCross._adopt(h, self.device)

    def dist(self, y):
        t = TTCross.lincomb([1.0, -1.0], [self, y])
        try:
            return t.norm()
        finally:
            t.close()

    def wdot(self, y, w=None):
        t = self.hadamard(y)
        try:
            return t.quad(w)
        finally:
            t.close()

    def algebra_last(self):
        ms, rd, wr = c_double(), c_double(), c_double()
        _check(load_library().ttx_algebra_last(self._h, ctypes.byref(ms), ctypes.byref(rd), ctypes.byref(wr)))
        return ms.value, rd.value, wr.value

    @staticmethod
    def lincomb_round(coefs, trains, rank=0, tol=-1.0, rmax=0, seed=0, mode="auto"):
        trains = list(trains)
        c = np.ascontiguousarray(np.asarray(coefs, dtype=np.float64).ravel())
        if not trains or c.size != len(trains):
            raise ValueError(f"lincomb_round: one coefficient per train expected (got {c.size} and {len(trains)})")
        md = _eval_mode(mode)
        hs = (c_void_p * len(trains))(*[t._h for t in trains])
        h = c_void_p()
        _check(load_library().ttx_lincomb_round(len(trains), _dp(c), hs, int(rank), float(tol), int(rmax), int(seed) & (2 ** 64 - 1), md, ctypes.byref(h)))
        return TTCross._adopt(h, trains[0].device)

    def roundsum_last(self):
        ms, fl, md = (c_double * 4)(), c_double(), c_int32()
        l = np.zeros(self.d + 1, dtype=np.int32)
# ... 496 lines not shown
```

Before: 252.7 million evals/s.

## Split exchange packing across blocks, lean tail boundary eval, fused tail event

Result: faster. 256.9 million evals/s (median of 6 runs) (+1.7%).

```diff
diff --git a/include/ttx.h b/include/ttx.h
--- a/include/ttx.h
+++ b/include/ttx.h
@@ -229,6 +229,7 @@
 int ttx_arith(const ttx_engine *h);
 int ttx_cluster_fallbacks(const ttx_engine *h);
 int ttx_cluster_entry(const ttx_engine *h, int64_t out[3]);
+int ttx_sweep_gap(const ttx_engine *h, int32_t out[4]);
 int ttx_det_fallbacks(const ttx_engine *h);
 int ttx_fun_id(const ttx_engine *h);
 int64_t ttx_resid_halfsteps(const ttx_engine *h);
diff --git a/ttcross_amd/csrc/ttx_cluster.h b/ttcross_amd/csrc/ttx_cluster.h
--- a/ttcross_amd/csrc/ttx_cluster.h
+++ b/ttcross_amd/csrc/ttx_cluster.h
@@ -146,6 +146,7 @@
 #define CL_ZCARRY 2
 #define CL_WORD 4
 #define CL_POWTAB 8
+#define CL_PACK2 16
 static_assert(CL_POWTAB_N == CB, "one table entry per thread of a workgroup");
 __device__ const ClPowTab cl_powtab = cl_make_powtab();
 struct ClArgs { DevProb P; int dir, nsteps, NB, ldsinv, epoch, zkeep; };
@@ -684,6 +685,12 @@
         CST_END();
     }
     CSE_MARK();
+    if (cb == 1) {
+        const ClArgs *K = (const ClArgs *)__builtin_amdgcn_kernarg_segment_ptr();
+        asm volatile("" : "+s"(K));
+        if (cl_pack_block(CL_PACK_LEFT, K->NB, (K->zkeep & CL_PACK2) != 0) == 1) exch_pack_left(K->P, g);
+        CSE(3);
+    }
     if (cb == 0) {
         const ClArgs *K = (const ClArgs *)__builtin_amdgcn_kernarg_segment_ptr();
         asm volatile("" : "+s"(K));
@@ -701,7 +708,8 @@
             if (P.tail_side) gs.amax_bnd[epoch & 1] = 0.0;
         }
         __syncthreads();
-        exch_pack_group(P, g);
+        exch_pack_right(P, g);
+        if (cl_pack_block(CL_PACK_LEFT, K->NB, (K->zkeep & CL_PACK2) != 0) == 0) exch_pack_left(P, g);
         CSE(3);
         CSE_END();
     }
diff --git a/ttcross_amd/csrc/ttx_cluster_rules.h b/ttcross_amd/csrc/ttx_cluster_rules.h
--- a/ttcross_amd/csrc/ttx_cluster_rules.h
+++ b/ttcross_amd/csrc/ttx_cluster_rules.h
@@ -77,4 +77,7 @@
 
 TTX_HD bool cl_word_valid(uint64_t word, uint64_t wpos, uint64_t rngpos) { return word != 0 && wpos == rngpos; }
 TTX_HD bool cl_lists_valid(int tag, int epoch) { return tag != 0 && tag == epoch - 1; }
+#define CL_PACK_RIGHT 0
+#define CL_PACK_LEFT 1
+TTX_HD int cl_pack_block(int part, int NB, bool split) { return (part == CL_PACK_LEFT && split && NB >= 2) ? 1 : 0; }
 TTX_HD size_t cl_zimage_ints(int nsteps, int RM) { return ((size_t)nsteps * 2 * (size_t)RM + 2 * (size_t)nsteps + 3) & ~(size_t)3; }
diff --git a/ttcross_amd/csrc/ttx_create_plan.h b/ttcross_amd/csrc/ttx_create_plan.h
--- a/ttcross_amd/csrc/ttx_create_plan.h
+++ b/ttcross_amd/csrc/ttx_create_plan.h
@@ -65,6 +65,9 @@
     bool cl_powtab_off = false;
     bool cl_word_off = false;
     bool cl_lists_off = false;
+    EnvText tail_event;
+    bool tail_lean_off = false;
+    bool cl_pack2_off = false;
 };
 template <class Get>
 CreateEnv create_env_from(Get get)
@@ -96,6 +99,8 @@
     v.fin_early_off = off("TTX_FIN_EARLY"); v.fin_skip_exch_off = off("TTX_FIN_SKIP_EXCH");
     v.init_wide_off = off("TTX_INIT_WIDE"); v.quad_lds_off = off("TTX_QUAD_LDS");
     v.cl_powtab_off = off("TTX_CL_POWTAB"); v.cl_word_off = off("TTX_CL_WORD"); v.cl_lists_off = off("TTX_CL_LISTS");
+    v.tail_event = text("TTX_TAIL_EVENT"); v.tail_lean_off = off("TTX_TAIL_LEAN");
+    v.cl_pack2_off = off("TTX_CL_PACK2");
     return v;
 }
 struct DevCaps { int ncu = 0; bool coop = false; };
@@ -146,6 +151,9 @@
     int cl_test_abort = 0; bool dbg_waves = false;
     bool sweep_tail = true;
     bool sweep_tail_side = true;
+    bool tail_event_kernel = true;
+    bool tail_lean = true;
+    bool cl_pack2 = true;
     bool head_direct = true;
     size_t lds_qtree = 0;
     bool init_wide = true;
@@ -354,6 +362,10 @@
         }
         p.cl_test_abort = env.cluster_test_abort; p.dbg_waves = env.dbg_waves;
         p.sweep_tail = !env.tail_off; p.sweep_tail_side = !env.tail_side_off;
+        if (env.tail_event.set && env.tail_event.v != "marker" && env.tail_event.v != "kernel")
+            return plan_refuse(p, TTX_EINVAL, "TTX_TAIL_EVENT must be marker or kernel (got %s)", env.tail_event.v.c_str());
+        p.tail_event_kernel = !(env.tail_event.set && env.tail_event.v == "marker");
+        p.tail_lean = !env.tail_lean_off; p.cl_pack2 = !env.cl_pack2_off;
         p.head_direct = !env.head_direct_off; p.init_wave = !env.init_wave_off; p.init_wide = !env.init_wide_off;
         p.fin_early = !env.fin_early_off; p.fin_skip_exch = !env.fin_skip_exch_off;
         const std::string want_sweep = env.sweep.set ? env.sweep.v : "auto";
diff --git a/ttcross_amd/csrc/ttx_engine.hip b/ttcross_amd/csrc/ttx_engine.hip
--- a/ttcross_amd/csrc/ttx_engine.hip
+++ b/ttcross_amd/csrc/ttx_engine.hip
@@ -1,4 +1,5 @@
 #include <hip/hip_runtime.h>
+#include <hip/hip_ext.h>
 
 #include <chrono>
 #include <cmath>
@@ -235,6 +236,7 @@
     int cluster_fallbacks = 0;
     int det_fallbacks = 0, de5_fallbacks = 0;
     bool cluster_aborted = false;
+    bool tail_event_retired = false; int tail_event_fallbacks = 0;
     double *h_svd = nullptr; double svd_seq = 0.0;
     hipStream_t qstream = nullptr;
     hipEvent_t ev_sum[2] = {nullptr, nullptr}, ev_val[2] = {nullptr, nullptr}, ev_tail[2] = {nullptr, nullptr}, ev_qb[2] = {nullptr, nullptr}, ev_fin[2] = {nullptr, nullptr};
@@ -1322,7 +1324,8 @@
     {
         const CreatePlan &s = h->sel;
         int dir = 2 - it_ % 2, epoch = it_, nsteps = h->nbmax, NB = s.cluster, ldsinv = s.cluster_ldsinv;
-        int zkeep = (s.cluster_zkeep ? CL_ZKEEP : 0) | (s.cl_lists ? CL_ZCARRY : 0) | (s.cl_word ? CL_WORD : 0) | (s.cl_powtab ? CL_POWTAB : 0);
+        int zkeep = (s.cluster_zkeep ? CL_ZKEEP : 0) | (s.cl_lists ? CL_ZCARRY : 0) | (s.cl_word ? CL_WORD : 0) | (s.cl_powtab ? CL_POWTAB : 0)
+                    | (s.cl_pack2 ? CL_PACK2 : 0);
         const dim3 grid(8 * NB * ((G + 7) / 8)), block(CB);
         KScope ks(h, TTX_K_HALFSTEP, 1);
         if (!cluster) hipLaunchKernelGGL(k_sweep_fused, dim3(G), dim3(FB), s.lds_fused, st, P, dir, nsteps);
@@ -1397,18 +1400,27 @@
         if (L.forkq) HIPCHECK(hipStreamWaitEvent(h->qstream, h->ev_sum[slot], 0));
         return enqueue_quadrature(it_, L.forkq ? h->qstream : st);
     }
+    int tail_lean() const { return h->sel.tail_lean ? 1 : 0; }
     int end_side(int it_)
     {
         const int slot = it_ & 1;
         HIPCHECK(hipStreamWaitEvent(st, h->ev_val[slot ^ 1], 0));
         KScope ks(h, TTX_K_EXCHANGE, 1);
-        launch(st, plan.exch_tail, P, it_);
+        if (h->sel.tail_event_kernel && !h->tail_event_retired) {
+            const KLaunch &k = plan.exch_tail;
+            int lean = tail_lean();
+            void *args[] = {(void *)&P, (void *)&it_, (void *)&lean};
+            if (hipExtLaunchKernel(k.fn, k.grid, k.block, args, k.lds, st, nullptr, h->ev_tail[slot], 0) == hipSuccess) return TTX_OK;
+            (void)hipGetLastError();
+            h->tail_event_retired = true; h->tail_event_fallbacks++;
+        }
+        launch(st, plan.exch_tail, P, it_, tail_lean());
         HIPCHECK(hipEventRecord(h->ev_tail[slot], st));
         return TTX_OK;
     }
     int end_tail(int it_)
     {
-        { KScope ks(h, TTX_K_EXCHANGE, 1); launch(st, plan.exch_tail, P, it_); }
+        { KScope ks(h, TTX_K_EXCHANGE, 1); launch(st, plan.exch_tail, P, it_, tail_lean()); }
         hipLaunchKernelGGL(k_sweep_end, dim3(1), dim3(256), 0, st, P, it_, h->h_sum_base + (size_t)(it_ & 1) * h->SB, 1);
         return TTX_OK;
     }
@@ -1423,7 +1435,7 @@
                 if (int rc = allreduce_dev(h, P.redsend, P.redrecv, 4, 1)) return rc;
             }
             hipLaunchKernelGGL(k_exch_max_apply, dim3(G), dim3(256), lds_fpersist(P), st, P, h->W > 1 ? 1 : 0, nproc > 1 ? 1 : 0);
-            if (nproc > 1) { if (int rc = EV(plan.exch_boundary)) return rc; }
+            if (nproc > 1) { if (int rc = EV(plan.exch_boundary, tail_lean())) return rc; }
         }
         double *const pinned = h->h_sum_base + (size_t)(it_ & 1) * h->SB;
         if (L.pipe) hipLaunchKernelGGL(k_sweep_end, dim3(1), dim3(256), 0, st, P, it_, h->W > 1 ? P.sumsend : pinned, 0);
@@ -2795,6 +2807,14 @@
     HIPCHECK(hipStreamSynchronize(h->stream));
     HIPCHECK(hipMemcpy(&g0s, h->P.gs, offsetof(GroupState, S), hipMemcpyDeviceToHost));
     out[1] = g0s.n_zload; out[2] = g0s.n_wload;
+    return TTX_OK;
+}
+extern "C" int ttx_sweep_gap(const ttx_engine *h, int32_t out[4])
+{
+    if (!h || !out) return fail(TTX_EINVAL, "ttx_sweep_gap: null argument");
+    const CreatePlan &s = h->sel;
+    out[0] = (s.tail_event_kernel && !h->tail_event_retired) ? 1 : 0; out[1] = h->tail_event_fallbacks;
+    out[2] = s.tail_lean ? 1 : 0; out[3] = s.cl_pack2 ? 1 : 0;
     return TTX_OK;
 }
 extern "C" int ttx_det_fallbacks(const ttx_engine *h) { return h ? h->det_fallbacks + h->de5_fallbacks : 0; }
diff --git a/ttcross_amd/csrc/ttx_exchange.h b/ttcross_amd/csrc/ttx_exchange.h
--- a/ttcross_amd/csrc/ttx_exchange.h
+++ b/ttcross_amd/csrc/ttx_exchange.h
@@ -3,7 +3,7 @@
 #include "ttx_de.h"
 #include "ttx_mvn.h"
 
-__device__ __forceinline__ void exch_pack_group(const DevProb &P, int g)
+__device__ __forceinline__ void exch_pack_right(const DevProb &P, int g)
 {
     const int tid = threadIdx.x, m = P.d;
     GroupState &gs = P.gs[g];
@@ -13,37 +13,36 @@
         double *red = P.red + (size_t)g * 4;
         red[0] = gs.amax; red[1] = gs.pivotmax; red[2] = (gs.pivotmin > 0.0) ? -gs.pivotmin : -999e9;
     }
-    {
-        const int q = last, u = upd[q];
-        char *base = P.msgR + (size_t)g * P.MSZ;
-        int *hh = (int *)base; int *ix = hh + XH; double *dd = (double *)(base + P.IOFF);
-        if (tid == 0) { hh[0] = u; hh[1] = r[q]; }
-        const int rq = r[q];
-        const double *gI = inv_ptr(P, g, q, first);
-        for (int x = tid; x < rq * rq; x += blockDim.x) dd[(size_t)P.RM * P.NM + x] = gI[x];
-        if (u) {
-            const short *Lt = L_ptr(P, g, q, first);
-            for (int x = tid; x < q; x += blockDim.x) ix[x] = Lt[(size_t)x * P.RM + (rq - 1)];
-            const double *A = core_ptr(P, P.arg, g, q + 1, first);
-            const int n2 = P.n[q + 1], rrq1 = rr[q + 1];
-            for (int x = tid; x < n2 * rrq1; x += blockDim.x) dd[x] = A[(rq - 1) + (size_t)P.RM * (x % n2) + P.SS * (x / n2)];
-        }
-    }
-    {
-        const int q = first, u = upd[q];
-        char *base = P.msgL + (size_t)g * P.MSZ;
-        int *hh = (int *)base; int *ix = hh + XH; double *dd = (double *)(base + P.IOFF);
-        if (tid == 0) { hh[0] = u; hh[1] = r[q]; }
-        if (u) {
-            const int rq = r[q];
-            const short *Rt = R_ptr(P, g, q, first);
-            for (int x = tid; x < m - q; x += blockDim.x) ix[x] = Rt[(size_t)x * P.RM + (rq - 1)];
-            const double *A = core_ptr(P, P.arg, g, q, first);
-            const int n1 = P.n[q], rr0 = rr[q - 1];
-            for (int x = tid; x < rr0 * n1; x += blockDim.x) dd[x] = A[(x % rr0) + (size_t)P.RM * (x / rr0) + P.SS * (rq - 1)];
-        }
-    }
-}
+    const int q = last, u = upd[q], rq = r[q], rrq1 = rr[q + 1], n2 = P.n[q + 1];
+    char *base = P.msgR + (size_t)g * P.MSZ;
+    int *hh = (int *)base; int *ix = hh + XH; double *dd = (double *)(base + P.IOFF);
+    if (tid == 0) { hh[0] = u; hh[1] = rq; }
+    const double *gI = inv_ptr(P, g, q, first);
+    for (int x = tid; x < rq * rq; x += blockDim.x) dd[(size_t)P.RM * P.NM + x] = gI[x];
+    if (u) {
+        const short *Lt = L_ptr(P, g, q, first);
+        for (int x = tid; x < q; x += blockDim.x) ix[x] = Lt[(size_t)x * P.RM + (rq - 1)];
+        const double *A = core_ptr(P, P.arg, g, q + 1, first);
+        for (int x = tid; x < n2 * rrq1; x += blockDim.x) dd[x] = A[(rq - 1) + (size_t)P.RM * (x % n2) + P.SS * (x / n2)];
+    }
+}
+__device__ __forceinline__ void exch_pack_left(const DevProb &P, int g)
+{
+    const int tid = threadIdx.x, m = P.d;
+    const int first = P.gs[g].first;
+    const int *r = P.r + (size_t)g * (m + 2), *rr = P.rr + (size_t)g * (m + 2), *upd = P.upd + (size_t)g * (m + 2);
+    const int q = first, u = upd[q], rq = r[q], rr0 = rr[q - 1], n1 = P.n[q];
+    char *base = P.msgL + (size_t)g * P.MSZ;
+    int *hh = (int *)base; int *ix = hh + XH; double *dd = (double *)(base + P.IOFF);
+    if (tid == 0) { hh[0] = u; hh[1] = rq; }
+    if (u) {
+        const short *Rt = R_ptr(P, g, q, first);
+        for (int x = tid; x < m - q; x += blockDim.x) ix[x] = Rt[(size_t)x * P.RM + (rq - 1)];
+        const double *A = core_ptr(P, P.arg, g, q, first);
+        for (int x = tid; x < rr0 * n1; x += blockDim.x) dd[x] = A[(x % rr0) + (size_t)P.RM * (x / rr0) + P.SS * (rq - 1)];
+    }
+}
+__device__ __forceinline__ void exch_pack_group(const DevProb &P, int g) { exch_pack_right(P, g); exch_pack_left(P, g); }
 
 __global__ void k_exch_localmax(DevProb P)
 {
@@ -125,7 +124,7 @@
 }
 
 template <int FUN, bool MSG>
-__device__ __forceinline__ void exch_boundary_block(const DevProb &P, int bx, int g, int par_)
+__device__ __forceinline__ void exch_boundary_block(const DevProb &P, int bx, int g, int par_, int lean)
 {
     extern __shared__ __align__(16) double dyn[];
     __shared__ double s_bc;
@@ -142,22 +141,45 @@
     __shared__ double s_corner;
     const bool dewave = (FUN == FUN_ISING) && P.ising_id != 1 && P.bnd_wave;
     const bool mvwave = (FUN == FUN_MVN) && P.bnd_wave;
+    const char *in_r = nullptr, *in_l = nullptr;
+    if (lean) { in_r = P.inR[g]; in_l = P.inL[g]; }
+    const bool cval = (FUN == FUN_ISING) && lean && P.ising_id == 1 && 4 * VSr <= 64 * 64;
+    double *cAn = lu, *cAw = cAn + VSr, *cBn = cAw + VSr, *cBw = cBn + VSr;
+    const double *gnodes = P.par - 1, *gweights = gnodes + (cval ? P.n[1] : 0);
     if (bx < P.NM) {
         const int k = bx, p = last, br = last + 1;
-        if (!P.inR[g]) return;
-        const int *hh = (const int *)P.inR[g], *ix = hh + XH;
-        if (!(MSG ? hh[0] : upd[br]) || k >= P.n[br]) return;
-        const int rp = r[p], rrp = rr[p], snew = (MSG ? hh[1] : r[br]) - 1, n2 = P.n[br];
-        const double *msg = (const double *)(P.inR[g] + P.IOFF);
+        const char *in = lean ? in_r : P.inR[g];
+        const int *hh = (const int *)in, *ix = hh + XH;
+        int rp, rrp, snew, n2, up = 0;
+        if (lean) {
+            const int *hq = in ? hh : &gs.first;
+            const int u_in = MSG ? hq[0] : upd[br];
+            rp = r[p]; rrp = rr[p]; snew = (MSG ? hq[1] : r[br]) - 1; n2 = P.n[br]; up = upd[p];
+            asm volatile("" ::: "memory");
+            if (!in || !u_in || k >= n2) return;
+        } else {
+            if (!in) return;
+            if (!(MSG ? hh[0] : upd[br]) || k >= P.n[br]) return;
+            rp = r[p]; rrp = rr[p]; snew = (MSG ? hh[1] : r[br]) - 1; n2 = P.n[br];
+        }
+        const double *msg = (const double *)(in + P.IOFF);
         double *A = core_ptr(P, P.arg, g, br, first), *W = core_ptr(P, P.row, g, br, first);
         double a = 0.0;
         if (tid < rrp) a = msg[tid + (size_t)rrp * k];
-        if (upd[p]) {
-            for (int x = tid; x < P.npar; x += TTX_BLK) par[x] = P.par[x];
+        if (!lean) up = upd[p];
+        if (up) {
             const int *vp = vip_ptr(P, g, p, first) + 4 * (rp - 1);
             const short *Lt = L_ptr(P, g, p - 1, first), *Rt = R_ptr(P, g, br, first);
             auto dimv = [&](int s) -> short { return (s < p) ? Lt[(size_t)(s - 1) * P.RM + (vp[0] - 1)] : (s == p) ? (short)vp[1] : (s == p + 1) ? (short)(k + 1) : MSG ? (short)ix[s - p - 2] : Rt[(size_t)(s - p - 2) * P.RM + snew]; };
-            for (int x = tid; x < VSr; x += TTX_BLK) { rowA[x] = (x < p - 1) ? dimv(x + 1) : (short)1; rowB[x] = (x < m - p) ? dimv(p + 1 + x) : (short)1; }
+            if (cval) {
+                for (int x = tid; x < VSr; x += TTX_BLK) {
+                    const int ia = (x < p - 1) ? dimv(x + 1) : 0, ib = (x < m - p) ? dimv(p + 1 + x) : 0;
+                    cAn[x] = ia ? gnodes[ia] : 0.0; cAw[x] = ia ? gweights[ia] : 0.0; cBn[x] = ib ? gnodes[ib] : 0.0; cBw[x] = ib ? gweights[ib] : 0.0;
+                }
+            } else {
+                for (int x = tid; x < P.npar; x += TTX_BLK) par[x] = P.par[x];
+                for (int x = tid; x < VSr; x += TTX_BLK) { rowA[x] = (x < p - 1) ? dimv(x + 1) : (short)1; rowB[x] = (x < m - p) ? dimv(p + 1 + x) : (short)1; }
+            }
             __syncthreads();
             if (dewave || mvwave) {
                 if (tid < 64) {
@@ -168,7 +190,8 @@
             }
             if (tid == rrp) {
                 Src3 sx{rowA, p - 1, (int)vp[1], rowB};
-                a = (dewave || mvwave) ? s_corner : eval_src3<FUN, true>(P, par, sx, (long)g * P.HS + k);
+                if (cval) a = f_ising_c3v(m, p - 1, cAn, cAw, gnodes[vp[1]], gweights[vp[1]], cBn, cBw);
+                else a = (dewave || mvwave) ? s_corner : eval_src3<FUN, true>(P, par, sx, (long)g * P.HS + k);
                 if (!HOST_PASS1(FUN, P)) {
                     atomic_max_pos(amax_to, fabs(a));
                     if (!MSG && k == 0) atomicAdd((unsigned long long *)&gs.neval, (unsigned long long)n2);
@@ -194,20 +217,38 @@
         if (tid < rp) W[k + (size_t)P.NM * snew + P.SW * tid] = xf;
     } else {
         const int j = bx - P.NM, p = first, bl = first - 1;
-        if (!P.inL[g]) return;
-        const int *hh = (const int *)P.inL[g], *ix = hh + XH;
-        if (!(MSG ? hh[0] : upd[bl]) || j >= P.n[p]) return;
-        const int rp = r[p], rrp = rr[p], inew = (MSG ? hh[1] : r[bl]) - 1, n1 = P.n[p];
-        const double *msg = (const double *)(P.inL[g] + P.IOFF);
+        const char *in = lean ? in_l : P.inL[g];
+        const int *hh = (const int *)in, *ix = hh + XH;
+        int rp, rrp, inew, n1, up = 0;
+        if (lean) {
+            const int *hq = in ? hh : &gs.first;
+            const int u_in = MSG ? hq[0] : upd[bl];
+            rp = r[p]; rrp = rr[p]; inew = (MSG ? hq[1] : r[bl]) - 1; n1 = P.n[p]; up = upd[p];
+            asm volatile("" ::: "memory");
+            if (!in || !u_in || j >= n1) return;
+        } else {
+            if (!in) return;
+            if (!(MSG ? hh[0] : upd[bl]) || j >= P.n[p]) return;
+            rp = r[p]; rrp = rr[p]; inew = (MSG ? hh[1] : r[bl]) - 1; n1 = P.n[p];
+        }
+        const double *msg = (const double *)(in + P.IOFF);
         double *A = core_ptr(P, P.arg, g, p, first), *C = core_ptr(P, P.col, g, p, first);
         double y = 0.0;
         if (tid < rrp) y = msg[j + (size_t)n1 * tid];
-        if (upd[p]) {
-            for (int x = tid; x < P.npar; x += TTX_BLK) par[x] = P.par[x];
+        if (!lean) up = upd[p];
+        if (up) {
             const int *vp = vip_ptr(P, g, p, first) + 4 * (rp - 1);
             const short *Lt = L_ptr(P, g, bl, first), *Rt = R_ptr(P, g, p + 1, first);
             auto dimv = [&](int s) -> short { return (s < p) ? (MSG ? (short)ix[s - 1] : Lt[(size_t)(s - 1) * P.RM + inew]) : (s == p) ? (short)(j + 1) : (s == p + 1) ? (short)vp[2] : Rt[(size_t)(s - p - 2) * P.RM + (vp[3] - 1)]; };
-            for (int x = tid; x < VSr; x += TTX_BLK) { rowA[x] = (x < p - 1) ? dimv(x + 1) : (short)1; rowB[x] = (x < m - p) ? dimv(p + 1 + x) : (short)1; }
+            if (cval) {
+                for (int x = tid; x < VSr; x += TTX_BLK) {
+                    const int ia = (x < p - 1) ? dimv(x + 1) : 0, ib = (x < m - p) ? dimv(p + 1 + x) : 0;
+                    cAn[x] = ia ? gnodes[ia] : 0.0; cAw[x] = ia ? gweights[ia] : 0.0; cBn[x] = ib ? gnodes[ib] : 0.0; cBw[x] = ib ? gweights[ib] : 0.0;
+                }
+            } else {
+                for (int x = tid; x < P.npar; x += TTX_BLK) par[x] = P.par[x];
+                for (int x = tid; x < VSr; x += TTX_BLK) { rowA[x] = (x < p - 1) ? dimv(x + 1) : (short)1; rowB[x] = (x < m - p) ? dimv(p + 1 + x) : (short)1; }
+            }
             __syncthreads();
             if (dewave || mvwave) {
                 if (tid < 64) {
@@ -218,7 +259,8 @@
             }
             if (tid == rrp) {
                 Src3 sx{rowA, p - 1, j + 1, rowB};
-                y = (dewave || mvwave) ? s_corner : eval_src3<FUN, true>(P, par, sx, (long)g * P.HS + P.NM + j);
+                if (cval) y = f_ising_c3v(m, p - 1, cAn, cAw, gnodes[j + 1], gweights[j + 1], cBn, cBw);
+                else y = (dewave || mvwave) ? s_corner : eval_src3<FUN, true>(P, par, sx, (long)g * P.HS + P.NM + j);
                 if (!HOST_PASS1(FUN, P)) {
                     atomic_max_pos(amax_to, fabs(y));
                     if (!MSG && j == 0) atomicAdd((unsigned long long *)&gs.neval, (unsigned long long)n1);
@@ -244,17 +286,17 @@
     }
 }
 template <int FUN>
-__global__ __launch_bounds__(TTX_BLK) void k_exch_boundary(DevProb P)
+__global__ __launch_bounds__(TTX_BLK) void k_exch_boundary(DevProb P, int lean)
 {
     if (P.ctl[0]) return;
-    exch_boundary_block<FUN, false>(P, (int)blockIdx.x, (int)blockIdx.y, 0);
+    exch_boundary_block<FUN, false>(P, (int)blockIdx.x, (int)blockIdx.y, 0, lean);
 }
 template <int FUN>
-__global__ __launch_bounds__(TTX_BLK) void k_exch_tail(DevProb P, int it)
+__global__ __launch_bounds__(TTX_BLK) void k_exch_tail(DevProb P, int it, int lean)
 {
     if (P.ctl[0]) return;
     const int g = blockIdx.y;
-    if ((int)blockIdx.x < 2 * P.NM) { exch_boundary_block<FUN, true>(P, (int)blockIdx.x, g, it & 1); return; }
+    if ((int)blockIdx.x < 2 * P.NM) { exch_boundary_block<FUN, true>(P, (int)blockIdx.x, g, it & 1, lean); return; }
     if (threadIdx.x == 0) {
         exch_max_group(P, g, 0);
         GroupState &gs = P.gs[g];
diff --git a/ttcross_amd/engine.py b/ttcross_amd/engine.py
--- a/ttcross_amd/engine.py
+++ b/ttcross_amd/engine.py
@@ -685,6 +685,14 @@
         _check(L.ttx_cluster_entry(self._h, out))
         return {"powtab": bool(out[0] & 1), "word": bool(out[0] & 2), "lists": bool(out[0] & 4), "lists_taken": int(out[1]), "word_taken": int(out[2])}
 
+    def sweep_gap(self):
+        L = load_library()
+        L.ttx_sweep_gap.argtypes = [c_void_p, ctypes.POINTER(ctypes.c_int32)]
+        out = (ctypes.c_int32 * 4)()
+        _check(L.ttx_sweep_gap(self._h, out))
+        return {"tail_event": "kernel" if out[0] else "marker", "tail_event_fallbacks": int(out[1]), "tail_lean": bool(out[2]),
+                "cl_pack2": bool(out[3])}
+
     @property
     def det_fallbacks(self):
         L = load_library()
```
